# pdlfs/old-vpic

Measured on AMD Instinct MI355X. Metric: particle-pushes/sec (full step: advance_p + sort when due + field solve + glue), higher is better.
Workload: dtype f32

## Files before the change

### include/vpic_hip.h

```cpp
#ifndef VPIC_HIP_H
#define VPIC_HIP_H

#include <stddef.h>
#include <stdint.h>

#ifdef __cplusplus
#define VPIC_HIP_STATIC_ASSERT(c, msg) static_assert(c, msg)
extern "C" {
#else
#define VPIC_HIP_STATIC_ASSERT(c, msg) _Static_assert(c, msg)
#endif


typedef struct vpic_particle {
  float dx, dy, dz;
  int32_t i;
  float ux, uy, uz;
  float q;
  int64_t tag, tag2;
} vpic_particle_t;
typedef struct vpic_particle_mover { float dispx, dispy, dispz; int32_t i; } vpic_particle_mover_t;
typedef struct vpic_particle_injector {
  float dx, dy, dz; int32_t i; float ux, uy, uz, q; float dispx, dispy, dispz; int32_t sp_id;
} vpic_particle_injector_t;
// ... 242 lines not shown
int vpic_hip_advance_p_async(vpic_hip_engine_t *e, int sp);
int vpic_hip_advance_p_phase(vpic_hip_engine_t *e, int sp, int phase);
int vpic_hip_exchange_pack_species(vpic_hip_engine_t *e, uint32_t species_mask, void *const dev_msg[6], const int32_t cap[6], int mover_cap);
int vpic_hip_exchange_begin(vpic_hip_engine_t *e);
int vpic_hip_exchange_pack(vpic_hip_engine_t *e, void *const dev_msg[6], const int32_t cap[6], int mover_cap);
int vpic_hip_exchange_inject(vpic_hip_engine_t *e, const void *dev_msg, int cap);
int vpic_hip_exchange_finish(vpic_hip_engine_t *e, const void *const *dev_msgs, int n_msgs , int32_t *headers , int32_t *flags);
int vpic_hip_boundary_p_counts(vpic_hip_engine_t *e, int32_t ns[6]);
void *vpic_hip_boundary_p_send_buffer(vpic_hip_engine_t *e, int face);
int vpic_hip_boundary_p_get_injectors(vpic_hip_engine_t *e, int face, void *dev_dst);
int vpic_hip_boundary_p_inject(vpic_hip_engine_t *e, const void *dev_injectors, int n);
int vpic_hip_face_count(const vpic_hip_engine_t *e, int dir);
int vpic_hip_pack_tang_b(vpic_hip_engine_t *e, int dir, void *dev_buf);
int vpic_hip_unpack_tang_b(vpic_hip_engine_t *e, int dir, const void *dev_buf);
int vpic_hip_pack_jf(vpic_hip_engine_t *e, int dir, void *dev_buf);
int vpic_hip_unpack_jf(vpic_hip_engine_t *e, int dir, const void *dev_buf);

int vpic_hip_clear_rhof(vpic_hip_engine_t *e);
int vpic_hip_accumulate_rho_p(vpic_hip_engine_t *e, int sp);
int vpic_hip_synchronize_rho(vpic_hip_engine_t *e);
int vpic_hip_local_adjust_rho(vpic_hip_engine_t *e);
int vpic_hip_synchronize_rho_self(vpic_hip_engine_t *e, int axis);
int vpic_hip_rho_count(const vpic_hip_engine_t *e, int dir);
int vpic_hip_pack_rho(vpic_hip_engine_t *e, int dir, void *dev_buf);
int vpic_hip_unpack_rho(vpic_hip_engine_t *e, int dir, const void *dev_buf);
int vpic_hip_compute_rhob(vpic_hip_engine_t *e);
int vpic_hip_compute_curl_b(vpic_hip_engine_t *e);
int vpic_hip_synchronize_tang_e_norm_b(vpic_hip_engine_t *e, double *err);
int vpic_hip_compute_div_e_err(vpic_hip_engine_t *e);
int vpic_hip_clean_div_e(vpic_hip_engine_t *e);
int vpic_hip_compute_div_b_err(vpic_hip_engine_t *e);
int vpic_hip_clean_div_b(vpic_hip_engine_t *e);
enum { VPIC_HIP_MSG_NORM_E = 0, VPIC_HIP_MSG_DIV_B = 1, VPIC_HIP_MSG_TANG_E_NORM_B = 2 };
int vpic_hip_face_message_count(const vpic_hip_engine_t *e, int kind, int dir);
int vpic_hip_pack_face_message(vpic_hip_engine_t *e, int kind, int dir, void *dev_buf);
int vpic_hip_unpack_face_message(vpic_hip_engine_t *e, int kind, int dir, const void *dev_buf, double *err);
int vpic_hip_local_adjust_tang_e_norm_b(vpic_hip_engine_t *e);
int vpic_hip_synchronize_tang_e_norm_b_self(vpic_hip_engine_t *e, int axis, double *err);
int vpic_hip_rms_div_e_err_local(vpic_hip_engine_t *e, double *local2);
int vpic_hip_rms_div_b_err_local(vpic_hip_engine_t *e, double *local2);
int vpic_hip_compute_rms_div_e_err(vpic_hip_engine_t *e, double *rms);
int vpic_hip_compute_rms_div_b_err(vpic_hip_engine_t *e, double *rms);

int vpic_hip_clear_hydro(vpic_hip_engine_t *e);
int vpic_hip_accumulate_hydro_p(vpic_hip_engine_t *e, int sp);
int vpic_hip_moments_stats(vpic_hip_engine_t *e, int64_t out[4]);
int vpic_hip_accumulate_hydro_p_select(vpic_hip_engine_t *e, int sp, const vpic_hip_select_t *s);
int vpic_hip_synchronize_hydro(vpic_hip_engine_t *e);
int vpic_hip_local_adjust_hydro(vpic_hip_engine_t *e);
int vpic_hip_synchronize_hydro_self(vpic_hip_engine_t *e, int axis);
int vpic_hip_hydro_count(const vpic_hip_engine_t *e, int dir);
int vpic_hip_pack_hydro(vpic_hip_engine_t *e, int dir, void *dev_buf);
int vpic_hip_unpack_hydro(vpic_hip_engine_t *e, int dir, const void *dev_buf);
int vpic_hip_set_hydro(vpic_hip_engine_t *e, const vpic_hydro_t *h);
int vpic_hip_get_hydro(vpic_hip_engine_t *e, vpic_hydro_t *h);

enum { VPIC_HIP_DUMP_FIELDS = 0, VPIC_HIP_DUMP_HYDRO = 1 };
enum { VPIC_HIP_DUMP_BAND = 0, VPIC_HIP_DUMP_INTERLEAVE = 1, VPIC_HIP_DUMP_INTERLEAVE_INNER = 2 };
int vpic_hip_dump_gather(vpic_hip_engine_t *e, int what, int layout, const int32_t *words, int nwords,
                         int sx, int sy, int sz, void *out, size_t out_bytes);

#define VPIC_HIP_COMM_ID_BYTES 128
typedef struct vpic_hip_comm vpic_hip_comm_t;
int vpic_hip_comm_unique_id(void *id128);
int vpic_hip_comm_create(vpic_hip_comm_t **c, vpic_hip_engine_t *e, const void *id128, int nranks, int rank);
int vpic_hip_comm_destroy(vpic_hip_comm_t *c);
int vpic_hip_comm_start(vpic_hip_comm_t *c, int n_send, const void *const *sbuf, const size_t *sbytes, const int *speer,
                        int n_recv, void *const *rbuf, const size_t *rbytes, const int *rpeer, int *token);
int vpic_hip_comm_finish(vpic_hip_comm_t *c, int token);
int vpic_hip_comm_stats(vpic_hip_comm_t *c, int64_t *messages_sent, int64_t *bytes_sent);
int vpic_hip_comm_timing(vpic_hip_comm_t *c, int on, double *exchange_ms, double *exposed_ms, int64_t *exchanges);

void *vpic_hip_device_alloc(vpic_hip_engine_t *e, size_t bytes);
void vpic_hip_device_free(vpic_hip_engine_t *e, void *p);
int vpic_hip_copy_to_host(vpic_hip_engine_t *e, void *host, const void *dev, size_t bytes);
int vpic_hip_copy_from_host(vpic_hip_engine_t *e, void *dev, const void *host, size_t bytes);

int vpic_hip_step(vpic_hip_engine_t *e, int64_t step, int sort_interval);

int vpic_hip_sort_due(vpic_hip_engine_t *e, int sp, int max_interval, int *due);
int vpic_hip_measure_disorder(vpic_hip_engine_t *e, int sp, double *fraction);
int vpic_hip_species_sort_order(vpic_hip_engine_t *e, int sp, int *order);
int vpic_hip_species_stats(vpic_hip_engine_t *e, int sp, int64_t out[8]);
int vpic_hip_set_sort_order(vpic_hip_engine_t *e, int order);

int vpic_hip_profile_enable(vpic_hip_engine_t *e, int on);
int vpic_hip_profile_read(vpic_hip_engine_t *e, double *advance_p_ms, int64_t *launches, int64_t *particles);
int vpic_hip_profile_read_sorting(vpic_hip_engine_t *e, double *advance_p_ms, int64_t *launches, int64_t *particles);
int vpic_hip_profile_read_species(vpic_hip_engine_t *e, int sp, double *advance_p_ms, int64_t *launches, int64_t *particles);

#ifdef __cplusplus
}
#endif
#endif
```

### old-vpic_amd/_lib.py

```python
import ctypes as C
import os
import subprocess

HERE = os.path.dirname(os.path.abspath(__file__))
SO = os.path.join(HERE, "libvpic_hip.so")
CSRC = os.path.join(HERE, "csrc")
_lib = None


def build(force=False):
    if force:
        subprocess.check_call(["make", "-s", "-C", CSRC, "clean"])
    subprocess.check_call(["make", "-s", "-C", CSRC, "-j4"])
    if not os.path.exists(SO):
        raise RuntimeError("building libvpic_hip.so failed")
    return SO


def _stale():
    if not os.path.exists(SO):
        return True
    t = os.path.getmtime(SO)
    srcs = [os.path.join(CSRC, f) for f in os.listdir(CSRC) if f.endswith((".hip", ".h"))]
    srcs += [os.path.join(HERE, "..", "include", f) for f in os.listdir(os.path.join(HERE, "..", "include"))]
# ... 25 lines not shown
        L.vpic_hip_species_capacity.argtypes = [C.c_void_p, C.c_int, C.c_void_p, C.c_void_p, C.c_void_p]
        L.vpic_hip_exchange_pack_species.argtypes = [C.c_void_p, C.c_uint32, C.c_void_p, C.c_void_p, C.c_int]
    if hasattr(L, "vpic_hip_set_accumulation"):
        L.vpic_hip_set_accumulation.argtypes = [C.c_void_p, C.c_int, C.c_double]
    L.vpic_hip_push_plan.argtypes = [C.c_int64, C.c_int, C.c_void_p, C.c_void_p, C.c_void_p, C.c_int]
    L.vpic_hip_set_reflux_draws.argtypes = [C.c_void_p, C.c_void_p, C.c_int64]
    L.vpic_hip_set_emit_draws.argtypes = [C.c_void_p, C.c_void_p, C.c_int64]
    L.vpic_hip_species_append_particles.argtypes = [C.c_void_p, C.c_int, C.c_void_p, C.c_int64]
    L.vpic_hip_emit.argtypes = [C.c_void_p, C.c_int, C.c_void_p, C.c_int, C.c_int, C.c_float, C.c_float, C.c_float, C.c_float, C.c_uint32]
    L.vpic_hip_inject_aged.argtypes = [C.c_void_p, C.c_void_p, C.c_void_p, C.c_int]
    L.vpic_hip_accumulate_rhob.argtypes = [C.c_void_p, C.c_void_p, C.c_int64, C.c_float]
    L.vpic_hip_set_maxwellian_reflux.argtypes = [C.c_void_p, C.c_int, C.c_void_p, C.c_void_p, C.c_int, C.c_uint32]
    L.vpic_hip_species_get_movers.argtypes = [C.c_void_p, C.c_int, C.c_void_p, C.c_int64]
    L.vpic_hip_species_np.argtypes = [C.c_void_p, C.c_int]
    L.vpic_hip_species_load_maxwellian.argtypes = [C.c_void_p, C.c_int, C.c_int, C.c_uint32] + [C.c_float] * 5
    L.vpic_hip_species_nm.argtypes = [C.c_void_p, C.c_int]
    L.vpic_hip_advance_b.argtypes = [C.c_void_p, C.c_float]
    L.vpic_hip_step.argtypes = [C.c_void_p, C.c_int64, C.c_int]
    L.vpic_hip_boundary_p_send_buffer.argtypes = [C.c_void_p, C.c_int]
    L.vpic_hip_boundary_p_inject.argtypes = [C.c_void_p, C.c_void_p, C.c_int]
    L.vpic_hip_boundary_p_get_injectors.argtypes = [C.c_void_p, C.c_int, C.c_void_p]
    L.vpic_hip_synchronize_jf_self.argtypes = [C.c_void_p, C.c_int]
    L.vpic_hip_exchange_pack.argtypes = [C.c_void_p, C.c_void_p, C.c_void_p, C.c_int]
    L.vpic_hip_exchange_inject.argtypes = [C.c_void_p, C.c_void_p, C.c_int]
    L.vpic_hip_exchange_finish.argtypes = [C.c_void_p, C.c_void_p, C.c_int, C.c_void_p, C.c_void_p]
    L.vpic_hip_stream_wait_event.argtypes = [C.c_void_p, C.c_void_p]
    L.vpic_hip_advance_e_part.argtypes = [C.c_void_p, C.c_int]
    for n in ("vpic_hip_pack_tang_b", "vpic_hip_unpack_tang_b", "vpic_hip_pack_jf", "vpic_hip_unpack_jf"):
        getattr(L, n).argtypes = [C.c_void_p, C.c_int, C.c_void_p]
    L.vpic_hip_face_count.argtypes = [C.c_void_p, C.c_int]
    if hasattr(L, "vpic_hip_comm_create"):
        L.vpic_hip_comm_unique_id.argtypes = [C.c_void_p]
        L.vpic_hip_comm_create.argtypes = [C.c_void_p, C.c_void_p, C.c_void_p, C.c_int, C.c_int]
        L.vpic_hip_comm_destroy.argtypes = [C.c_void_p]
        L.vpic_hip_comm_start.argtypes = [C.c_void_p, C.c_int, C.c_void_p, C.c_void_p, C.c_void_p, C.c_int, C.c_void_p, C.c_void_p, C.c_void_p, C.c_void_p]
        L.vpic_hip_comm_finish.argtypes = [C.c_void_p, C.c_int]
        L.vpic_hip_comm_stats.argtypes = [C.c_void_p, C.c_void_p, C.c_void_p]
        L.vpic_hip_comm_timing.argtypes = [C.c_void_p, C.c_int, C.c_void_p, C.c_void_p, C.c_void_p]
    L.vpic_hip_energy_spectrum.argtypes = [C.c_void_p, C.c_int, C.c_void_p, C.c_void_p, C.c_void_p]
    L.vpic_hip_energy_bands.argtypes = [C.c_void_p, C.c_int, C.c_void_p, C.c_void_p]
    L.vpic_hip_energy_spectrum_stats.argtypes = [C.c_void_p, C.c_void_p]
    L.vpic_hip_species_distribution.argtypes = [C.c_void_p, C.c_int, C.c_void_p, C.c_void_p]
    L.vpic_hip_species_distribution_stats.argtypes = [C.c_void_p, C.c_void_p]
    L.vpic_hip_species_distribution_sums.argtypes = [C.c_void_p, C.c_int, C.c_void_p, C.c_void_p, C.c_int, C.c_void_p, C.c_void_p]
    L.vpic_hip_species_distribution_sums_stats.argtypes = [C.c_void_p, C.c_void_p]
    L.vpic_hip_cell_distribution.argtypes = [C.c_void_p, C.c_void_p, C.c_void_p, C.c_int, C.c_void_p, C.c_void_p]
    L.vpic_hip_cell_distribution_stats.argtypes = [C.c_void_p, C.c_void_p]
    L.vpic_hip_moments_stats.argtypes = [C.c_void_p, C.c_void_p]
    L.vpic_hip_species_select_count.argtypes = [C.c_void_p, C.c_int, C.c_void_p, C.c_void_p]
    L.vpic_hip_species_select.argtypes = [C.c_void_p, C.c_int, C.c_void_p, C.c_int64] + [C.c_void_p] * 4
    L.vpic_hip_species_select_stats.argtypes = [C.c_void_p, C.c_void_p]
    L.vpic_hip_accumulate_hydro_p_select.argtypes = [C.c_void_p, C.c_int, C.c_void_p]
    if hasattr(L, "vpic_hip_collide"):
        L.vpic_hip_collide.argtypes = [C.c_void_p, C.c_void_p]
        L.vpic_hip_collide_stats.argtypes = [C.c_void_p, C.c_void_p]
        L.vpic_hip_collide_instance.argtypes = [C.c_void_p, C.c_void_p]
        L.vpic_hip_set_collide_draws.argtypes = [C.c_void_p, C.c_void_p, C.c_int64]
    if hasattr(L, "vpic_hip_collide_relativistic"):
        L.vpic_hip_collide_relativistic.argtypes = [C.c_void_p, C.c_void_p]
    if hasattr(L, "vpic_hip_wall_setup"):
        L.vpic_hip_wall_setup.argtypes = [C.c_void_p, C.c_double, C.c_double, C.c_int64]
        L.vpic_hip_set_wall.argtypes = [C.c_void_p, C.c_int, C.c_int]
        L.vpic_hip_wall_tally.argtypes = [C.c_void_p, C.c_void_p, C.c_int, C.c_int]
        L.vpic_hip_wall_records.argtypes = [C.c_void_p, C.c_void_p, C.c_int64, C.c_void_p, C.c_void_p, C.c_int]
    if hasattr(L, "vpic_hip_species_load_profile"):
        L.vpic_hip_species_load_profile.argtypes = [C.c_void_p, C.c_int, C.c_void_p, C.c_void_p]
        L.vpic_hip_set_load_draws.argtypes = [C.c_void_p, C.c_void_p, C.c_int64]
    L.vpic_hip_dump_gather.argtypes = [C.c_void_p, C.c_int, C.c_int, C.c_void_p] + [C.c_int] * 4 + [C.c_void_p, C.c_size_t]
    _lib = L
    return L


EXPORTS = """vpic_hip_clear_jf_unload_accumulator vpic_hip_set_emit_draws vpic_hip_set_reflux_draws vpic_hip_set_host_access_hook vpic_hip_last_error vpic_hip_device_count vpic_hip_create vpic_hip_destroy vpic_hip_sync
vpic_hip_stream vpic_hip_nv vpic_hip_set_fields vpic_hip_get_fields vpic_hip_set_interpolator
vpic_hip_get_interpolator vpic_hip_set_accumulator vpic_hip_get_accumulator
vpic_hip_set_material_coefficients vpic_hip_species_create vpic_hip_species_set_particles vpic_hip_species_append_particles vpic_hip_set_maxwellian_reflux vpic_hip_accumulate_rhob vpic_hip_inject_aged vpic_hip_emit
vpic_hip_species_get_particles vpic_hip_species_load_maxwellian vpic_hip_species_np vpic_hip_species_nm vpic_hip_species_get_movers
vpic_hip_species_get_partition vpic_hip_load_interpolator vpic_hip_clear_accumulators
vpic_hip_reduce_accumulators vpic_hip_unload_accumulator vpic_hip_advance_p vpic_hip_sort_p
vpic_hip_set_push_mode vpic_hip_species_get_particles_range vpic_hip_push_plan vpic_hip_species_sort_hint vpic_hip_set_accumulation vpic_hip_advance_p_async vpic_hip_advance_p_phase vpic_hip_exchange_pack_species vpic_hip_species_capacity vpic_hip_species_reserve vpic_hip_exchange_begin vpic_hip_exchange_pack vpic_hip_exchange_inject vpic_hip_exchange_finish vpic_hip_advance_e_part vpic_hip_stream_wait_event vpic_hip_energy_p vpic_hip_center_p vpic_hip_uncenter_p vpic_hip_clear_jf vpic_hip_sort_due vpic_hip_species_sort_order vpic_hip_set_sort_order vpic_hip_measure_disorder vpic_hip_species_set_movers vpic_hip_device_alloc vpic_hip_device_free vpic_hip_copy_to_host vpic_hip_copy_from_host vpic_hip_clear_hydro vpic_hip_accumulate_hydro_p vpic_hip_synchronize_hydro vpic_hip_local_adjust_hydro vpic_hip_synchronize_hydro_self vpic_hip_hydro_count vpic_hip_pack_hydro vpic_hip_unpack_hydro vpic_hip_set_hydro vpic_hip_get_hydro vpic_hip_dump_gather vpic_hip_clear_rhof vpic_hip_accumulate_rho_p vpic_hip_synchronize_rho vpic_hip_local_adjust_rho vpic_hip_synchronize_rho_self vpic_hip_rho_count vpic_hip_pack_rho vpic_hip_unpack_rho vpic_hip_compute_rhob vpic_hip_compute_curl_b vpic_hip_synchronize_tang_e_norm_b vpic_hip_face_message_count vpic_hip_pack_face_message vpic_hip_unpack_face_message vpic_hip_local_adjust_tang_e_norm_b vpic_hip_synchronize_tang_e_norm_b_self vpic_hip_compute_div_e_err vpic_hip_clean_div_e vpic_hip_compute_div_b_err vpic_hip_clean_div_b vpic_hip_rms_div_e_err_local vpic_hip_rms_div_b_err_local vpic_hip_compute_rms_div_e_err vpic_hip_compute_rms_div_b_err vpic_hip_synchronize_jf vpic_hip_advance_b vpic_hip_advance_e
vpic_hip_energy_f vpic_hip_boundary_p_pack vpic_hip_boundary_p_counts vpic_hip_boundary_p_send_buffer
vpic_hip_boundary_p_inject vpic_hip_boundary_p_get_injectors vpic_hip_local_adjust_jf
vpic_hip_synchronize_jf_self vpic_hip_face_count vpic_hip_pack_tang_b vpic_hip_unpack_tang_b
vpic_hip_pack_jf vpic_hip_unpack_jf vpic_hip_step vpic_hip_profile_enable vpic_hip_profile_read vpic_hip_profile_read_sorting vpic_hip_sort_advance_p vpic_hip_species_get_tile_partition vpic_hip_profile_read_species vpic_hip_comm_unique_id vpic_hip_comm_create vpic_hip_comm_destroy vpic_hip_comm_start vpic_hip_comm_finish vpic_hip_comm_stats vpic_hip_comm_timing vpic_hip_species_stats
vpic_hip_energy_spectrum vpic_hip_energy_bands vpic_hip_energy_spectrum_stats
vpic_hip_species_distribution vpic_hip_species_distribution_stats vpic_hip_moments_stats
vpic_hip_species_distribution_sums vpic_hip_species_distribution_sums_stats
vpic_hip_cell_distribution vpic_hip_cell_distribution_stats
vpic_hip_species_select_count vpic_hip_species_select vpic_hip_species_select_stats
vpic_hip_accumulate_hydro_p_select
vpic_hip_wall_setup vpic_hip_set_wall vpic_hip_wall_tally vpic_hip_wall_records
vpic_hip_collide vpic_hip_collide_relativistic vpic_hip_collide_stats vpic_hip_collide_instance vpic_hip_set_collide_draws
vpic_hip_species_load_profile vpic_hip_set_load_draws""".split()
```

### old-vpic_amd/csrc/engine.h

```cpp
#pragma once
#include <hip/hip_runtime.h>
#include <stdint.h>
#include <string>
#include <vector>
#include "vpic_hip.h"
#include "policy.h"
#include "moments_device.h"

namespace vpichip {

void set_error(const char *fmt, ...);
#define VH_CHECK(expr)                                                                     \
  do {                                                                                     \
    hipError_t _e = (expr);                                                                \
    if (_e != hipSuccess) {                                                                \
      vpichip::set_error("%s failed: %s (%s:%d)", #expr, hipGetErrorString(_e), __FILE__, __LINE__); \
      return 1;                                                                            \
    }                                                                                      \
  } while (0)
#define VH_FAIL(...) do { vpichip::set_error(__VA_ARGS__); return 1; } while (0)

struct GridK {
  int nx, ny, nz, sy, sz, nv;
  int fbc[6], pbc[6];
  int rank;
};

enum { F_EX = 0, F_EY, F_EZ, F_DIV_E_ERR, F_CBX, F_CBY, F_CBZ, F_DIV_B_ERR,
       F_TCAX, F_TCAY, F_TCAZ, F_RHOB, F_JFX, F_JFY, F_JFZ, F_RHOF, F_NCOMP };
enum { M_EMATX = 0, M_EMATY, M_EMATZ, M_NMAT, M_FMATX, M_FMATY, M_FMATZ, M_CMAT, M_NCOMP };
struct FieldsK {
  float *c[F_NCOMP];
  uint16_t *m[M_NCOMP];
};

struct ParticlesK {
  float4 *r;
  float *ux, *uy, *uz, *q;
};
__host__ __device__ __forceinline__ float4 make_record(float dx, float dy, float dz, int i) {
  union { int i; float f; } w; w.i = i;
  return make_float4(dx, dy, dz, w.f);
}
__device__ __forceinline__ int record_cell(const float4 *r, long long k) { return __float_as_int(r[k].w); }
__device__ __forceinline__ int record_cell(const float4 &v) { return __float_as_int(v.w); }
__device__ __forceinline__ void record_set_cell(float4 *r, long long k, int i) { r[k].w = __int_as_float(i); }
__host__ __device__ __forceinline__ ParticlesK offset_particles(const ParticlesK &p, int64_t at) {
  ParticlesK o = p;
  o.r += at; o.ux += at; o.uy += at; o.uz += at; o.q += at;
  return o;
}

struct DrainParams {
  int nx, ny, nz, sy, sz, rank, max_nm;
  unsigned mul_sz;
  int pbc[6];
  unsigned mul_sy, shifts;
  vpic_particle_mover_t *pm;
  int *nm_counter;
};

inline void magic_div(unsigned d, unsigned &mul, unsigned &shift) {
  unsigned l = 0;
  while ((1ull << l) < d) l++;
  const unsigned p = 31 + l;
  mul = (unsigned)(((unsigned long long)1 << p) / d + 1);
  shift = p - 32;
}

enum { C_NM = 0, C_DISORDER = 1, C_LOCAL = 2, C_SEND = 8, C_HOLES = 14, C_FILLS = 15, C_NP = 16, C_NMS = 48, C_CHARGED = 80, C_OVER = 81, C_RETRY = 82, C_QMSG = 83, C_NHOLE = 96, C_QTOP = 128, C_TOTAL = 160 };
constexpr int MAX_SPECIES = 32;
constexpr int HEADER_BASE = 256, MAX_HEADERS = 192;
constexpr int RETRY_CAP = 1 << 16;
static_assert(C_NMS + MAX_SPECIES == C_CHARGED && C_NP + MAX_SPECIES == C_NMS && C_NHOLE + MAX_SPECIES == C_QTOP && C_QTOP + MAX_SPECIES == C_TOTAL && C_TOTAL <= HEADER_BASE, "counter layout");

struct Species {
  float q_m = 0;
  float q_max = 0;
  int64_t np = 0, max_np = 0, nm = 0, max_nm = 0;
  int64_t n_holes = 0;
  ParticlesK p{}, aux{};
  DrainParams *drain_k = nullptr;
  hipEvent_t ev[4] = {nullptr, nullptr, nullptr, nullptr};
  bool push_timed = false, sort_timed = false;
  Policy pol;
  int64_t *tag = nullptr, *tag2 = nullptr, *tag_aux = nullptr, *tag2_aux = nullptr;
  bool has_tags = false;
  unsigned *crossed_dev = nullptr, *crossed_host = nullptr, *crossed_host_dev = nullptr;
  bool chargeless = false;
  vpic_particle_mover_t *pm = nullptr;
  int *nm_dev = nullptr;
  int *partition = nullptr;
  bool partition_valid = false;
  int *tpart = nullptr; int64_t tpart_count = 0;
  int *ttail = nullptr;
  bool tail_sorted = false;
  int *hist = nullptr; int64_t hist_count = 0; bool hist_request = false, hist_valid = false;
  bool tail_regrouped = false;
  int *tpart2 = nullptr; int64_t tpart2_count = 0; bool fuse_pending = false;
  bool phase_pending = false;
  bool tile_valid = false, adaptive = false;
  int64_t n_sorted = 0;
  bool coarse_sorted = false;
  hipEvent_t sp_ev[2] = {nullptr, nullptr}; int sp_kind = -1;
  hipEvent_t hp_ev[2] = {nullptr, nullptr}; bool hp_pending = false;
};

constexpr int TILE_CELLS = TILE_EDGE * TILE_EDGE * TILE_EDGE;
struct TileK {
  int sy, sz, ntx, nty, ntz, ntiles;
  unsigned mul_sy, sh_sy, mul_sz, sh_sz;
  int mx, my, mz;
};
TileK make_tile_k(const GridK &g);

__device__ __forceinline__ void voxel_cell(int voxel, const TileK &t, int &cx, int &cy, int &cz) {
  cz = (int)(__umulhi((unsigned)voxel, t.mul_sz) >> t.sh_sz);
  const int rem = voxel - cz * t.sz;
  cy = (int)(__umulhi((unsigned)rem, t.mul_sy) >> t.sh_sy);
  cx = rem - cy * t.sy;
}

template <bool TILE>
__device__ __forceinline__ int sort_key(int voxel, const TileK &t) {
  if (!TILE) return voxel;
  int cx, cy, cz;
  voxel_cell(voxel, t, cx, cy, cz);
  const int x = min(max(cx - 1, 0), t.mx), y = min(max(cy - 1, 0), t.my), z = min(max(cz - 1, 0), t.mz);
  const int tile = ((z >> 2) * t.nty + (y >> 2)) * t.ntx + (x >> 2);
  return tile * TILE_CELLS + ((z & 3) << 4 | (y & 3) << 2 | (x & 3));
}

template <typename T>
__device__ __forceinline__ void add_together(T *word, int a, bool on, int lane) {
  const unsigned long long any = __ballot(on);
  if (!any) return;
  const int lead = __ffsll((long long)any) - 1;
  const int a0 = __builtin_amdgcn_readlane(a, lead);
  const unsigned long long same = __ballot(on && a == a0);
  if (on) {
    if (a != a0) atomicAdd(word + a, (T)1);
    else if (lane == lead) atomicAdd(word + a, (T)__popcll(same));
  }
}

constexpr int SUMS_TOGETHER_MIN = 8;

__device__ __forceinline__ void add_sums_together(unsigned long long *word, int a, long long x, bool on, bool together,
                                                  unsigned long long same, int lead, int lane) {
  bool mine = on;
  if (together) {
    const bool shared = same >> lane & 1ull;
    long long s = shared ? x : 0;
#pragma unroll
    for (int m = 32; m >= 1; m >>= 1) s += __shfl_xor(s, m);
    if (shared) { mine = lane == lead; x = s; }
  }
  if (mine && x) atomicAdd(word + a, (unsigned long long)x);
}

constexpr int WINDOW_BACKOFF = 16;
struct SlideWindow {
  int base = 0, backoff = 0;
  bool placed = false;
};
template <typename Place, typename Flush>
__device__ __forceinline__ bool window_add(SlideWindow &w, unsigned *win, int n_slots, int stride, int pos, int offset, bool pending, int lane,
                                           Place place, Flush flush) {
  for (int round = 0; round < 3; round++) {
    if (round > 0) {
      const unsigned long long left = __ballot(pending && pos >= 0);
      if (!left) break;
      if (w.backoff > 0) { w.backoff--; break; }
      if (w.placed) flush(w.base);
      w.base = place(left);
      w.placed = true;
    }
    const bool hit = w.placed && pending && pos >= w.base && pos < w.base + n_slots;
    add_together(win, (pos - w.base) * stride + offset, hit, lane);
    if (hit) pending = false;
    if (round == 2 && __popcll(__ballot(pending)) > 32) w.backoff = WINDOW_BACKOFF;
  }
  return pending;
}

struct Knobs {
  int window = 0;
  int tile_coarse = -1;
  long long tail_sort_min = 4096;
  bool no_tail_sort = false;
  int iters = 0;
  int ablate = 0;
  bool policy_debug = false;
  int follow = -1;
  int fuse_in_step = -1;
  bool old_sort = false;
  int stage = -1;
  int follow_from = 16;
  bool early_sort = true;
  int unload_tiled = 1;
  int field_tiles = 0;
  bool rho_per_particle = false, hydro_per_particle = false;
  bool collide_group = false;
  bool moments_tiled = true;
};
Knobs read_knobs();

template <typename T, bool PINNED = false>
inline int grow(T *&buf, size_t &have, size_t want) {
  if (want <= have) return 0;
  (void)(PINNED ? hipHostFree(buf) : hipFree(buf)); buf = nullptr; have = 0;
  VH_CHECK(PINNED ? hipHostMalloc((void **)&buf, want * sizeof(T), hipHostMallocDefault) : hipMalloc((void **)&buf, want * sizeof(T)));
  have = want;
  return 0;
}
template <typename T> inline int grow_pinned(T *&buf, size_t &have, size_t want) { return grow<T, true>(buf, have, want); }

template <int WORDS>
struct DiagStats {
  unsigned long long *dev = nullptr, *host = nullptr;
  int64_t last[WORDS] = {};
  bool pending = false;
  int begin(hipStream_t stream) {
    if (!dev) VH_CHECK(hipMalloc((void **)&dev, (WORDS + 1) * sizeof(unsigned long long)));
    if (!host) VH_CHECK(hipHostMalloc((void **)&host, WORDS * sizeof(unsigned long long), hipHostMallocDefault));
    VH_CHECK(hipMemsetAsync(dev, 0, (WORDS + 1) * sizeof(unsigned long long), stream));
    return 0;
  }
  int read(hipStream_t stream) {
    VH_CHECK(hipMemcpyAsync(host, dev, WORDS * sizeof(unsigned long long), hipMemcpyDeviceToHost, stream));
    VH_CHECK(hipStreamSynchronize(stream));
    for (int j = 0; j < WORDS; j++) last[j] = (int64_t)host[j];
    pending = false;
    return 0;
  }
  unsigned *bad_partition() const { return reinterpret_cast<unsigned *>(dev + WORDS); }
  void release() { (void)hipFree(dev); (void)hipHostFree(host); dev = host = nullptr; }
};

struct HistResult {
  unsigned long long *counts = nullptr, *counts_host = nullptr, *sums = nullptr, *sums_host = nullptr;
  size_t bins = 0, words = 0;
  DiagStats<8> stats;
  static int grow_pair(unsigned long long *&dev, unsigned long long *&host, size_t &have, size_t want) {
    size_t dev_have = have;
    return grow(dev, dev_have, want) || grow_pinned(host, have, want);
  }
  int grow_counts(size_t n_bins) { return grow_pair(counts, counts_host, bins, n_bins); }
  int grow_sums(size_t n_words) { return grow_pair(sums, sums_host, words, n_words); }
  int begin(size_t n_bins, size_t n_words, hipStream_t stream) {
    if (grow_counts(n_bins) || grow_sums(n_words) || stats.begin(stream)) return 1;
    VH_CHECK(hipMemsetAsync(counts, 0, n_bins * sizeof(unsigned long long), stream));
    if (n_words) VH_CHECK(hipMemsetAsync(sums, 0, n_words * sizeof(unsigned long long), stream));
    return 0;
  }
  int read(size_t n_bins, size_t n_words, hipStream_t stream) {
    VH_CHECK(hipMemcpyAsync(counts_host, counts, n_bins * sizeof(unsigned long long), hipMemcpyDeviceToHost, stream));
    if (n_words) VH_CHECK(hipMemcpyAsync(sums_host, sums, n_words * sizeof(unsigned long long), hipMemcpyDeviceToHost, stream));
    return stats.read(stream);
  }
  void release() {
    (void)hipFree(counts); (void)hipHostFree(counts_host); (void)hipFree(sums); (void)hipHostFree(sums_host);
    counts = counts_host = sums = sums_host = nullptr; bins = words = 0;
    stats.release();
  }
};

struct Engine {
  int device = 0;
  Knobs knobs;
  hipStream_t stream = nullptr;
  vpic_hip_grid_t grid{};
  GridK gk{};
  FieldsK f{};
  float *field_block = nullptr;
  uint16_t *mat_block = nullptr;
  vpic_material_coefficient_t *mc = nullptr;
  int n_mat = 0;
// ... 61 lines not shown
  hipEvent_t step_done[4] = {}; int64_t steps_enqueued = 0;
  bool profile = false;
  std::vector<std::pair<hipEvent_t, hipEvent_t>> ev_pool;
  size_t ev_used = 0;
  std::vector<int64_t> ev_particles;
  std::vector<char> ev_kind;
  std::vector<int> ev_species;
  double prof_sp_ms[MAX_SPECIES] = {}; int64_t prof_sp_launches[MAX_SPECIES] = {}, prof_sp_particles[MAX_SPECIES] = {};
  double prof_ms = 0; int64_t prof_launches = 0, prof_particles = 0;
  double prof_sort_ms = 0; int64_t prof_sort_launches = 0, prof_sort_particles = 0;
};

int ensure_stage(Engine *e, size_t bytes);
int acc_prepare_det(Engine *e, double q_arriving = 0);
int acc_finalize(Engine *e);
void host_will_read(const void *p, size_t bytes);
void host_will_write(void *p, size_t bytes);
constexpr int PUSH_TILE = 64;
constexpr int64_t PARTICLE_PAD = 2048;
int alloc_particles(ParticlesK &p, int64_t n);
void free_particles(ParticlesK &p);

int k_fields_from_aos(Engine *e, const vpic_field_t *host);
int k_fields_to_aos(Engine *e, vpic_field_t *host);
int k_load_interpolator(Engine *e);
int k_unload_accumulator(Engine *e);
int k_clear_jf(Engine *e);
int k_clear_jf_unload_accumulator(Engine *e);
int k_synchronize_jf_local(Engine *e);
int k_synchronize_jf_self(Engine *e, int axis);
int k_advance_b(Engine *e, float frac);
int k_advance_e(Engine *e, int part = 0);
int k_energy_f(Engine *e, double *en6);
int k_clear_rhof(Engine *e);
int k_accumulate_rho_p(Engine *e, Species &s, bool wants_tile);
int k_rho_p_untiled(Engine *e, Species &s, bool by_cell);
int k_compute_div_e_err(Engine *e);
int k_compute_rhob(Engine *e);
int k_rms_div_e_err_local(Engine *e, double *local2);
int k_rms_div_b_err_local(Engine *e, double *local2);
int k_clean_div_e(Engine *e);
int k_compute_div_b_err(Engine *e);
int k_clean_div_b(Engine *e);
int k_compute_curl_b(Engine *e);
enum { FAM_TANG_B = 0, FAM_JF, FAM_RHO, FAM_HYDRO, FAM_NORM_E, FAM_DIV_B, FAM_TANG_E_NORM_B, FAM_COUNT };
int k_msg_count(const Engine *e, int fam, int dir);
int k_pack_msg(Engine *e, int fam, int dir, float *buf);
int k_unpack_msg(Engine *e, int fam, int dir, const float *buf);
int k_local_adjust(Engine *e, int fam);
int k_synchronize_self(Engine *e, int fam, int axis);
int k_synchronize_local(Engine *e, int fam, double *err = nullptr);
int k_err_begin(Engine *e);
int k_err_read(Engine *e, double *err);
int ensure_hydro(Engine *e);
int k_dump_gather(Engine *e, int what, int layout, const int32_t *words, int nwords, int sx, int sy, int sz, void *out, size_t out_bytes);
int k_clear_hydro(Engine *e);
int k_accumulate_hydro_p(Engine *e, Species &s, bool wants_tile);
int k_accumulate_hydro_p_select(Engine *e, Species &s, const vpic_hip_select_t &d);
int k_hydro_p_untiled(Engine *e, Species &s, bool by_cell);
HydroConsts hydro_consts(const Engine *e, const Species &s);
int k_moments_stats(Engine *e, int64_t out[4]);
int k_check_tile_partition(Engine *e, const Species &s, unsigned *bad);
inline bool tile_partition_usable(const Species &s, const TileK &t) {
  return s.tile_valid && s.tpart && s.tpart_count >= (int64_t)t.ntiles * TILE_CELLS + 1 && s.n_sorted >= 0 && s.n_sorted <= s.np;
}

int k_particles_from_aos(Engine *e, Species &s, const vpic_particle_t *host, int64_t n_new, int64_t at = 0, bool any_voxel = false);
int k_particles_to_aos(Engine *e, Species &s, vpic_particle_t *host, int64_t cap, int64_t from = 0, int64_t count = -1);
int k_load_maxwellian(Engine *e, Species &s, int ppc, unsigned seed, float q, float ux, float uy, float uz, float vth);
int ensure_tags(Engine *e, Species &s);
int k_load_profile(Engine *e, Species &s, const vpic_hip_load_t &d, int64_t *n_loaded);
int k_energy_p(Engine *e, Species &s, double *energy);
int k_center_p(Engine *e, Species &s, bool uncenter);
int k_energy_spectrum(Engine *e, Species &s, const vpic_hip_spectrum_t &sp);
int k_energy_bands(Engine *e, int n_lin);
int k_species_distribution(Engine *e, Species &s, const vpic_hip_dist_t &d);
int k_species_distribution_sums(Engine *e, Species &s, const vpic_hip_dist_t &d, const vpic_hip_dist_value_t *v, int n_val);
int k_cell_distribution(Engine *e, const vpic_hip_dist_t &d, const vpic_hip_dist_value_t *v, int n_val);
int k_species_select(Engine *e, Species &s, const vpic_hip_select_t &d, int64_t cap, bool want_p, bool want_f, bool want_i, bool count_only);
int k_collide(Engine *e, const vpic_hip_collision_t &c, bool wants_tile_a, bool wants_tile_b, bool relativistic);
int k_sort_p(Engine *e, Species &s, bool tile_order = false, bool may_fuse = false);
int k_sort_scan(Engine *e, const int *counts, int *starts, int n1);
int k_sort_check(Engine *e, Species &s, const int *starts, int n1);
int k_sort_finish(Engine *e, Species &s, bool tile_order, bool coarse);
int k_tail_sort(Engine *e, Species &s);
int k_measure_disorder(Engine *e, Species &s, int slot);
int k_boundary_p_pack(Engine *e);
int k_exchange_begin(Engine *e);
int k_exchange_pack(Engine *e, void *const msg[6], const int32_t cap[6], int mover_cap, uint32_t species_mask = ~0u);
int k_compact(Engine *e, Species &s);
int k_species_reserve(Engine *e, Species &s, int64_t max_np, int64_t max_nm);
int k_exchange_inject(Engine *e, const void *msg, int cap);
int k_exchange_finish(Engine *e, const void *const *recv, int n_recv, int32_t *headers_out, int32_t *flags_out);
int k_advance_p(Engine *e, Species &s, bool async = false, int phase = 0);
int k_boundary_p_inject(Engine *e, const vpic_particle_injector_t *inj, int n, const int64_t *tags = nullptr);
int k_emit(Engine *e, int sp, const int32_t *host_components, int n, int n_emit, float ut_perp, float ut_para, float coef, float thresh, unsigned seed);
int k_inject_aged(Engine *e, const vpic_particle_injector_t *host_inj, const int64_t *host_tags, int n);
int k_accumulate_rhob(Engine *e, const vpic_particle_t *host, int64_t n, float q_scale);

__device__ __forceinline__ int pbc_of(const GridK &g, int face) {
  return face == 0 ? g.pbc[0] : face == 1 ? g.pbc[1] : face == 2 ? g.pbc[2]
       : face == 3 ? g.pbc[3] : face == 4 ? g.pbc[4] : g.pbc[5];
}

__device__ __forceinline__ unsigned xcd_block(unsigned b, unsigned nb) {
  const unsigned per = nb >> 3;
  if (per == 0 || (nb & 7)) return b;
  return (b & 7) * per + (b >> 3);
}

}

struct vpic_hip_engine : public vpichip::Engine {};
```

### old-vpic_amd/csrc/engine.hip

```cpp
#include "engine.h"
#include "cell_coords.h"
#include <algorithm>
#include <cstdarg>
#include <cstdio>
#include <cstring>
#include <functional>
#include <cstdlib>
#include <cmath>

namespace vpichip {

static thread_local char g_error[1024] = "";
void set_error(const char *fmt, ...) {
  va_list ap;
  va_start(ap, fmt);
  vsnprintf(g_error, sizeof(g_error), fmt, ap);
  va_end(ap);
}

static vpic_hip_host_access_fn g_host_access = nullptr;
void host_will_read(const void *p, size_t bytes) { if (g_host_access && p && bytes) g_host_access(p, bytes, 0); }
void host_will_write(void *p, size_t bytes) { if (g_host_access && p && bytes) g_host_access(p, bytes, 1); }

int ensure_stage(Engine *e, size_t bytes) { return grow(e->stage, e->stage_bytes, bytes); }

Knobs read_knobs() {
  Knobs k;
  if (const char *w = getenv("VPIC_HIP_WINDOW")) k.window = (w[0] == 't' || w[0] == 'w' || w[0] == 'n') ? w[0] : 0;
  if (const char *c = getenv("VPIC_HIP_TILE_COARSE")) k.tile_coarse = atoi(c) != 0;
  if (const char *t = getenv("VPIC_HIP_TAIL_SORT_MIN")) k.tail_sort_min = atoll(t);
  k.no_tail_sort = getenv("VPIC_HIP_NO_TAIL_SORT") != nullptr;
  if (const char *it = getenv("VPIC_HIP_ITERS")) k.iters = atoi(it) > 0 ? atoi(it) : 0;
  if (const char *ab = getenv("VPIC_HIP_ABLATE")) k.ablate = atoi(ab);
  k.policy_debug = getenv("VPIC_HIP_POLICY_DEBUG") != nullptr;
  k.old_sort = getenv("VPIC_HIP_OLD_SORT") != nullptr;
  if (const char *v = getenv("VPIC_HIP_SORT_IN_PUSH")) k.fuse_in_step = atoi(v) != 0 ? 1 : 0;
  if (const char *v = getenv("VPIC_HIP_FOLLOW")) k.follow = atoi(v) != 0;
  if (const char *v = getenv("VPIC_HIP_STAGE")) k.stage = atoi(v) != 0;
  if (const char *v = getenv("VPIC_HIP_FOLLOW_FROM")) k.follow_from = atoi(v) > 0 ? atoi(v) : 16;
  if (const char *v = getenv("VPIC_HIP_EARLY_SORT")) k.early_sort = atoi(v) != 0;
  if (const char *v = getenv("VPIC_HIP_UNLOAD_TILED")) k.unload_tiled = atoi(v);
  if (const char *v = getenv("VPIC_HIP_FIELD_TILES")) k.field_tiles = atoi(v);
  k.rho_per_particle = getenv("VPIC_HIP_RHO_PER_PARTICLE") != nullptr;
  k.hydro_per_particle = getenv("VPIC_HIP_HYDRO_PER_PARTICLE") != nullptr;
  if (const char *v = getenv("VPIC_HIP_MOMENTS_TILED")) k.moments_tiled = atoi(v) != 0;
  if (const char *v = getenv("VPIC_HIP_COLLIDE_INSTANCE")) k.collide_group = v[0] == 'g';
  return k;
}

static int validate_grid(const vpic_hip_grid_t *g) {
  if (!g) VH_FAIL("Bad grid");
  if (g->nx < 1 || g->ny < 1 || g->nz < 1) VH_FAIL("Bad resolution %d x %d x %d", g->nx, g->ny, g->nz);
  const int64_t nv = (int64_t)(g->nx + 2) * (g->ny + 2) * (g->nz + 2);
  if (nv * 12 >= (1ll << 31)) VH_FAIL("domain of %lld voxels is too large for 32-bit voxel arithmetic", (long long)nv);
  if (!(g->dt > 0) || !(g->cvac > 0) || !(g->eps0 > 0)) VH_FAIL("Bad dt/cvac/eps0");
  for (int f = 0; f < 6; f++) {
    if (g->fbc[f] < VPIC_ABSORB_FIELDS) VH_FAIL("Bad field boundary code %d on face %d", g->fbc[f], f);
  }
  for (int a = 0; a < 3; a++) {
    if ((g->fbc[a] == g->rank) != (g->fbc[a + 3] == g->rank)) VH_FAIL("axis %d: field faces are periodic on one side only", a);
    if ((g->pbc[a] == g->rank) != (g->pbc[a + 3] == g->rank)) VH_FAIL("axis %d: particle faces are periodic on one side only", a);
  }
  return 0;
}

static int create(Engine *e, const vpic_hip_grid_t *g, int device) {
  if (validate_grid(g)) return 1;
  e->knobs = read_knobs();
  int n_dev = 0;
  if (hipGetDeviceCount(&n_dev) != hipSuccess || n_dev < 1)
    VH_FAIL("no HIP device is available: the MI355X engine has no CPU fallback");
  if (device >= 0) { VH_CHECK(hipSetDevice(device)); }
  VH_CHECK(hipGetDevice(&e->device));
  VH_CHECK(hipStreamCreateWithFlags(&e->stream, hipStreamNonBlocking));
  e->grid = *g;
  GridK &k = e->gk;
  k.nx = g->nx; k.ny = g->ny; k.nz = g->nz;
  k.sy = g->nx + 2; k.sz = k.sy * (g->ny + 2); k.nv = k.sz * (g->nz + 2);
  for (int f = 0; f < 6; f++) { k.fbc[f] = g->fbc[f]; k.pbc[f] = g->pbc[f]; }
  k.rank = g->rank;
  for (int f = 0; f < 6; f++) if (g->pbc[f] != g->rank && g->pbc[f] != VPIC_REFLECT_PARTICLES) e->can_strand = true;
  const size_t nv = (size_t)k.nv;

  VH_CHECK(hipMalloc(&e->field_block, sizeof(float) * F_NCOMP * nv));
  VH_CHECK(hipMemsetAsync(e->field_block, 0, sizeof(float) * F_NCOMP * nv, e->stream));
  for (int c = 0; c < F_NCOMP; c++) e->f.c[c] = e->field_block + c * nv;
  for (int c = 0; c < M_NCOMP; c++) e->f.m[c] = nullptr;
  VH_CHECK(hipMalloc(&e->fi, sizeof(vpic_interpolator_t) * nv));
  VH_CHECK(hipMemsetAsync(e->fi, 0, sizeof(vpic_interpolator_t) * nv, e->stream));
  VH_CHECK(hipMalloc(&e->acc_block, sizeof(vpic_accumulator_t) * nv));
  e->acc = reinterpret_cast<vpic_accumulator_t *>(e->acc_block);
  VH_CHECK(hipHostMalloc(&e->host_miss, sizeof(int) * MAX_SPECIES));
  for (int k = 0; k < MAX_SPECIES; k++) e->host_miss[k] = 0;
  VH_CHECK(hipMemsetAsync(e->acc, 0, sizeof(vpic_accumulator_t) * nv, e->stream));

  VH_CHECK(hipMalloc(&e->counters, sizeof(int) * 256));
  VH_CHECK(hipMemsetAsync(e->counters, 0, sizeof(int) * 256, e->stream));
  VH_CHECK(hipHostMalloc(&e->host_counters, sizeof(int) * (HEADER_BASE + 4 * MAX_HEADERS)));
  e->dsum_count = 6 * 1024;
  VH_CHECK(hipMalloc(&e->dsum, sizeof(double) * e->dsum_count));
  VH_CHECK(hipHostMalloc(&e->host_dsum, sizeof(double) * e->dsum_count));
  {
    const TileK tk = make_tile_k(e->gk);
    const size_t n1 = (size_t)std::max((int64_t)nv, (int64_t)tk.ntiles * TILE_CELLS) + 1;
    VH_CHECK(hipMalloc(&e->sort_next, sizeof(int) * n1));
    e->scan_tmp_count = (n1 + 1023) / 1024 + 1;
  }
  VH_CHECK(hipMalloc(&e->scan_tmp, sizeof(int) * e->scan_tmp_count));
  size_t face = 0;
  for (int fam = 0; fam < FAM_COUNT; fam++) {
    if (fam == FAM_HYDRO) continue;
    for (int d = 0; d < 3; d++) face = std::max(face, (size_t)k_msg_count(e, fam, d));
  }
  e->face_buf_count = face;
  VH_CHECK(hipMalloc(&e->face_buf[0], sizeof(float) * face));
  VH_CHECK(hipMalloc(&e->face_buf[1], sizeof(float) * face));
  VH_CHECK(hipStreamSynchronize(e->stream));
  return 0;
}

__global__ __launch_bounds__(256)
void acc_finalize_kernel(float *__restrict__ acc, unsigned long long *__restrict__ acc64, size_t n, double inv_scale) {
  const size_t k = (size_t)blockIdx.x * 256 + threadIdx.x;
  if (k >= n) return;
  const long long v = (long long)acc64[k];
  if (v) { acc[k] += (float)((double)v * inv_scale); acc64[k] = 0; }
}
static double fixed_scale(double largest) {
  int ex = 0;
  (void)frexp(largest, &ex);
  return ldexp(1.0, 37 - ex);
}
int acc_prepare_det(Engine *e, double q_arriving) {
  if (!e->acc64) {
    VH_CHECK(hipMalloc(&e->acc64, sizeof(unsigned long long) * 12 * (size_t)e->gk.nv));
    VH_CHECK(hipMemsetAsync(e->acc64, 0, sizeof(unsigned long long) * 12 * (size_t)e->gk.nv, e->stream));
  }
  if (e->acc_scale == 0) {
    double q = e->acc_qref;
    if (!(q > 0)) for (auto &s : e->species) q = std::max(q, (double)s.q_max);
    if (!(q > 0)) q = q_arriving;
    if (!(q > 0) && q_arriving < 0) return 0;
    if (!(q > 0)) VH_FAIL("deterministic accumulation: no macro-particle charge is known yet (give vpic_hip_set_accumulation a reference charge)");
    e->acc_scale = fixed_scale(4.2 * q);
  }
  e->acc64_dirty = true;
  return 0;
}
int acc_finalize(Engine *e) {
  if (!e->acc64 || !e->acc64_dirty) return 0;
  const size_t n = 12 * (size_t)e->gk.nv;
  hipLaunchKernelGGL(acc_finalize_kernel, dim3((unsigned)((n + 255) / 256)), dim3(256), 0, e->stream,
                     reinterpret_cast<float *>(e->acc), e->acc64, n, 1.0 / e->acc_scale);
  VH_CHECK(hipGetLastError());
  e->acc64_dirty = false;
  return 0;
}

void free_particles(ParticlesK &p) {
  (void)hipFree(p.r);
  (void)hipFree(p.ux); (void)hipFree(p.uy); (void)hipFree(p.uz); (void)hipFree(p.q);
  p = ParticlesK{};
}

static void destroy(Engine *e) {
  if (e->stream) (void)hipStreamSynchronize(e->stream);
  for (auto &s : e->species) {
    free_particles(s.p); free_particles(s.aux);
    (void)hipFree(s.tag); (void)hipFree(s.tag2); (void)hipFree(s.tag_aux); (void)hipFree(s.tag2_aux);
    (void)hipFree(s.pm); (void)hipFree(s.partition); (void)hipFree(s.tpart); (void)hipFree(s.tpart2); (void)hipFree(s.ttail); (void)hipFree(s.hist); (void)hipFree(s.drain_k); (void)hipFree(s.crossed_dev); (void)hipHostFree(s.crossed_host);
    for (int i = 0; i < 4; i++) if (s.ev[i]) (void)hipEventDestroy(s.ev[i]);
    for (auto ev : s.sp_ev) if (ev) (void)hipEventDestroy(ev);
    for (auto ev : s.hp_ev) if (ev) (void)hipEventDestroy(ev);
  }
  (void)hipFree(e->field_block); (void)hipFree(e->mat_block); (void)hipFree(e->mc);
  (void)hipFree(e->fi); (void)hipFree(e->acc_block); (void)hipHostFree(e->host_miss); (void)hipFree(e->stage); (void)hipFree(e->counters); (void)hipFree(e->hydro); (void)hipFree(e->hydro_buf[0]); (void)hipFree(e->hydro_buf[1]);
  (void)hipHostFree(e->host_counters); (void)hipFree(e->dsum); (void)hipHostFree(e->host_dsum);
  (void)hipFree(e->sort_next); (void)hipFree(e->scan_tmp);
  (void)hipFree(e->face_buf[0]); (void)hipFree(e->face_buf[1]);
  for (int f = 0; f < 6; f++) (void)hipFree(e->send_buf[f]);
  (void)hipFree(e->local_buf); (void)hipFree(e->reflux_draws); (void)hipFree(e->emit_draws);
  (void)hipFree(e->wall_table); (void)hipFree(e->wall_rec); (void)hipFree(e->wall_cursor);
  (void)hipFree(e->collide_draws); (void)hipFree(e->collide_dev); (void)hipHostFree(e->collide_host);
  (void)hipFree(e->load_draws); (void)hipFree(e->load_tab);
  (void)hipFree(e->hole_list); (void)hipFree(e->fill_list); (void)hipFree(e->tail_flag);
  (void)hipFree(e->sp_table_dev); (void)hipHostFree(e->sp_table_host); (void)hipFree(e->xmsg_dev); (void)hipHostFree(e->xmsg_host);
  (void)hipFree(e->retry_buf); (void)hipFree(e->tile_list[0]); (void)hipFree(e->tile_list[1]);
  (void)hipFree(e->acc64); (void)hipFree(e->rho64);
  (void)hipFree(e->spec_lin); (void)hipFree(e->spec_bands); (void)hipFree(e->spec_log); (void)hipHostFree(e->spec_log_host);
  e->species_hist.release(); e->cell_hist.release(); (void)hipFree(e->hydro64);
  (void)hipFree(e->sel_mask); (void)hipFree(e->sel_offsets); (void)hipFree(e->sel_counts);
  (void)hipFree(e->sel_p); (void)hipFree(e->sel_f); (void)hipFree(e->sel_i);
  for (DiagStats<4> *st : {&e->spec_stats, &e->dist_stats, &e->mom_stats, &e->sel_stats}) st->release();
  for (auto &ev : e->ev_pool) { (void)hipEventDestroy(ev.first); (void)hipEventDestroy(ev.second); }
  for (auto ev : e->step_done) if (ev) (void)hipEventDestroy(ev);
  if (e->stream) (void)hipStreamDestroy(e->stream);
}

static int collect_profile(Engine *e) {
  for (size_t k = 0; k < e->ev_used; k++) {
    float ms = 0;
    VH_CHECK(hipEventSynchronize(e->ev_pool[k].second));
    VH_CHECK(hipEventElapsedTime(&ms, e->ev_pool[k].first, e->ev_pool[k].second));
    if (e->ev_kind[k]) { e->prof_sort_ms += ms; e->prof_sort_launches++; e->prof_sort_particles += e->ev_particles[k]; continue; }
    e->prof_ms += ms;
    if (e->ev_particles[k] >= 0) { e->prof_launches++; e->prof_particles += e->ev_particles[k]; }
    const int sp = e->ev_species[k];
    if (sp >= 0 && sp < MAX_SPECIES) {
      e->prof_sp_ms[sp] += ms;
      if (e->ev_particles[k] >= 0) { e->prof_sp_launches[sp]++; e->prof_sp_particles[sp] += e->ev_particles[k]; }
    }
  }
  e->ev_used = 0;
  return 0;
}

}

using namespace vpichip;

#define ENGINE(e) do { if (!(e)) { set_error("null engine"); return 1; } if (hipSetDevice((e)->device) != hipSuccess) { set_error("hipSetDevice failed"); return 1; } } while (0)
#define SPECIES(e, sp) do { if ((sp) < 0 || (size_t)(sp) >= (e)->species.size()) { set_error("bad species id %d", (sp)); return 1; } } while (0)

extern "C" {

const char *vpic_hip_last_error(void) { return g_error; }
void vpic_hip_set_host_access_hook(vpic_hip_host_access_fn fn) { g_host_access = fn; }

int vpic_hip_device_count(void) {
  int n = 0;
  if (hipGetDeviceCount(&n) != hipSuccess) return 0;
  return n;
}

int vpic_hip_create(vpic_hip_engine_t **out, const vpic_hip_grid_t *g, int device) {
  if (!out) { set_error("null output pointer"); return 1; }
  *out = nullptr;
  vpic_hip_engine *e = new vpic_hip_engine();
  if (create(e, g, device)) { destroy(e); delete e; return 1; }
  *out = e;
  return 0;
}

void vpic_hip_destroy(vpic_hip_engine_t *e) {
  if (!e) return;
  (void)hipSetDevice(e->device);
  destroy(e);
  delete e;
}

int vpic_hip_sync(vpic_hip_engine_t *e) { ENGINE(e); VH_CHECK(hipStreamSynchronize(e->stream)); return 0; }
void *vpic_hip_stream(vpic_hip_engine_t *e) { return e ? (void *)e->stream : nullptr; }
int vpic_hip_nv(const vpic_hip_engine_t *e) { return e ? e->gk.nv : 0; }
// ... 752 lines not shown
  double l2[2];
  if (k_rms_div_b_err_local(e, l2)) return 1;
  *rms = e->grid.eps0 * sqrt(l2[0] / l2[1]);
  return 0;
}
int vpic_hip_synchronize_jf(vpic_hip_engine_t *e) { ENGINE(e); return k_synchronize_jf_local(e); }
int vpic_hip_local_adjust_jf(vpic_hip_engine_t *e) { ENGINE(e); return k_local_adjust(e, FAM_JF); }
int vpic_hip_synchronize_jf_self(vpic_hip_engine_t *e, int axis) {
  ENGINE(e);
  if (axis < 0 || axis > 2) VH_FAIL("bad axis %d", axis);
  return k_synchronize_jf_self(e, axis);
}
int vpic_hip_advance_b(vpic_hip_engine_t *e, float frac) { ENGINE(e); return k_advance_b(e, frac); }
int vpic_hip_advance_e(vpic_hip_engine_t *e) { ENGINE(e); return k_advance_e(e); }
int vpic_hip_advance_e_part(vpic_hip_engine_t *e, int part) { ENGINE(e); if (part < 0 || part > 2) VH_FAIL("Bad part"); return k_advance_e(e, part); }
int vpic_hip_stream_wait_event(vpic_hip_engine_t *e, void *event) { ENGINE(e); VH_CHECK(hipStreamWaitEvent(e->stream, (hipEvent_t)event, 0)); return 0; }
int vpic_hip_energy_f(vpic_hip_engine_t *e, double *en6) {
  ENGINE(e);
  if (!en6) VH_FAIL("Bad energy");
  return k_energy_f(e, en6);
}

int vpic_hip_boundary_p_pack(vpic_hip_engine_t *e) { ENGINE(e); return k_boundary_p_pack(e); }
void *vpic_hip_device_alloc(vpic_hip_engine_t *e, size_t bytes) {
  if (!e || hipSetDevice(e->device) != hipSuccess) return nullptr;
  void *p = nullptr;
  if (hipMalloc(&p, bytes ? bytes : 1) != hipSuccess) { set_error("out of device memory (%zu bytes)", bytes); return nullptr; }
  return p;
}
void vpic_hip_device_free(vpic_hip_engine_t *e, void *p) { if (e && p) { (void)hipSetDevice(e->device); (void)hipFree(p); } }
int vpic_hip_copy_to_host(vpic_hip_engine_t *e, void *host, const void *dev, size_t bytes) {
  ENGINE(e); if (bytes && (!host || !dev)) VH_FAIL("Bad buffer");
  return bytes ? copy_out(e, host, dev, bytes) : 0;
}
int vpic_hip_copy_from_host(vpic_hip_engine_t *e, void *dev, const void *host, size_t bytes) {
  ENGINE(e); if (bytes && (!host || !dev)) VH_FAIL("Bad buffer");
  return bytes ? copy_in(e, dev, host, bytes) : 0;
}
int vpic_hip_boundary_p_counts(vpic_hip_engine_t *e, int32_t ns[6]) {
  ENGINE(e);
  for (int f = 0; f < 6; f++) ns[f] = e->send_count[f];
  return 0;
}
void *vpic_hip_boundary_p_send_buffer(vpic_hip_engine_t *e, int face) {
  return (e && face >= 0 && face < 6) ? (void *)e->send_buf[face] : nullptr;
}
int vpic_hip_boundary_p_get_injectors(vpic_hip_engine_t *e, int face, void *dev_dst) {
  ENGINE(e);
  if (face < 0 || face > 5 || !dev_dst) VH_FAIL("bad face/buffer");
  const size_t n = (size_t)e->send_count[face];
  if (n) VH_CHECK(hipMemcpyAsync(dev_dst, e->send_buf[face], n * sizeof(vpic_particle_injector_t), hipMemcpyDeviceToDevice, e->stream));
  return 0;
}
int vpic_hip_boundary_p_inject(vpic_hip_engine_t *e, const void *dev_injectors, int n) {
  ENGINE(e);
  return k_boundary_p_inject(e, (const vpic_particle_injector_t *)dev_injectors, n);
}

int vpic_hip_face_count(const vpic_hip_engine_t *e, int dir) { return (e && dir >= 0 && dir < 6) ? k_msg_count(e, FAM_TANG_B, dir) : 0; }
int vpic_hip_pack_tang_b(vpic_hip_engine_t *e, int dir, void *buf) { ENGINE(e); if (dir < 0 || dir > 5 || !buf) VH_FAIL("Bad face message"); return k_pack_msg(e, FAM_TANG_B, dir, (float *)buf); }
int vpic_hip_unpack_tang_b(vpic_hip_engine_t *e, int dir, const void *buf) { ENGINE(e); if (dir < 0 || dir > 5 || !buf) VH_FAIL("Bad face message"); return k_unpack_msg(e, FAM_TANG_B, dir, (const float *)buf); }
int vpic_hip_pack_jf(vpic_hip_engine_t *e, int dir, void *buf) { ENGINE(e); if (dir < 0 || dir > 5 || !buf) VH_FAIL("Bad face message"); return k_pack_msg(e, FAM_JF, dir, (float *)buf); }
int vpic_hip_unpack_jf(vpic_hip_engine_t *e, int dir, const void *buf) { ENGINE(e); if (dir < 0 || dir > 5 || !buf) VH_FAIL("Bad face message"); return k_unpack_msg(e, FAM_JF, dir, (const float *)buf); }

static int sort_due(Engine *e, Species &s, int max_interval, int *due) {
  e->time_kernels = true;
  s.adaptive = true;
  const float sort_ms = s.sort_timed ? event_ms(s.ev + 2, true) : -1, push_ms = s.push_timed ? event_ms(s.ev, true) : -1;
  if (sort_ms >= 0) s.sort_timed = false;
  if (push_ms >= 0) s.push_timed = false;
  *due = vpichip::sort_due(s.pol, sort_ms, push_ms, s.coarse_sorted, s.tile_valid, max_interval, e->knobs.policy_debug);
  return 0;
}
int vpic_hip_sort_due(vpic_hip_engine_t *e, int sp, int max_interval, int *due) {
  ENGINE(e); SPECIES(e, sp); if (!due) VH_FAIL("Bad output");
  return sort_due(e, e->species[sp], max_interval, due);
}

int vpic_hip_species_sort_hint(vpic_hip_engine_t *e, int sp) {
  ENGINE(e); SPECIES(e, sp);
  e->species[sp].hist_request = true;
  return 0;
}
int vpic_hip_species_stats(vpic_hip_engine_t *e, int sp, int64_t out[8]) {
  ENGINE(e); SPECIES(e, sp); if (!out) VH_FAIL("Bad output");
  const Species &s = e->species[sp];
  out[0] = s.crossed_host ? s.crossed_host[PW_CROSSERS] : 0; out[1] = s.crossed_host ? s.crossed_host[PW_FULLEST_TILE] : 0; out[2] = s.crossed_host ? s.crossed_host[PW_MISSED] : 0;
  out[3] = s.pol.n_cycle; out[4] = s.pol.early_sorts; out[5] = s.pol.tile_unbalanced; out[6] = s.coarse_sorted; out[7] = s.n_holes;
  return 0;
}
int vpic_hip_species_sort_order(vpic_hip_engine_t *e, int sp, int *order) {
  ENGINE(e); SPECIES(e, sp); if (!order) VH_FAIL("Bad output");
  const Species &s = e->species[sp];
  *order = s.tile_valid ? 2 : s.partition_valid ? 1 : 0;
  return 0;
}

int vpic_hip_step(vpic_hip_engine_t *e, int64_t step, int sort_interval) {
  ENGINE(e);
  for (int f = 0; f < 6; f++) {
    const int fb = e->gk.fbc[f], pb = e->gk.pbc[f];
    if ((fb >= 0 && fb != e->gk.rank) || (pb >= 0 && pb != e->gk.rank))
      VH_FAIL("vpic_hip_step drives single-domain steps; face %d is shared with another domain", f);
  }
  if (!e->step_done[0]) for (auto &ev : e->step_done) VH_CHECK(hipEventCreateWithFlags(&ev, hipEventDisableTiming));
  if (e->steps_enqueued >= 2) VH_CHECK(hipEventSynchronize(e->step_done[(e->steps_enqueued - 2) & 3]));
  if (vpic_hip_clear_accumulators(e)) return 1;
  std::vector<int> due_list;
  for (size_t k = 0; k < e->species.size(); k++) {
    Species &s = e->species[k];
    int due = sort_interval > 0 && step % sort_interval == 0;
    if (sort_interval < 0 && sort_due(e, s, -sort_interval, &due)) return 1;
    if (!due && sort_interval > 0 && e->knobs.early_sort && s.tile_valid && !s.chargeless && s.crossed_host &&
        early_sort(s.pol, s.crossed_host[PW_MISSED], s.crossed_host[PW_CYCLE], sort_interval - step % sort_interval, make_tile_k(e->gk).ntiles, s.np)) due = 1;
    if (due) due_list.push_back((int)k);
  }
  std::vector<char> pushed(e->species.size(), 0), sort_first(e->species.size(), 0);
  auto push = [&](size_t k) -> int {
    Species &s = e->species[k];
    pushed[k] = 1;
    auto hints = [&](Species &sp) -> int {
      if (sort_interval > 0 && (step + 1) % sort_interval == 0 && wants_tile_order(e, sp)) sp.hist_request = true;
      return order_for_deterministic_push(e, sp);
    };
    if (sort_first[k]) { sort_first[k] = 0; return sort_and_push(e, s, sort_interval > 0, hints); }
    if (hints(s)) return 1;
    return push_timing_hinted(e, s);
  };
  for (int k : due_list) sort_first[(size_t)k] = 1;
  for (size_t k = 0; k < e->species.size(); k++) if (!pushed[k] && push(k)) return 1;
  for (int round = 0; round < 3; round++) {
    if (k_boundary_p_pack(e)) return 1;
    bool pending = false;
    for (auto &s : e->species) pending = pending || s.nm > 0;
    if (!pending) break;
  }
  if (k_clear_jf_unload_accumulator(e)) return 1;
  if (k_synchronize_jf_local(e)) return 1;
  if (k_advance_b(e, 0.5f)) return 1;
  if (k_advance_e(e)) return 1;
  if (k_advance_b(e, 0.5f)) return 1;
  if (k_load_interpolator(e)) return 1;
  VH_CHECK(hipEventRecord(e->step_done[e->steps_enqueued & 3], e->stream));
  e->steps_enqueued++;
  return 0;
}

int vpic_hip_measure_disorder(vpic_hip_engine_t *e, int sp, double *fraction) {
  ENGINE(e); SPECIES(e, sp); if (!fraction || sp >= MAX_SPECIES) VH_FAIL("Bad argument");
  if (k_measure_disorder(e, e->species[sp], sp)) return 1;
  VH_CHECK(hipStreamSynchronize(e->stream));
  *fraction = e->species[sp].np ? 8.0 * e->host_miss[sp] / (double)e->species[sp].np : 0.0;
  return 0;
}
int vpic_hip_profile_enable(vpic_hip_engine_t *e, int on) {
  ENGINE(e);
  if (collect_profile(e)) return 1;
  e->profile = on != 0;
  e->prof_ms = 0; e->prof_launches = 0; e->prof_particles = 0;
  e->prof_sort_ms = 0; e->prof_sort_launches = 0; e->prof_sort_particles = 0;
  for (int k = 0; k < MAX_SPECIES; k++) { e->prof_sp_ms[k] = 0; e->prof_sp_launches[k] = 0; e->prof_sp_particles[k] = 0; }
  return 0;
}
int vpic_hip_profile_read_species(vpic_hip_engine_t *e, int sp, double *ms, int64_t *launches, int64_t *particles) {
  ENGINE(e); SPECIES(e, sp); if (sp >= MAX_SPECIES) VH_FAIL("bad species id %d", sp);
  VH_CHECK(hipStreamSynchronize(e->stream));
// ... 27 lines not shown
```

### old-vpic_amd/csrc/particles.hip

```cpp
#include "push_device.h"
#include "unit_draw.h"
#include "dist_coords.h"
#include <cstddef>
#include <cstring>
#include <algorithm>

namespace vpichip {

__global__ void particles_from_aos_kernel(ParticlesK p, int64_t *tag, int64_t *tag2,
                                          const vpic_particle_t *__restrict__ src, int64_t first, int n) {
  const int t = blockIdx.x * blockDim.x + threadIdx.x;
  if (t >= n) return;
  const vpic_particle_t s = src[t];
  const int64_t k = first + t;
  p.r[k] = make_record(s.dx, s.dy, s.dz, s.i);
  p.ux[k] = s.ux; p.uy[k] = s.uy; p.uz[k] = s.uz; p.q[k] = s.q;
  if (tag) { tag[k] = s.tag; tag2[k] = s.tag2; }
}
__global__ void particles_to_aos_kernel(ParticlesK p, const int64_t *tag, const int64_t *tag2,
                                        vpic_particle_t *__restrict__ dst, int64_t first, int n) {
  const int t = blockIdx.x * blockDim.x + threadIdx.x;
  if (t >= n) return;
  const int64_t k = first + t;
  vpic_particle_t s;
// ... 402 lines not shown
__device__ __forceinline__ int tile_of(int voxel, const TileK &t) { return sort_key<true>(voxel, t) / TILE_CELLS; }

__device__ __forceinline__ int coarse_slot(int *s_key, int tile) {
  unsigned h = ((unsigned)tile * 2654435761u) >> 25;
  for (int probe = 0; probe < COARSE_TABLE; probe++) {
    const int prev = atomicCAS(&s_key[h], -1, tile);
    if (prev == -1 || prev == tile) return (int)h;
    h = (h + 1) & (COARSE_TABLE - 1);
  }
  return -1;
}

__global__ __launch_bounds__(256)
void coarse_count_kernel(const float4 *__restrict__ rec, int np, int *__restrict__ count, const TileK t) {
  __shared__ int s_key[COARSE_TABLE], s_cnt[COARSE_TABLE];
  if (threadIdx.x < COARSE_TABLE) { s_key[threadIdx.x] = -1; s_cnt[threadIdx.x] = 0; }
  __syncthreads();
  const int first = blockIdx.x * COARSE_CHUNK;
#pragma unroll
  for (int j = 0; j < COARSE_PER_THREAD; j++) {
    const int idx = first + j * 256 + threadIdx.x;
    const int voxel = idx < np ? record_cell(rec, idx) : -1;
    if (voxel >= 0) {
      const int tile = tile_of(voxel, t);
      const int h = coarse_slot(s_key, tile);
      if (h >= 0) atomicAdd(&s_cnt[h], 1);
      else atomicAdd(&count[tile * TILE_CELLS], 1);
    }
  }
  __syncthreads();
  if (threadIdx.x < COARSE_TABLE && s_key[threadIdx.x] >= 0) atomicAdd(&count[s_key[threadIdx.x] * TILE_CELLS], s_cnt[threadIdx.x]);
}

int alloc_particles(ParticlesK &p, int64_t n_req) {
  const int64_t n = (n_req + PUSH_TILE + PARTICLE_PAD - 1) / PARTICLE_PAD * PARTICLE_PAD;
  if (alloc_particles_raw(p, n)) return 1;
  VH_CHECK(hipMemset(p.r + (n - PARTICLE_PAD), 0, sizeof(float4) * PARTICLE_PAD));
  float *arr[4] = {p.ux, p.uy, p.uz, p.q};
  for (float *a : arr) VH_CHECK(hipMemset(a + (n - PARTICLE_PAD), 0, sizeof(float) * PARTICLE_PAD));
  VH_CHECK(hipDeviceSynchronize());
  return 0;
}
static int alloc_particles_raw_impl(ParticlesK &p, int64_t n) {
  VH_CHECK(hipMalloc(&p.r, sizeof(float4) * n));
  VH_CHECK(hipMalloc(&p.ux, sizeof(float) * n)); VH_CHECK(hipMalloc(&p.uy, sizeof(float) * n));
  VH_CHECK(hipMalloc(&p.uz, sizeof(float) * n)); VH_CHECK(hipMalloc(&p.q, sizeof(float) * n));
  return 0;
}

__global__ __launch_bounds__(256) void tile_max_kernel(const int *__restrict__ tpart, int ntiles, unsigned *__restrict__ host_word) {
  __shared__ int s_max[4];
  int m = 0;
  for (int t = blockIdx.x * 256 + threadIdx.x; t < ntiles; t += gridDim.x * 256) m = max(m, tpart[(t + 1) * TILE_CELLS] - tpart[t * TILE_CELLS]);
  for (int off = 32; off; off >>= 1) m = max(m, __shfl_down(m, off));
  if ((threadIdx.x & 63) == 0) s_max[threadIdx.x >> 6] = m;
  __syncthreads();
  if (threadIdx.x == 0) atomicMax(host_word, (unsigned)max(max(s_max[0], s_max[1]), max(s_max[2], s_max[3])));
}
__global__ void clear_word_kernel(unsigned *__restrict__ w) { *w = 0; }
__global__ void publish_word_kernel(unsigned *__restrict__ host_word, const unsigned *__restrict__ dev_word) { *host_word = *dev_word; }

int k_sort_p(Engine *e, Species &s, bool tile_order, bool may_fuse) {
  const TileK tk = make_tile_k(e->gk);
  const int n1 = (tile_order ? tk.ntiles * TILE_CELLS : e->gk.nv) + 1;
  SortInputs in;
  in.tile_order = tile_order; in.may_fuse = may_fuse; in.np = s.np; in.n_sorted = s.n_sorted;
  in.adaptive = s.adaptive; in.chargeless = s.chargeless; in.has_tags = s.has_tags;
  in.tile_valid = s.tile_valid; in.coarse_sorted = s.coarse_sorted; in.counts_ready = s.hist_valid && s.hist && s.hist_count >= n1;
  in.det_acc = e->det_acc; in.time_kernels = e->time_kernels; in.tile_coarse = e->knobs.tile_coarse; in.old_sort = e->knobs.old_sort;
  const SortPlan pl = plan_sort(s.pol, in);
  const bool coarse = pl.coarse;
  const int nv = e->gk.nv;
  if (!s.partition) VH_CHECK(hipMalloc(&s.partition, sizeof(int) * (nv + 1)));
  if (tile_order && s.tpart_count < n1) {
    if (s.tpart) VH_CHECK(hipFree(s.tpart));
    s.tpart = nullptr; s.tpart_count = 0;
    VH_CHECK(hipMalloc(&s.tpart, sizeof(int) * n1));
    s.tpart_count = n1;
  }
  s.tile_valid = false;
  if (s.np == s.n_holes) { s.np = 0; s.n_holes = 0; }
  if (s.np == 0) return 0;
  if (!s.aux.r && alloc_particles(s.aux, s.max_np)) return 1;
  if (s.has_tags && !s.tag_aux) {
    VH_CHECK(hipMalloc(&s.tag_aux, sizeof(int64_t) * s.max_np));
    VH_CHECK(hipMalloc(&s.tag2_aux, sizeof(int64_t) * s.max_np));
  }
  const int np = (int)s.np;
  s.fuse_pending = false;
  if (pl.fuse) {
    if (s.tpart2_count < n1) {
      if (s.tpart2) VH_CHECK(hipFree(s.tpart2));
      s.tpart2 = nullptr; s.tpart2_count = 0;
      VH_CHECK(hipMalloc(&s.tpart2, sizeof(int) * n1));
      s.tpart2_count = n1;
    }
    s.fuse_pending = true; s.tile_valid = true;
    return 0;
  }
  const bool by_wave = pl.by_wave, count_by_wave = pl.count_by_wave;
  int *starts = tile_order ? s.tpart : s.partition;
  if (e->time_kernels) { if (!s.ev[0]) for (int i = 0; i < 4; i++) VH_CHECK(hipEventCreate(&s.ev[i])); (void)hipEventRecord(s.ev[2], e->stream); }
  const bool counted = pl.counted;
  const int *counts = counted ? s.hist : e->sort_next;
  s.hist_valid = false;
  if (counted) {}
  else VH_CHECK(hipMemsetAsync(e->sort_next, 0, sizeof(int) * n1, e->stream));
  if (counted) {}
  else if (coarse) hipLaunchKernelGGL(coarse_count_kernel, dim3((np + COARSE_CHUNK - 1) / COARSE_CHUNK), dim3(256), 0, e->stream, (const float4 *)s.p.r, np, e->sort_next, tk);
  else if (count_by_wave) {
    if (tile_order) hipLaunchKernelGGL(sort_count_kernel<true>, dim3((np + 255) / 256), dim3(256), 0, e->stream, (const float4 *)s.p.r, np, e->sort_next, tk);
    else hipLaunchKernelGGL(sort_count_kernel<false>, dim3((np + 255) / 256), dim3(256), 0, e->stream, (const float4 *)s.p.r, np, e->sort_next, tk);
  }
  else if (tile_order) hipLaunchKernelGGL(wg_count_kernel<true>, dim3((np + WG_CHUNK - 1) / WG_CHUNK), dim3(WG_T), 0, e->stream, (const float4 *)s.p.r, np, e->sort_next, tk);
  else hipLaunchKernelGGL(wg_count_kernel<false>, dim3((np + WG_CHUNK - 1) / WG_CHUNK), dim3(WG_T), 0, e->stream, (const float4 *)s.p.r, np, e->sort_next, tk);
  if (k_sort_scan(e, counts, starts, n1)) return 1;
  if (coarse) hipLaunchKernelGGL((wg_scatter_kernel<true, true>), dim3(((np + WG_CHUNK - 1) / WG_CHUNK + 7) / 8 * 8), dim3(WG_T), 0, e->stream, s.p, s.aux,
                             s.has_tags ? s.tag : nullptr, s.tag2, s.tag_aux, s.tag2_aux, np, e->sort_next, tk);
  else if (by_wave) {
    if (tile_order) hipLaunchKernelGGL(sort_scatter_kernel<true>, dim3((np + 255) / 256), dim3(256), 0, e->stream, s.p, s.aux,
                                       s.has_tags ? s.tag : nullptr, s.tag2, s.tag_aux, s.tag2_aux, np, e->sort_next, tk);
    else hipLaunchKernelGGL(sort_scatter_kernel<false>, dim3((np + 255) / 256), dim3(256), 0, e->stream, s.p, s.aux,
                            s.has_tags ? s.tag : nullptr, s.tag2, s.tag_aux, s.tag2_aux, np, e->sort_next, tk);
  }
  else if (tile_order) hipLaunchKernelGGL(wg_scatter_kernel<true>, dim3(((np + WG_CHUNK - 1) / WG_CHUNK + 7) / 8 * 8), dim3(WG_T), 0, e->stream, s.p, s.aux,
                                     s.has_tags ? s.tag : nullptr, s.tag2, s.tag_aux, s.tag2_aux, np, e->sort_next, tk);
  else hipLaunchKernelGGL(wg_scatter_kernel<false>, dim3(((np + WG_CHUNK - 1) / WG_CHUNK + 7) / 8 * 8), dim3(WG_T), 0, e->stream, s.p, s.aux,
                          s.has_tags ? s.tag : nullptr, s.tag2, s.tag_aux, s.tag2_aux, np, e->sort_next, tk);
  VH_CHECK(hipGetLastError());
  if (counted && k_sort_check(e, s, starts, n1)) return 1;
  return k_sort_finish(e, s, tile_order, coarse);
}

int k_sort_scan(Engine *e, const int *counts, int *starts, int n1) {
  const int nb = (n1 + 1023) / 1024;
  hipLaunchKernelGGL(scan_local_kernel, dim3(nb), dim3(256), 0, e->stream, counts, starts, e->scan_tmp, n1);
  hipLaunchKernelGGL(scan_blocks_kernel, dim3(1), dim3(256), 0, e->stream, e->scan_tmp, nb);
  hipLaunchKernelGGL(scan_add_kernel, dim3(nb), dim3(256), 0, e->stream, starts, e->sort_next, e->scan_tmp, n1);
  VH_CHECK(hipGetLastError());
  return 0;
}

int k_sort_finish(Engine *e, Species &s, bool tile_order, bool coarse) {
  const TileK tk = make_tile_k(e->gk);
  if (tile_order) {
    unsigned *word = reinterpret_cast<unsigned *>(e->counters + 200);
    hipLaunchKernelGGL(clear_word_kernel, dim3(1), dim3(1), 0, e->stream, word);
    hipLaunchKernelGGL(tile_max_kernel, dim3((unsigned)std::min(256, (tk.ntiles + 255) / 256)), dim3(256), 0, e->stream, s.tpart, tk.ntiles, word);
    hipLaunchKernelGGL(publish_word_kernel, dim3(1), dim3(1), 0, e->stream, s.crossed_host_dev + PW_FULLEST_TILE, (const unsigned *)word);
  }
  VH_CHECK(hipGetLastError());
  std::swap(s.p, s.aux);
  if (s.has_tags) { std::swap(s.tag, s.tag_aux); std::swap(s.tag2, s.tag2_aux); }
  s.np -= s.n_holes; s.n_holes = 0;
  s.partition_valid = !tile_order;
  s.tile_valid = tile_order; s.n_sorted = s.np; s.coarse_sorted = coarse;
  if (s.crossed_dev) VH_CHECK(hipMemsetAsync(s.crossed_dev + 2, 0, sizeof(unsigned), e->stream));
  if (e->time_kernels) { (void)hipEventRecord(s.ev[3], e->stream); s.sort_timed = true; }
  s.pol.new_cycle(tile_order);
  return 0;
}

int k_compact(Engine *e, Species &s) { return s.n_holes > 0 ? k_sort_p(e, s, s.tile_valid) : 0; }

int k_species_reserve(Engine *e, Species &s, int64_t max_np, int64_t max_nm) {
  VH_CHECK(hipStreamSynchronize(e->stream));
  if (max_np > (1ll << 31) - 8192) VH_FAIL("a species holds at most 2^31 - 8192 particles");
  if (max_np > s.max_np) {
    ParticlesK bigger{};
    if (alloc_particles(bigger, max_np)) return 1;
    float *src[4] = {s.p.ux, s.p.uy, s.p.uz, s.p.q};
    float *dst[4] = {bigger.ux, bigger.uy, bigger.uz, bigger.q};
    if (s.np > 0) VH_CHECK(hipMemcpyAsync(bigger.r, s.p.r, sizeof(float4) * (size_t)s.np, hipMemcpyDeviceToDevice, e->stream));
    for (int a = 0; a < 4; a++) {
      if (s.np > 0) VH_CHECK(hipMemcpyAsync(dst[a], src[a], sizeof(float) * (size_t)s.np, hipMemcpyDeviceToDevice, e->stream));
    }
    VH_CHECK(hipStreamSynchronize(e->stream));
    free_particles(s.p);
    s.p = bigger;
// ... 834 lines not shown
```

### old-vpic_amd/csrc/policy.h

```cpp
#pragma once
#include <stdint.h>
#include <stdio.h>
#include <math.h>
#include <algorithm>

namespace vpichip {

constexpr int TILE_EDGE = 4;

enum PinnedWord { PW_CROSSERS = 0, PW_FULLEST_TILE, PW_SORT_CHECK, PW_MISSED, PW_CYCLE };

struct Policy {
  bool sorted_once = false;
  double t_sort = 0, t_sum = 0; int n_push = 0;
  double t_last = 0, growth_first = 0; int n_cycle = 0;
  double t_hist[2][32] = {{0}}; int n_hist[2] = {0, 0};
  double s_hist[2][33] = {{0}}; int sorted_after = 0;
  double c_hist[2][34] = {{0}}; double prev_sum = 0;
  bool coarse_order = false;
  double flavour_cost[2] = {0, 0}; int flavour_cycles = 0;
  float sort_push_ms[2] = {0, 0}; bool sp_last = true;
  float hint_push_ms = 0;
  bool wide_window = false;
  bool tile_unbalanced = false;
// ... 33 lines not shown
    s.t_last = ms;
    s.t_sum += ms; s.n_push++;
    const int n = s.n_push;
    const double t_next = ms + (growth > 0 ? growth : 0);
    const double sort_now = (n <= 32 && s_hist[n] > 0) ? s_hist[n] : s.t_sort;
    double sort_later = (n + 1 <= 32 && s_hist[n + 1] > 0) ? s_hist[n + 1] : sort_now;
    if (sort_later < sort_now) sort_later = sort_now;
    if ((s.n_cycle & 63) == 63) sort_later = sort_now;
    due = (sort_later + s.t_sum + t_next) * n >= (sort_now + s.t_sum) * (n + 1);
    if ((s.n_cycle & 63) == 63) for (int k = 0; k < 34; k++) c_hist[k] = 0;
    if (n <= 32 && c_hist[n] > 0 && c_hist[n + 1] > 0) due = c_hist[n] <= c_hist[n + 1];
    else if (!due && n <= 32 && c_hist[n] == 0 && (s.n_cycle & 7) == 7 && n == s.sorted_after - 1) due = true;
    if (debug) fprintf(stderr, "sort policy: n=%d T=%.3f T_next=%.3f S_now=%.3f S_later=%.3f sum=%.3f c[n]=%.3f c[n+1]=%.3f flavour %d (%.3f / %.3f per step) -> %s\n", n, ms, t_next, sort_now, sort_later, s.t_sum, n <= 32 ? c_hist[n] : 0.0, n <= 32 ? c_hist[n + 1] : 0.0, (int)coarse_sorted, s.flavour_cost[0], s.flavour_cost[1], due ? "sort" : "go on");
  }
  if (!s.sorted_once || (max_interval > 0 && s.n_push >= max_interval)) due = true;
  return due;
}

inline bool wants_tile_order(const Policy &s, int64_t np, int window, int min_axis, bool engine_choice) {
  if (np > ((int64_t)1 << 30)) return false;
  if (window == 't') return true;
  if (window == 'w' || window == 'n') return false;
  if (min_axis < TILE_EDGE) return false;
  if (s.tile_unbalanced && (s.n_cycle & 31) != 31) return false;
  return engine_choice;
}

inline bool sort_inside_push(Policy &s, bool debug) {
  if (s.sort_push_ms[1] == 0) s.sp_last = true;
  else if (s.sort_push_ms[0] == 0)
    s.sp_last = !((s.hint_push_ms > 0 && s.sort_push_ms[1] > 1.9f * s.hint_push_ms) || (s.n_cycle & 15) == 15);
  else { s.sp_last = s.sort_push_ms[1] <= s.sort_push_ms[0]; if ((s.n_cycle & 7) == 7) s.sp_last = !s.sp_last; }
  if (debug) fprintf(stderr, "sort and push: inside %.2f ms, before %.2f ms, the push that counted %.2f ms -> %s\n", (double)s.sort_push_ms[1], (double)s.sort_push_ms[0], (double)s.hint_push_ms, s.sp_last ? "inside" : "before");
  return s.sp_last;
}

inline bool early_sort(Policy &s, int64_t missed, unsigned cycle, int64_t left, int64_t ntiles, int64_t np) {
  if (cycle == (unsigned)s.n_cycle && left >= 2 && missed > 32ll * ntiles && missed * left * 27 > np) { s.early_sorts++; return true; }
  return false;
}

struct SortInputs {
  bool tile_order = false, may_fuse = false, adaptive = false, chargeless = false, has_tags = false, tile_valid = false, coarse_sorted = false;
  bool counts_ready = false, det_acc = false, time_kernels = false, old_sort = false; int tile_coarse = -1; int64_t np = 0, n_sorted = 0;
};
struct SortPlan { bool coarse = false, fuse = false, counted = false, by_wave = false, count_by_wave = false; };
inline SortPlan plan_sort(Policy &s, const SortInputs &in) {
  SortPlan pl;
  if (in.tile_order) {
    const bool eligible = in.np >= ((int64_t)8 << 20) && (s.cross_frac > 0.20 || (s.coarse_order && s.cross_frac > 0.15));
    if (!eligible) { s.coarse_order = false; s.flavour_cost[0] = s.flavour_cost[1] = 0; s.flavour_cycles = 0; }
    else if (!in.adaptive) s.coarse_order = true;
    else {
      const int cur = s.coarse_order ? 1 : 0, other = 1 - cur;
      bool change = false;
      if ((s.n_cycle & 127) == 127) s.flavour_cost[other] = 0;
      if (s.flavour_cycles >= 4 && s.flavour_cost[cur] > 0) {
        if (s.flavour_cost[other] == 0) change = true;
        else if (s.flavour_cost[other] < 0.97 * s.flavour_cost[cur]) change = true;
      }
      if (change) {
        s.coarse_order = !s.coarse_order; s.flavour_cycles = 0;
      }
    }
  }
  pl.coarse = in.tile_order && (s.coarse_order || in.chargeless);
  if (in.tile_order && in.tile_coarse >= 0) pl.coarse = in.tile_coarse != 0;
  pl.fuse = in.may_fuse && in.tile_order && !pl.coarse && in.tile_valid && !in.coarse_sorted && !s.tile_unbalanced && in.counts_ready &&
            !in.has_tags && !in.det_acc && !in.time_kernels && !in.old_sort && in.np <= ((int64_t)1 << 30) && in.np == in.n_sorted;
  pl.by_wave = in.old_sort;
  pl.count_by_wave = pl.by_wave || (!in.tile_order && s.cross_frac > 0.15);
  pl.counted = in.tile_order && !pl.coarse && in.counts_ready;
  return pl;
}

struct PushInputs {
  int phase = 0;
  int64_t np = 0, n_sorted = 0; double ppc = 0;
  unsigned crossers = 0, fullest_tile = 0;
  int window = 0, iters = 0, stage = -1; int64_t tail_sort_min = 0; bool no_tail_sort = false;
  int wx[2] = {0, 0}, wmargin = 0, threads = 0, max_iters = 0;
  bool tile_valid = false, chargeless = false, coarse_sorted = false, det_acc = false, time_kernels = false;
  bool fuse_pending = false, hist_request = false, hist_valid = false, fuse_buffers = false;
};
enum class PushInstance { chargeless, det_tile_only, det_tile, det_row, tile_only, tile_sort, tile_hist, tile, row_wide, row_narrow };
struct PushPlan {
  bool tiled = false, fuse = false, sort_first = false, regroup_tail = false, hist = false, det = false; int stage = 0;
  PushInstance instance = PushInstance::row_narrow;
};

inline int push_passes(Policy &s, const PushInputs &in) {
  if (in.phase != 2) {
    const double frac = s.np_pushed_last > 0 ? (double)in.crossers / (double)s.np_pushed_last : 0.0;
    s.cross_frac = frac;
    if (frac > 0.30) s.wide_window = true; else if (frac < 0.20) s.wide_window = false;
    if (in.window == 'w') s.wide_window = true; else if (in.window == 'n') s.wide_window = false;
    s.np_pushed_last = in.np;
  }
  const int wx = in.wx[s.wide_window ? 1 : 0];
  const int it = (int)(0.9 * (wx - 2 * in.wmargin) * in.ppc / in.threads);
  if (in.iters > 0) return in.iters;
  return it < 1 ? 1 : it > in.max_iters ? in.max_iters : it;
}

inline PushPlan plan_push(Policy &s, const PushInputs &in, int n_seg) {
  PushPlan pl;
  if (in.phase != 2 && in.tile_valid && (double)in.fullest_tile * 1280.0 > 4.0 * (double)in.np && in.fullest_tile > 65536u) s.tile_unbalanced = true;
  pl.tiled = in.phase == 2 ? true : (in.tile_valid && !s.tile_unbalanced && !in.chargeless && n_seg == 1);
  pl.stage = in.stage >= 0 ? in.stage : (s.cross_frac > 0.33 ? 1 : 0);
  pl.fuse = in.fuse_pending && pl.tiled && !in.coarse_sorted && in.phase == 0 && !in.det_acc && !in.hist_request && in.hist_valid &&
            in.fuse_buffers && in.np == in.n_sorted && !in.time_kernels;
  pl.sort_first = in.fuse_pending && !pl.fuse;
  const int64_t behind = in.np > in.n_sorted ? in.np - in.n_sorted : 0;
  pl.regroup_tail = pl.tiled && behind >= in.tail_sort_min && behind > 0 && !in.no_tail_sort;
  pl.hist = !pl.fuse && in.hist_request && pl.tiled && !in.coarse_sorted && in.phase == 0 && !(in.det_acc && !in.chargeless) &&
            (uint64_t)in.fullest_tile + (uint64_t)behind < 30000u;
  pl.det = in.det_acc && !in.chargeless;
  pl.instance = in.chargeless ? PushInstance::chargeless
              : pl.det ? (pl.tiled ? (in.coarse_sorted ? PushInstance::det_tile_only : PushInstance::det_tile) : PushInstance::det_row)
              : !pl.tiled ? (s.wide_window ? PushInstance::row_wide : PushInstance::row_narrow)
              : in.coarse_sorted ? PushInstance::tile_only : pl.fuse ? PushInstance::tile_sort : pl.hist ? PushInstance::tile_hist : PushInstance::tile;
  return pl;
}

inline long long chunk_for(long long n, long long waves) { return ((n + waves - 1) / waves + 63) / 64 * 64; }
struct Chunks { long long groups = 0, chunk = 0; };
inline Chunks plan_chunks(long long np, int waves_per_group) {
  Chunks c;
  const long long per_group = 64ll * waves_per_group * 16;
  c.groups = std::min(2048ll, (np + per_group - 1) / per_group);
  c.chunk = chunk_for(np, c.groups * waves_per_group);
  return c;
}

constexpr int SPEC_WIN_WORDS = 3072;
constexpr int SPEC_WIN_KEYS = 128;
inline int spectrum_window(int n_lin) {
  if (n_lin <= 0) return 0;
  const int win = SPEC_WIN_WORDS / n_lin;
  return win >= SPEC_WIN_KEYS ? SPEC_WIN_KEYS : win >= 64 ? 64 : 0;
}

constexpr int DIST_WIN_WORDS = 3072;
constexpr int DIST_WIN_SPARE_WORDS = 2048;
constexpr int DIST_WIN_SPARE = 3;
enum { DIST_LDS = 0, DIST_WINDOW = 1, DIST_GLOBAL = 2 };
struct DistPlan { int path = DIST_LDS, pos_axis = 0, win = 0, n_other = 1; };
inline DistPlan plan_distribution(int n_axes, const int n[2], const double d[2], const bool position[2], int lds_bins) {
  DistPlan pl;
  if ((long long)n[0] * n[1] <= lds_bins) return pl;
  pl.path = DIST_GLOBAL;
  int pa = -1;
  for (int a = n_axes - 1; a >= 0; a--) if (position[a]) pa = a;
  if (pa < 0) return pl;
  const int n_pos = n[pa], n_other = n[1 - pa];
  const double tile_bins = ceil((double)TILE_EDGE / d[pa]) + 1.0;
  if (!(tile_bins * n_other <= (double)DIST_WIN_WORDS)) return pl;
  int win = (int)tile_bins;
  if ((win + DIST_WIN_SPARE) * n_other <= DIST_WIN_SPARE_WORDS) win += DIST_WIN_SPARE;
  if (win > n_pos) win = n_pos;
  pl.path = DIST_WINDOW; pl.pos_axis = pa; pl.win = win; pl.n_other = n_other;
  return pl;
}

struct DistSumsPlan { int path = DIST_LDS; long long words = 0; };
inline DistSumsPlan plan_distribution_sums(long long bins, int n_val, int lds_words) {
  DistSumsPlan pl;
  const long long words = bins * (1 + 2 * (long long)n_val);
  if (words <= lds_words) pl.words = words; else pl.path = DIST_GLOBAL;
  return pl;
}

inline long long plan_cell_groups(long long cells, int per_group) {
  return std::max(1ll, std::min(2048ll, (cells + per_group - 1) / per_group));
}

constexpr long long DIST_ITEM_PARTICLES = 32768;
struct DistTilePlan {
  bool by_tile = false;
  int n_col = 0, members = 0, group = 0, groups_per_col = 0, items = 0, item_waves = 0;
  long long groups = 0, tail_chunk = 0, fallback_chunk = 0;
};
inline DistTilePlan plan_dist_tiles(int ntx, int nty, int ntz, int axis, bool usable, long long n_sorted, long long np, int waves_per_group) {
  DistTilePlan pl;
  if (!usable || n_sorted <= 0) return pl;
  const int ntiles = ntx * nty * ntz;
  pl.n_col = axis == 0 ? ntx : axis == 1 ? nty : ntz;
  pl.members = ntiles / pl.n_col;
  pl.group = std::min(pl.members, std::max(8, (ntiles + 8191) / 8192));
  while (pl.group > 1 && (long long)pl.n_col * ((pl.members + pl.group - 1) / pl.group) * DIST_ITEM_PARTICLES < n_sorted)
    pl.group = (pl.group + 1) / 2;
  pl.groups_per_col = (pl.members + pl.group - 1) / pl.group;
  pl.items = pl.n_col * pl.groups_per_col;
  if (!(pl.items >= 4096 || (long long)pl.items * DIST_ITEM_PARTICLES >= n_sorted)) return pl;
  pl.by_tile = true;
  const long long item_groups = (pl.items + waves_per_group - 1) / waves_per_group;
  pl.item_waves = (int)(item_groups * waves_per_group);
  const Chunks tail = np > n_sorted ? plan_chunks(np - n_sorted, waves_per_group) : Chunks();
  pl.tail_chunk = tail.chunk;
// ... 69 lines not shown
```

### old-vpic_amd/csrc/push.hip

```cpp
#include "push_device.h"
#include "record_offsets.h"
#include <cstdlib>
#include <cstring>
#include <cstddef>
#include <vector>
#include <algorithm>

namespace vpichip {

struct PushParams {
  float qdt_2mc, cdt_dx, cdt_dy, cdt_dz;
  int np;
  int iters;
  int sy, sz;
  int idx_base;
  unsigned *crossed;
  const int *tpart, *ttail; int ntx, nty, ntiles, n_sorted; unsigned mul_sy, sh_sy, mul_sz, sh_sz;
  const int *tile_list; int n_launch, tail_chunks;
  int nx, ny, nz;
  int follow;
  double acc_scale;
  int *hist; int ntz;
  ParticlesK out; int *next;
  int stage;
#ifdef VPIC_HIP_ABLATION
  int ablate;
#endif
};

#define SEG_STEP(v, flag, CTRL)                                                                   \
  asm volatile("v_fmac_f32_dpp %0, %0, %1 " CTRL : "+v"(v) : "v"(flag))
#define SEG_STEP12(a, flag, CTRL)                                                                 \
  do {                                                                                            \
    asm volatile("s_nop 1");                                                                      \
    SEG_STEP(a[0], flag, CTRL); SEG_STEP(a[1], flag, CTRL); SEG_STEP(a[2], flag, CTRL);           \
    SEG_STEP(a[3], flag, CTRL); SEG_STEP(a[4], flag, CTRL); SEG_STEP(a[5], flag, CTRL);           \
    SEG_STEP(a[6], flag, CTRL); SEG_STEP(a[7], flag, CTRL); SEG_STEP(a[8], flag, CTRL);           \
    SEG_STEP(a[9], flag, CTRL); SEG_STEP(a[10], flag, CTRL); SEG_STEP(a[11], flag, CTRL);         \
  } while (0)

typedef float rec4 __attribute__((ext_vector_type(4)));
__device__ __forceinline__ rec4 ldr(const float4 *base, unsigned off) { return *reinterpret_cast<const rec4 *>(reinterpret_cast<const char *>(base) + off); }
__device__ __forceinline__ void str(float4 *base, unsigned off, float x, float y, float z, int i) {
  rec4 v; v.x = x; v.y = y; v.z = z; v.w = __int_as_float(i);
  *reinterpret_cast<rec4 *>(reinterpret_cast<char *>(base) + off) = v;
}
__device__ __forceinline__ void str_nt(float4 *base, unsigned off, float x, float y, float z, int i) {
  rec4 v; v.x = x; v.y = y; v.z = z; v.w = __int_as_float(i);
  __builtin_nontemporal_store(v, reinterpret_cast<rec4 *>(reinterpret_cast<char *>(base) + off));
}
__device__ __forceinline__ rec4 *rec_at(float4 *base, unsigned dst) {
  return reinterpret_cast<rec4 *>(reinterpret_cast<char *>(base) + ((uint64_t)dst << RECORD_SHIFT));
}
__device__ __forceinline__ int ldcell(const float4 *base, unsigned off) { return __float_as_int(*reinterpret_cast<const float *>(reinterpret_cast<const char *>(base) + off + 12u)); }
__device__ __forceinline__ float ldf(const float *base, unsigned off) { return *reinterpret_cast<const float *>(reinterpret_cast<const char *>(base) + off); }
__device__ __forceinline__ void stf(float *base, unsigned off, float v) { *reinterpret_cast<float *>(reinterpret_cast<char *>(base) + off) = v; }
__device__ __forceinline__ void stf_nt(float *base, unsigned off, float v) { __builtin_nontemporal_store(v, reinterpret_cast<float *>(reinterpret_cast<char *>(base) + off)); }


__device__ __forceinline__ int in_vgpr(int s) { int v; asm volatile("v_mov_b32 %0, %1" : "=v"(v) : "s"(s)); return v; }

__device__ __forceinline__ int mbcnt64(unsigned long long m) {
  return (int)__builtin_amdgcn_mbcnt_hi((unsigned)(m >> 32), __builtin_amdgcn_mbcnt_lo((unsigned)m, 0u));
}

#ifndef VPIC_HIP_MAX_KEYS
#define VPIC_HIP_MAX_KEYS 12
#endif
constexpr int MAX_KEYS = VPIC_HIP_MAX_KEYS;

__device__ __forceinline__ int group_lanes_by_key(int key, int lane) {
  unsigned long long todo = ~0ull;
  int dest = lane, offset = 0;
  for (int it = 0; todo && it < MAX_KEYS; ++it) {
    const int lead = __ffsll((long long)todo) - 1;
    const int k0 = __builtin_amdgcn_readlane(key, lead);
    const bool mine = (key == k0);
    const unsigned long long m = __ballot(mine);
    if (mine) dest = offset + mbcnt64(m);
    offset += __popcll(m);
    todo &= ~m;
  }
  if ((todo >> lane) & 1ull) dest = offset + mbcnt64(todo);
  return dest;
}

constexpr int MISS_CAP = 5;
struct MissList { int key[MISS_CAP]; float v[MISS_CAP][12]; int total; };

__device__ __forceinline__ void flush_misses(MissList *ml, int &n_miss, float *g_acc, int lane) {
  if (n_miss > 0) {
    __builtin_amdgcn_fence(__ATOMIC_ACQ_REL, "workgroup");
    const int entry = lane / 12, k = lane - entry * 12;
    if (entry < n_miss) atomicAdd(g_acc + (size_t)ml->key[entry] * 12 + k, ml->v[entry][k]);
    if (lane == 0) ml->total += n_miss;
    __builtin_amdgcn_fence(__ATOMIC_ACQ_REL, "workgroup");
    n_miss = 0;
  }
}

struct HistK { int *hist; unsigned *s_cnt; TileK tk; };
template <class W>
__device__ __forceinline__ void hist_count(const HistK &h, int key, int wbase, int sy, int sz, const TileDiv &td) {
  const int slot = slot_of<W>(key, wbase, sy, sz, td);
  if (slot >= 0) atomicAdd(&h.s_cnt[slot >> 1], 1u << ((slot & 1) << 4));
  else atomicAdd(&h.hist[sort_key<true>(key, h.tk)], 1);
}

template <class W>
__device__ __forceinline__ void deposit_run(const bool tail, float (&a)[12], int key, int lane, typename W::acc_t *s_acc, float *g_acc,
                                            int wbase, int sy, int sz, const TileDiv &td, MissList *ml, int &n_miss, const int pre_slot = -2) {
  const int slot = pre_slot != -2 ? pre_slot : slot_of<W>(key, wbase, sy, sz, td);
  if constexpr (is_det<W>::value) {
    if (tail) deposit12<true, W>(s_acc, g_acc, key, slot, a, td.scale);
    return;
  }
  if (tail && slot >= 0) deposit12<true, W>(s_acc, g_acc, key, slot, a);
  const bool miss = tail && slot < 0;
  const unsigned long long mm = __ballot(miss);
  if (mm) {
    if (miss) moments_to_terms(a, a);
    const int cnt = __popcll(mm);
    if (cnt > MISS_CAP) {
      if (miss) deposit12<true, W>(s_acc, g_acc, key, -1, a);
      if (lane == 0) ml->total += cnt;
      } else {
      if (n_miss + cnt > MISS_CAP) flush_misses(ml, n_miss, g_acc, lane);
      if (miss) {
        const int e = n_miss + mbcnt64(mm);
        ml->key[e] = key;
#pragma unroll
        for (int k = 0; k < 12; k++) ml->v[e][k] = a[k];
      }
      n_miss += cnt;
    }
  }
}

template <int BLOCK, class W>
__device__ __forceinline__ void run_deposit(float (&a)[12], int key, int lane, typename W::acc_t *s_acc, float *g_acc,
                                            int wbase, int sy, int sz, const TileDiv &td, MissList *ml, int &n_miss,
                                            const HistK *hk = nullptr, const bool counted = false, const int given_slot = -2) {
  static_assert(BLOCK == 1 || BLOCK == 2 || BLOCK == 4 || BLOCK == 8 || BLOCK == 16 || BLOCK == 64, "scan width");
  if (BLOCK == 1) {
    deposit_run<W>(key >= 0, a, key, lane, s_acc, g_acc, wbase, sy, sz, td, ml, n_miss);
    return;
  }
  const int prev = __builtin_amdgcn_update_dpp(-2, key, 0x138 , 0xf, 0xf, false);
  const unsigned long long block_heads = BLOCK == 64 ? 0ull : BLOCK == 16 ? 0x0001000100010001ull : BLOCK == 8 ? 0x0101010101010101ull
                                       : BLOCK == 4 ? 0x1111111111111111ull : 0x5555555555555555ull;
  const unsigned long long heads = __ballot(prev != key) | block_heads;
  const unsigned long long below = heads & ((2ull << lane) - 1ull);
  const int d = lane - (63 - __clzll((long long)below));
  const float f1 = d >= 1 ? 1.f : 0.f;
  SEG_STEP12(a, f1, "row_shr:1 row_mask:0xf bank_mask:0xf bound_ctrl:1");
  if (BLOCK >= 4) {
    const float f2 = d >= 2 ? 1.f : 0.f;
    SEG_STEP12(a, f2, "row_shr:2 row_mask:0xf bank_mask:0xf bound_ctrl:1");
  }
  if (BLOCK >= 8) {
    const float f4 = d >= 4 ? 1.f : 0.f;
    SEG_STEP12(a, f4, "row_shr:4 row_mask:0xf bank_mask:0xf bound_ctrl:1");
  }
  if (BLOCK >= 16) {
    const float f8 = d >= 8 ? 1.f : 0.f;
    SEG_STEP12(a, f8, "row_shr:8 row_mask:0xf bank_mask:0xf bound_ctrl:1");
  }
  if (BLOCK == 64) {
    const int r = lane & 15;
    const float f16 = d > r ? 1.f : 0.f;
    const float f32 = d > (lane & 31) ? 1.f : 0.f;
    SEG_STEP12(a, f16, "row_bcast:15 row_mask:0xa bank_mask:0xf");
    SEG_STEP12(a, f32, "row_bcast:31 row_mask:0xc bank_mask:0xf");
  }
  asm volatile("s_nop 1");
  const bool tail = (lane == 63) || ((heads >> ((lane + 1) & 63)) & 1ull);
  if (hk) {
    const int slot = slot_of<W>(key, wbase, sy, sz, td);
    const unsigned long long inc = __ballot(counted);
    const unsigned long long run = ((2ull << lane) - 1ull) & ~((1ull << (lane - d)) - 1ull);
    const int n = __popcll(inc & run);
    if (tail && key >= 0 && n) {
      if (slot >= 0) atomicAdd(&hk->s_cnt[slot >> 1], (unsigned)n << ((slot & 1) << 4));
      else atomicAdd(&hk->hist[sort_key<true>(key, hk->tk)], n);
    }
    deposit_run<W>(tail && key >= 0, a, key, lane, s_acc, g_acc, wbase, sy, sz, td, ml, n_miss, slot);
    return;
  }
  deposit_run<W>(tail && key >= 0, a, key, lane, s_acc, g_acc, wbase, sy, sz, td, ml, n_miss, given_slot);
}

template <int BLOCK, class W>
__device__ __forceinline__ void run_deposit_fixed(const float (&a)[12], int key, int lane, typename W::acc_t *s_acc, float *g_acc,
                                                  int wbase, int sy, int sz, const TileDiv &td, MissList *ml, int &n_miss) {
  static_assert(BLOCK == 16, "runs of at most 16 lanes, within a DPP row");
  unsigned long long v[12];
#pragma unroll
  for (int k = 0; k < 12; k++) v[k] = to_fixed(a[k], td.scale);
  const int prev = __builtin_amdgcn_update_dpp(-2, key, 0x138 , 0xf, 0xf, false);
  const unsigned long long heads = __ballot(prev != key) | 0x0001000100010001ull;
  const unsigned long long below = heads & ((2ull << lane) - 1ull);
  const int d = lane - (63 - __clzll((long long)below));
#pragma unroll
  for (int step = 1; step < 16; step <<= 1) {
    const bool on = d >= step;
#pragma unroll
    for (int k = 0; k < 12; k++) {
      const int lo = (int)(unsigned)v[k], hi = (int)(unsigned)(v[k] >> 32);
      const int tl = step == 1 ? __builtin_amdgcn_update_dpp(0, lo, 0x111 , 0xf, 0xf, true)
                   : step == 2 ? __builtin_amdgcn_update_dpp(0, lo, 0x112, 0xf, 0xf, true)
                   : step == 4 ? __builtin_amdgcn_update_dpp(0, lo, 0x114, 0xf, 0xf, true)
                               : __builtin_amdgcn_update_dpp(0, lo, 0x118, 0xf, 0xf, true);
      const int th = step == 1 ? __builtin_amdgcn_update_dpp(0, hi, 0x111, 0xf, 0xf, true)
                   : step == 2 ? __builtin_amdgcn_update_dpp(0, hi, 0x112, 0xf, 0xf, true)
                   : step == 4 ? __builtin_amdgcn_update_dpp(0, hi, 0x114, 0xf, 0xf, true)
                               : __builtin_amdgcn_update_dpp(0, hi, 0x118, 0xf, 0xf, true);
      const unsigned long long t = ((unsigned long long)(unsigned)th << 32) | (unsigned long long)(unsigned)tl;
      v[k] += on ? t : 0ull;
    }
  }
  const bool tail = key >= 0 && ((lane == 63) || ((heads >> ((lane + 1) & 63)) & 1ull));
  if (tail) {
    const int slot = slot_of<W>(key, wbase, sy, sz, td);
    unsigned long long *g64 = reinterpret_cast<unsigned long long *>(g_acc) + (size_t)key * 12;
#pragma unroll
    for (int k = 0; k < 12; k++) {
      if (slot >= 0) atomicAdd(&s_acc[k * W::NSLOT_PAD + slot], v[k]); else atomicAdd(&g64[k], v[k]);
    }
  }
  asm volatile("" ::: "memory");
}

constexpr int WAVES = PUSH_THREADS / 64;

#ifndef VPIC_HIP_MQW
#define VPIC_HIP_MQW 64
#endif
static_assert(VPIC_HIP_MQW >= 64, "a pass can yield 64 cell-crossers: the queue must hold them once it has been drained");
constexpr int MQW = VPIC_HIP_MQW;
struct WaveQueue { float4 pos_i[MQW]; float4 disp_idx[MQW]; float q[MQW]; };
constexpr int FLIP_SHIFT = 28;

__device__ __forceinline__ float fast_rsq(float x) { return __builtin_amdgcn_rsqf(x); }
__device__ __forceinline__ float fast_rcp(float x) { return __builtin_amdgcn_rcpf(x); }

template <class W>
__device__ __forceinline__ void mover_streak12(float *a, float q, float mx, float my, float mz, float sx, float sy, float sz) {
  if constexpr (is_det<W>::value) {
    const float v5 = (float)((double)(q * sx * sy * sz) * (1. / 3.));
    streak12(a, q, mx, my, mz, sx, sy, sz, v5);
  } else {
    streak12_moments(a, q, mx, my, mz, sx, sy, sz);
  }
}

constexpr int STAGE_CAP = 2;
template <bool CHARGELESS> struct StageRounds { static constexpr int value = CHARGELESS ? 2 : 1; };
struct StagePark { int base[STAGE_CAP], qb[STAGE_CAP]; unsigned cm_lo[STAGE_CAP], cm_hi[STAGE_CAP], act_lo[STAGE_CAP], act_hi[STAGE_CAP]; };
constexpr int STAGED_BIT = 31;
struct Straggler { float4 pos_i, disp_idx; float q; bool live; unsigned long long again; };

template <bool FAST, class W, bool HIST = false, bool STAGE = false, bool WIDE = false>
__device__ __forceinline__ int drain_wave(const ParticlesK &p, const int rel, WaveQueue *mq, const int n_mq,
                                          const int lane, typename W::acc_t *s_acc, float *g_acc, const int wbase,
                                          const DrainParams *dp, const int ablate, const int max_round, const int idx_base,
                                          MissList *ml, int &n_miss, const double det_scale = 0, const HistK *hk = nullptr, Straggler *sg = nullptr) {
  if (ablate & 64) return 0;
// ... 68 lines not shown
      const bool wall = live && moved_on && edge && wcode;
      const bool refl = wall && rcode, stop = wall && !rcode;
      const bool hop = live && moved_on && !wall;
      if (live) {
        m.dispx -= s_dispx; m.dispy -= s_dispy; m.dispz -= s_dispz;
        dx += s_dispx + s_dispx; dy += s_dispy + s_dispy; dz += s_dispz + s_dispz;
        const float dir = ty0 ? s_dir0 : ty1 ? s_dir1 : s_dir2;
        const float face = hop ? -dir : dir;
        dx = ty0 ? face : dx; dy = ty1 ? face : dy; dz = ty2 ? face : dz;
        const int sgn = hi ? 1 : -1;
        const int nm1 = ty0 ? gnx - 1 : ty1 ? gny - 1 : gnz - 1;
        const int stride = ty0 ? 1 : ty1 ? gsy : gsz;
        const int dc = hop ? (edge ? -sgn * nm1 : sgn) : 0;
        pi += dc * stride;
        cx += ty0 ? dc : 0; cy += ty1 ? dc : 0; cz += ty2 ? dc : 0;
      }
      if (__ballot(refl)) {
        if (refl && ty0) { flips ^= 1; m.dispx = -m.dispx; }
        if (refl && ty1) { flips ^= 2; m.dispy = -m.dispy; }
        if (refl && ty2) { flips ^= 4; m.dispz = -m.dispz; }
      }
      stuck = stuck || stop;
      live = hop || refl;
      if (ablate & 32) {}
      else run_deposit<W::DRAIN_BLOCK, W>(a, key, lane, s_acc, g_acc, wbase, gsy, gsz, td, ml, n_miss);
      {
        const float n0 = ((m.dispx > 0) ? 1.f : -1.f) - dx, n1 = ((m.dispy > 0) ? 1.f : -1.f) - dy, n2 = ((m.dispz > 0) ? 1.f : -1.f) - dz;
        const float d0 = m.dispx + m.dispx, d1 = m.dispy + m.dispy, d2 = m.dispz + m.dispz;
        const bool h0 = (m.dispx > 0) ? (n0 < d0) : (m.dispx < 0) ? (n0 > d0) : false;
        const bool h1 = (m.dispy > 0) ? (n1 < d1) : (m.dispy < 0) ? (n1 > d1) : false;
        const bool h2 = (m.dispz > 0) ? (n2 < d2) : (m.dispz < 0) ? (n2 > d2) : false;
        const bool fin = live && !(h0 || h1 || h2);
        if (__ballot(fin)) {
          float b[12];
          mover_streak12<W>(b, q, dx + m.dispx, dy + m.dispy, dz + m.dispz, m.dispx, m.dispy, m.dispz);
          const int fkey = fin ? pi : -1;
          if (fin) {
            dx += m.dispx + m.dispx; dy += m.dispy + m.dispy; dz += m.dispz + m.dispz;
            live = false;
          }
          if (ablate & 32) {}
          else run_deposit<W::DRAIN_BLOCK, W>(b, fkey, lane, s_acc, g_acc, wbase, gsy, gsz, td, ml, n_miss);
        }
      }
    }
    const unsigned long long again = __ballot(live);
    if (STAGE) {
      sg->live = live; sg->again = again; sg->q = q;
      sg->pos_i = make_float4(dx, dy, dz, __int_as_float(pi | (flips << FLIP_SHIFT)));
      sg->disp_idx = make_float4(m.dispx, m.dispy, m.dispz, __int_as_float(idx));
      if (staged) mq->pos_i[k] = make_float4(dx, dy, dz, __int_as_float(live ? -1 : pi));
    } else
    if (live) {
      const int d = mbcnt64(again);
      mq->pos_i[d] = make_float4(dx, dy, dz, __int_as_float(pi | (flips << FLIP_SHIFT)));
      mq->disp_idx[d] = make_float4(m.dispx, m.dispy, m.dispz, __int_as_float(idx));
      mq->q[d] = q;
    }
    n_again = __popcll(again);
    if (mine && !live) {
#ifdef VPIC_HIP_ABLATION
      if (ablate & 256) {} else
#endif
      if (!staged) {
        if (WIDE) { rec4 v; v.x = dx; v.y = dy; v.z = dz; v.w = __int_as_float(pi); __builtin_nontemporal_store(v, rec_at(p.r, (unsigned)idx)); }
        else str_nt(p.r, o4 << 2, dx, dy, dz, pi);
      }
      if (HIST) hist_count<W>(*hk, pi, wbase, gsy, gsz, td);
      if (flips) {
        asm volatile("s_waitcnt vmcnt(0)" ::: "memory");
        if (flips & 1) stf(p.ux, o4, -ldf(p.ux, o4));
        if (flips & 2) stf(p.uy, o4, -ldf(p.uy, o4));
        if (flips & 4) stf(p.uz, o4, -ldf(p.uz, o4));
      }
      if (stuck) {
        const int gs = __hip_atomic_fetch_add(nm_counter, 1, __ATOMIC_RELAXED, __HIP_MEMORY_SCOPE_AGENT);
        if (gs < max_nm) { pm[gs].dispx = m.dispx; pm[gs].dispy = m.dispy; pm[gs].dispz = m.dispz; pm[gs].i = m.i + idx_base; }
      }
    }
  }
  return n_again;
}

constexpr int TAIL_CHUNK = 1024;

template <bool CHARGELESS = false, bool FAST = false, int WIN = 0, bool HIST = false, bool SORT = false>
#ifndef VPIC_HIP_PUSH_VGPRS
#define VPIC_HIP_PUSH_VGPRS 80
#endif
__global__ __launch_bounds__(PUSH_THREADS) __attribute__((amdgpu_num_vgpr(VPIC_HIP_PUSH_VGPRS)))
void advance_p_kernel(ParticlesK p, const float4 *__restrict__ fi, float *__restrict__ g_acc,
                      const DrainParams *__restrict__ dp, const PushParams P) {
  typedef Window<WIN> W;
  typedef typename W::acc_t acc_t;
  constexpr bool TILE = W::TILE;
  constexpr bool DET = is_det<W>::value;
  constexpr bool UNORDERED = WIN == 3 || WIN == 5 || WIN == 6;
  constexpr int WX = W::WX, NSLOT_PAD = W::NSLOT_PAD;
  __shared__ acc_t s_acc[12 * NSLOT_PAD];
  __shared__ WaveQueue s_mq[WAVES];
  __shared__ MissList s_miss[WAVES];
  __shared__ int s_wbase;
  __shared__ unsigned s_cnt[HIST ? (NSLOT_PAD + 1) / 2 : SORT ? NSLOT_PAD : 1];
  constexpr bool STAGE = (WIN == 3 || CHARGELESS) && !HIST && !SORT;
  __shared__ StagePark s_park[STAGE ? WAVES : 1];
  static_assert(!HIST || WIN == 2, "the histogram of the next sort is taken in tile order, by cell");
  static_assert(!SORT || (WIN == 2 && !HIST && !CHARGELESS), "the sort inside the push: tile order by cell, its counts taken by the push before");

#ifdef VPIC_HIP_ABLATION
  const int ablate = P.ablate | (CHARGELESS ? (1 | 8 | 16 | 32) : 0);
#else
  constexpr int ablate = CHARGELESS ? (1 | 8 | 16 | 32) : 0;
#endif
  const int tid = threadIdx.x;
  const int lane = tid & 63;
  const int wave = __builtin_amdgcn_readfirstlane(tid >> 6);
  const unsigned chunk = xcd_block(blockIdx.x, gridDim.x);
  int first, last, wave_span = 0, tile_base = NO_WINDOW;
  int first2 = 0, last2 = 0;
  int bx0 = 0, by0 = 0, bz0 = 0;
  if (TILE) {
    if (chunk < (unsigned)P.n_launch) {
      const unsigned tile = P.tile_list ? (unsigned)P.tile_list[chunk] : chunk;
      first = min(P.tpart[tile * TILE_CELLS], P.np);
      last = min(P.tpart[tile * TILE_CELLS + TILE_CELLS], P.np);
      if (P.ttail) {
        first2 = min(P.n_sorted + P.ttail[tile * TILE_CELLS], P.np);
        last2 = min(P.n_sorted + P.ttail[tile * TILE_CELLS + TILE_CELLS], P.np);
      }
      const unsigned txy = tile % (unsigned)(P.ntx * P.nty), tz = tile / (unsigned)(P.ntx * P.nty);
      const unsigned tx = txy % (unsigned)P.ntx, ty = txy / (unsigned)P.ntx;
      tile_base = TILE_EDGE * ((int)tx + P.sy * (int)ty + P.sz * (int)tz);
      bx0 = TILE_EDGE * (int)tx; by0 = TILE_EDGE * (int)ty; bz0 = TILE_EDGE * (int)tz;
    } else {
      if (chunk - (unsigned)P.n_launch >= (unsigned)P.tail_chunks) return;
      first = min(P.n_sorted, P.np) + (int)(chunk - (unsigned)P.n_launch) * TAIL_CHUNK;
      last = min(first + TAIL_CHUNK, P.np);
    }
    if (first >= last && first2 >= last2) return;
  } else {
    wave_span = 64 * P.iters;
    if ((long long)chunk * (WAVES * wave_span) >= P.np) return;
    first = (int)chunk * (WAVES * wave_span);
    last = P.np;
  }

#ifndef VPIC_HIP_FOLLOW
#define VPIC_HIP_FOLLOW 1
#endif
  constexpr int FOLLOW_REACH = 3;
  int sample = -1;
  bool follow = false;
  if (TILE && VPIC_HIP_FOLLOW && tile_base != NO_WINDOW) {
    unsigned flag = 0;
    if (P.follow < 0) asm volatile("s_load_dword %0, %1, 0x8\n\ts_waitcnt lgkmcnt(0)" : "=s"(flag) : "s"(P.crossed));
    follow = P.follow > 0 || flag == 1u;
  }
  if (follow && wave == 0 && last > first)
    sample = record_cell(p.r, (long long)first + (int)(((long long)lane * (last - first)) >> 6));
  if (!CHARGELESS)
    for (int k = tid; k < 12 * NSLOT_PAD; k += PUSH_THREADS) s_acc[k] = 0;
  if (HIST)
    for (int k = tid; k < (NSLOT_PAD + 1) / 2; k += PUSH_THREADS) s_cnt[k] = 0;
  if (SORT)
    for (int k = tid; k < NSLOT_PAD; k += PUSH_THREADS) s_cnt[k] = 0;
  if (TILE) {
    if (follow) {
      if (wave == 0) {
        const bool have = sample >= 0;
        const int cz = (int)(__umulhi((unsigned)max(sample, 0), P.mul_sz) >> P.sh_sz), rem = max(sample, 0) - cz * P.sz;
        const int cy = (int)(__umulhi((unsigned)rem, P.mul_sy) >> P.sh_sy), cx = rem - cy * P.sy;
        int best[3];
#pragma unroll
        for (int a = 0; a < 3; a++) {
          const int c = a == 0 ? cx : a == 1 ? cy : cz, b0 = a == 0 ? bx0 : a == 1 ? by0 : bz0, n = a == 0 ? P.nx : a == 1 ? P.ny : P.nz;
          const int hi = max(n - 4, 0);
          int pick = min(max(b0, 0), hi), top = -1;
#pragma unroll
          for (int t = 0; t < 2 * FOLLOW_REACH + 1; t++) {
            const int d = (t & 1) ? -((t + 1) >> 1) : (t >> 1);
            const int b = min(max(b0 + d, 0), hi);
            const int cover = __popcll(__ballot(have && c >= b && c <= b + 5)), inner = __popcll(__ballot(have && c > b && c < b + 5));
            const int score = 2 * cover + inner;
            if (score > top) { top = score; pick = b; }
          }
          best[a] = pick;
        }
        if (lane == 0) s_wbase = best[0] + P.sy * best[1] + P.sz * best[2];
      }
    } else if (tid == 0) s_wbase = tile_base;
  } else if (DET) {
    if (tid == 0) s_wbase = NO_WINDOW;
  } else if (!CHARGELESS && wave == 0) {
    const int chunk_n = min(WAVES * wave_span, P.np - first);
    const int sidx = first + (int)(((long long)lane * chunk_n) >> 6);
    const int k0 = record_cell(p.r, sidx);
    int rank = 0;
    for (int l = 0; l < 64; l++) {
      const int kl = __builtin_amdgcn_readlane(k0, l);
      rank += (kl < k0 || (kl == k0 && l < lane)) ? 1 : 0;
    }
    const unsigned long long is_med = __ballot(rank == 31);
    const int m = __builtin_amdgcn_readlane(k0, __ffsll((long long)is_med) - 1) - WX / 2 + WMARGIN;
    if (lane == 0) s_wbase = m - WMARGIN;
  }
  __syncthreads();
  const int wbase = s_wbase;
  const int gsy = P.sy, gsz = P.sz;
  WaveQueue *mq = &s_mq[wave];
  MissList *ml = &s_miss[wave];
  if (lane == 0) ml->total = 0;
  int n_miss = 0;
  int n_mq = 0, n_crossed = 0;

  TileDiv td = {0u, 0u, 0u, 0u, 0.0};
  if (TILE) { td.mul_sy = P.mul_sy; td.sh_sy = P.sh_sy; td.mul_sz = P.mul_sz; td.sh_sz = P.sh_sz; }
  if (DET) td.scale = P.acc_scale;
  TileDiv vtd = td;
  int vsy = gsy, vsz = gsz;
  if (TILE && !DET) {
    vtd.mul_sy = (unsigned)in_vgpr((int)P.mul_sy); vtd.sh_sy = (unsigned)in_vgpr((int)P.sh_sy);
    vtd.mul_sz = (unsigned)in_vgpr((int)P.mul_sz); vtd.sh_sz = (unsigned)in_vgpr((int)P.sh_sz);
    vsy = in_vgpr(gsy); vsz = in_vgpr(gsz);
  }
  HistK hk;
  if (HIST || SORT) {
    hk.hist = P.hist; hk.s_cnt = s_cnt;
    hk.tk.sy = P.sy; hk.tk.sz = P.sz; hk.tk.ntx = P.ntx; hk.tk.nty = P.nty; hk.tk.ntz = P.ntz; hk.tk.ntiles = P.ntiles;
    hk.tk.mul_sy = P.mul_sy; hk.tk.sh_sy = P.sh_sy; hk.tk.mul_sz = P.mul_sz; hk.tk.sh_sz = P.sh_sz;
    hk.tk.mx = P.nx - 1; hk.tk.my = P.ny - 1; hk.tk.mz = P.nz - 1;
  }

  float st0x = 0.f, st0y = 0.f, st0z = 0.f, st1x = 0.f, st1y = 0.f, st1z = 0.f;
  int st0i = 0, st1i = 0;
  int n_pend = 0;
  const bool stage = STAGE && P.stage != 0;
  StagePark *park = &s_park[STAGE ? wave : 0];
  ParticlesK pw = p;
  int rel = 0;
  auto drain_release = [&](const bool all) -> int {
    Straggler sg; sg.live = false; sg.again = 0ull;
    int n_back = 0;
    if (n_mq > 0) {
      __builtin_amdgcn_fence(__ATOMIC_RELEASE, "workgroup");
      n_back = drain_wave<FAST, W, HIST, STAGE>(pw, rel, mq, n_mq, lane, s_acc, g_acc, wbase, dp, ablate, all ? (1 << 30) : StageRounds<CHARGELESS>::value, P.idx_base, ml, n_miss, td.scale, &hk, &sg);
      __builtin_amdgcn_fence(__ATOMIC_ACQ_REL, "workgroup");
    }
#pragma unroll
    for (int j = 0; j < STAGE_CAP; j++) {
      if (j >= n_pend) break;
      const int pb = __builtin_amdgcn_readfirstlane(park->base[j]), qb = __builtin_amdgcn_readfirstlane(park->qb[j]);
      const unsigned long long cmj = ((unsigned long long)(unsigned)__builtin_amdgcn_readfirstlane((int)park->cm_hi[j]) << 32) | (unsigned)__builtin_amdgcn_readfirstlane((int)park->cm_lo[j]);
      const unsigned long long actj = ((unsigned long long)(unsigned)__builtin_amdgcn_readfirstlane((int)park->act_hi[j]) << 32) | (unsigned)__builtin_amdgcn_readfirstlane((int)park->act_lo[j]);
      float fx = j ? st1x : st0x, fy = j ? st1y : st0y, fz = j ? st1z : st0z;
      int fi_ = j ? st1i : st0i;
      const bool cr = (cmj >> lane) & 1ull;
      if (cr) {
        const float4 r = mq->pos_i[qb + mbcnt64(cmj)];
        const int newi = __float_as_int(r.w);
        if (newi >= 0) { fx = r.x; fy = r.y; fz = r.z; fi_ = newi; }
      }
      if ((actj >> lane) & 1ull) str(pw.r, record_offset(pb + lane, rel), fx, fy, fz, fi_);
    }
    n_pend = 0;
    __builtin_amdgcn_fence(__ATOMIC_ACQ_REL, "workgroup");
    if (sg.live) {
      const int d = mbcnt64(sg.again);
      mq->pos_i[d] = sg.pos_i; mq->disp_idx[d] = sg.disp_idx; mq->q[d] = sg.q;
    }
    return n_back;
  };
  const float one = 1.f, one_third = 1. / 3., two_fifteenths = 2. / 15.;
  const float qdt_2mc = P.qdt_2mc, cdt_dx = P.cdt_dx, cdt_dy = P.cdt_dy, cdt_dz = P.cdt_dz;

  if (SORT) {
    typedef __attribute__((address_space(1))) int *global_int_ptr;
#pragma unroll 1
    for (int seg = 0; seg < 2; seg++) {
      const int sfirst = seg ? first2 : first, slast = seg ? last2 : last;
      constexpr int AHEAD = 8;
#pragma unroll 1
      for (int base = sfirst + wave * 64; base < slast; base += AHEAD * PUSH_THREADS) {
        int keys[AHEAD];
        const float4 *const recs = p.r + sfirst;
#pragma unroll
        for (int j = 0; j < AHEAD; j++) { const int at = base + j * PUSH_THREADS + lane; keys[j] = at < slast ? ldcell(recs, record_offset(at, sfirst)) : -1; }
#pragma unroll
        for (int j = 0; j < AHEAD; j++) {
          const int key = keys[j];
          const int slot = key >= 0 ? slot_of<W>(key, wbase, vsy, vsz, vtd) : -1;
          const int kprev = __builtin_amdgcn_update_dpp(-2, key, 0x138 , 0xf, 0xf, false);
          const unsigned long long heads = __ballot(kprev != key);
          const unsigned long long above = heads & ~((2ull << lane) - 1ull);
          const int run_end = above ? __ffsll((long long)above) - 1 : 64;
          if (((heads >> lane) & 1ull) && slot >= 0) atomicAdd(&s_cnt[slot], (unsigned)(run_end - lane));
        }
      }
    }
    __syncthreads();
    for (int t = tid; t < W::NSLOT; t += PUSH_THREADS) {
      const unsigned c = s_cnt[t];
      if (c) {
        const int lx = t % WX, lyz = t / WX, ly = lyz % WX, lz = lyz / WX;
        s_cnt[t] = (unsigned)__hip_atomic_fetch_add((global_int_ptr)P.next + sort_key<true>(wbase + lx + gsy * ly + gsz * lz, hk.tk), (int)c,
                                                    __ATOMIC_RELAXED, __HIP_MEMORY_SCOPE_AGENT);
      }
    }
    __syncthreads();
  }

#pragma unroll 1
  for (int seg = 0; seg < (TILE ? 2 : 1); seg++) {
  const int sfirst = seg ? first2 : first, slast = seg ? last2 : last;
  if (TILE && sfirst >= slast) continue;
  const int sspan = TILE ? ((slast - sfirst + 64 * WAVES - 1) / (64 * WAVES)) * 64 : wave_span;
  const int wave_passes = TILE ? sspan >> 6 : P.iters;
  constexpr int PASS_STRIDE = 64;
  const int wave_first = sfirst + wave * sspan;
  const int wave_last = TILE ? min(slast, wave_first + sspan) : slast;
  if (TILE && !SORT && seg && (n_mq > 0 || (STAGE && n_pend > 0))) {
    __builtin_amdgcn_fence(__ATOMIC_RELEASE, "workgroup");
    if constexpr (STAGE) n_mq = drain_release(true);
    else n_mq = drain_wave<FAST, W, HIST>(pw, rel, mq, n_mq, lane, s_acc, g_acc, wbase, dp, ablate, 1 << 30, P.idx_base, ml, n_miss, td.scale, &hk);
    __builtin_amdgcn_fence(__ATOMIC_ACQ_REL, "workgroup");
  }
  pw = offset_particles(p, sfirst);
  rel = SORT ? 0 : sfirst;
  const int vrel_max = TILE ? in_vgpr(P.np - 1 - sfirst) : P.np - 1 - sfirst;
  rec4 r_rec;
  float r_ux, r_uy, r_uz, r_q;
  {
    const unsigned k4 = (unsigned)min(wave_first - sfirst + lane, P.np - 1 - sfirst) << 2;
    r_rec = ldr(pw.r, k4 << 2);
    r_ux = ldf(pw.ux, k4); r_uy = ldf(pw.uy, k4); r_uz = ldf(pw.uz, k4); r_q = ldf(pw.q, k4);
  }

#pragma unroll 1
  for (int it = 0; it < wave_passes; it++) {
    const int base = wave_first + it * PASS_STRIDE;
    if (base >= wave_last) break;
    int idx = base + lane, key = (base + lane < wave_last) ? __float_as_int(r_rec.w) : -1;
    float dx = r_rec.x, dy = r_rec.y, dz = r_rec.z, ux = r_ux, uy = r_uy, uz = r_uz, q = r_q;
    const int kk = key < 0 ? 0x7fffffff : key;
    const int kprev = __builtin_amdgcn_update_dpp((int)0x80000000, kk, 0x138 , 0xf, 0xf, false);
    if (!UNORDERED && !(ablate & 16) && __ballot(kk < kprev)) {
      const int dest = group_lanes_by_key(key, lane);
      if (__ballot(dest != lane)) {
        const int a4 = dest << 2;
        idx = base + __builtin_amdgcn_ds_permute(a4, lane);
        key = __builtin_amdgcn_ds_permute(a4, key);
        dx = __int_as_float(__builtin_amdgcn_ds_permute(a4, __float_as_int(dx)));
        dy = __int_as_float(__builtin_amdgcn_ds_permute(a4, __float_as_int(dy)));
        dz = __int_as_float(__builtin_amdgcn_ds_permute(a4, __float_as_int(dz)));
        ux = __int_as_float(__builtin_amdgcn_ds_permute(a4, __float_as_int(ux)));
        uy = __int_as_float(__builtin_amdgcn_ds_permute(a4, __float_as_int(uy)));
        uz = __int_as_float(__builtin_amdgcn_ds_permute(a4, __float_as_int(uz)));
        q = __int_as_float(__builtin_amdgcn_ds_permute(a4, __float_as_int(q)));
      }
    }
    int dst = idx, sort_slot = -2, sort_b = 0, sort_head = 0;
    if (SORT) {
      typedef __attribute__((address_space(1))) int *global_int_ptr;
      const int slot = key >= 0 ? slot_of<W>(key, wbase, vsy, vsz, vtd) : -1;
      sort_slot = slot;
      const int kprev2 = __builtin_amdgcn_update_dpp(-2, key, 0x138 , 0xf, 0xf, false);
      const unsigned long long heads = __ballot(kprev2 != key);
      const unsigned long long upto = (2ull << lane) - 1ull;
      const int head = 63 - __clzll((long long)(heads & upto));
      const unsigned long long above = heads & ~upto;
      const int run_end = above ? __ffsll((long long)above) - 1 : 64;
      const bool reserves = lane == head && key >= 0;
      int b = 0;
      if (reserves && slot >= 0) b = (int)atomicAdd(&s_cnt[slot], (unsigned)(run_end - lane));
      if (__ballot(reserves && slot < 0)) {
        if (reserves && slot < 0)
          b = __hip_atomic_fetch_add((global_int_ptr)P.next + sort_key<true>(key, hk.tk), run_end - lane, __ATOMIC_RELAXED, __HIP_MEMORY_SCOPE_AGENT);
      }
      sort_b = b; sort_head = head;
    }
    const float4 *f = reinterpret_cast<const float4 *>(reinterpret_cast<const char *>(fi) + (unsigned)((ablate & 4) ? 0 : max(key, 0)) * 80u);
    const float4 fe_x = f[0], fe_y = f[1], fe_z = f[2], fb0 = f[3];
    const float2 fb1 = *reinterpret_cast<const float2 *>(f + 4);
    __builtin_amdgcn_sched_barrier(0);
    {
      const int k = base - sfirst + ((it + 1 < wave_passes) ? PASS_STRIDE : 0) + lane;
      const unsigned k4 = (unsigned)min(k, vrel_max) << 2;
      r_rec = ldr(pw.r, k4 << 2);
      r_ux = ldf(pw.ux, k4); r_uy = ldf(pw.uy, k4); r_uz = ldf(pw.uz, k4); r_q = ldf(pw.q, k4);
    }
    __builtin_amdgcn_sched_barrier(0);
    const bool active = key >= 0;
    float a[12];
    bool crosser;
    float sux, suy, suz;
    float spx = 0.f, spy = 0.f, spz = 0.f;
    {
      const unsigned o4 = word_offset(idx, sfirst);
      float v0, v1, v2, v3, v4, v5;
      if (FAST) {
        const float hax = qdt_2mc * __builtin_fmaf(dz, __builtin_fmaf(dy, fe_x.w, fe_x.z), __builtin_fmaf(dy, fe_x.y, fe_x.x));
        const float hay = qdt_2mc * __builtin_fmaf(dx, __builtin_fmaf(dz, fe_y.w, fe_y.z), __builtin_fmaf(dz, fe_y.y, fe_y.x));
        const float haz = qdt_2mc * __builtin_fmaf(dy, __builtin_fmaf(dx, fe_z.w, fe_z.z), __builtin_fmaf(dx, fe_z.y, fe_z.x));
        const float cbx = __builtin_fmaf(dx, fb0.y, fb0.x), cby = __builtin_fmaf(dy, fb0.w, fb0.z), cbz = __builtin_fmaf(dz, fb1.y, fb1.x);
        ux += hax; uy += hay; uz += haz;
        v0 = qdt_2mc * fast_rsq(__builtin_fmaf(ux, ux, __builtin_fmaf(uy, uy, __builtin_fmaf(uz, uz, one))));
        v1 = __builtin_fmaf(cbx, cbx, __builtin_fmaf(cby, cby, cbz * cbz));
        v2 = (v0 * v0) * v1;
        v3 = v0 * __builtin_fmaf(v2, __builtin_fmaf(v2, two_fifteenths, one_third), one);
        v4 = (v3 + v3) * fast_rcp(__builtin_fmaf(v1, v3 * v3, one));
        v0 = __builtin_fmaf(v3, __builtin_fmaf(uy, cbz, -(uz * cby)), ux);
        v1 = __builtin_fmaf(v3, __builtin_fmaf(uz, cbx, -(ux * cbz)), uy);
        v2 = __builtin_fmaf(v3, __builtin_fmaf(ux, cby, -(uy * cbx)), uz);
        ux = __builtin_fmaf(v4, __builtin_fmaf(v1, cbz, -(v2 * cby)), ux);
        uy = __builtin_fmaf(v4, __builtin_fmaf(v2, cbx, -(v0 * cbz)), uy);
        uz = __builtin_fmaf(v4, __builtin_fmaf(v0, cby, -(v1 * cbx)), uz);
        ux += hax; uy += hay; uz += haz;
      } else {
        const float hax = qdt_2mc * ((fe_x.x + dy * fe_x.y) + dz * (fe_x.z + dy * fe_x.w));
        const float hay = qdt_2mc * ((fe_y.x + dz * fe_y.y) + dx * (fe_y.z + dz * fe_y.w));
        const float haz = qdt_2mc * ((fe_z.x + dx * fe_z.y) + dy * (fe_z.z + dx * fe_z.w));
        const float cbx = fb0.x + dx * fb0.y;
        const float cby = fb0.z + dy * fb0.w;
        const float cbz = fb1.x + dz * fb1.y;
        ux += hax; uy += hay; uz += haz;
        v0 = div_normal(qdt_2mc, sqrt_normal(one + (ux * ux + (uy * uy + uz * uz))));
        v1 = cbx * cbx + (cby * cby + cbz * cbz);
        v2 = (v0 * v0) * v1;
        v3 = v0 * (one + v2 * (one_third + v2 * two_fifteenths));
        v4 = div_normal(v3, one + v1 * (v3 * v3));
        v4 += v4;
        v0 = ux + v3 * (uy * cbz - uz * cby);
        v1 = uy + v3 * (uz * cbx - ux * cbz);
        v2 = uz + v3 * (ux * cby - uy * cbx);
        ux += v4 * (v1 * cbz - v2 * cby);
        uy += v4 * (v2 * cbx - v0 * cbz);
        uz += v4 * (v0 * cby - v1 * cbx);
        ux += hax; uy += hay; uz += haz;
      }
      sux = ux; suy = uy; suz = uz;
      if (FAST) v0 = fast_rsq(__builtin_fmaf(ux, ux, __builtin_fmaf(uy, uy, __builtin_fmaf(uz, uz, one))));
      else v0 = div_normal(one, sqrt_normal(one + (ux * ux + (uy * uy + uz * uz))));
      ux *= cdt_dx; uy *= cdt_dy; uz *= cdt_dz;
      ux *= v0; uy *= v0; uz *= v0;
      v0 = dx + ux; v1 = dy + uy; v2 = dz + uz;
      v3 = v0 + ux; v4 = v1 + uy; v5 = v2 + uz;
      const bool incell = (ablate & 2) || fmaxf(fmaxf(fabsf(v3), fabsf(v4)), fabsf(v5)) <= one;
      crosser = active && !incell;
      if (SORT) {
        dst = __shfl(sort_b, sort_head) + (lane - sort_head);
        if (active) {
          const unsigned d4 = (unsigned)dst << 2;
          stf(P.out.ux, d4, sux); stf(P.out.uy, d4, suy); stf(P.out.uz, d4, suz);
          rec4 v; v.x = incell ? v3 : dx; v.y = incell ? v4 : dy; v.z = incell ? v5 : dz; v.w = __int_as_float(key);
          *rec_at(P.out.r, (unsigned)dst) = v;
          stf(P.out.q, d4, q);
        }
      } else
      if (STAGE && stage) {
        if (!TILE || active) { stf(pw.ux, o4, sux); stf(pw.uy, o4, suy); stf(pw.uz, o4, suz); }
        spx = incell ? v3 : dx; spy = incell ? v4 : dy; spz = incell ? v5 : dz;
      } else
      if ((!TILE || active) && !(ablate & 128)) {
        stf_nt(pw.ux, o4, sux); stf_nt(pw.uy, o4, suy); stf_nt(pw.uz, o4, suz);
        str(pw.r, o4 << 2, incell ? v3 : dx, incell ? v4 : dy, incell ? v5 : dz, key);
      }
      if (!CHARGELESS && !(ablate & 1)) {
        const float qd = (incell && active) ? q : 0.f;
// ... 5 lines not shown
      }
    }
    if constexpr (WIN == 4) run_deposit_fixed<16, W>(a, key, lane, s_acc, g_acc, wbase, gsy, gsz, td, ml, n_miss);
    else
    if (!CHARGELESS) run_deposit<UNORDERED ? 1 : TILE ? TILE_MAIN_BLOCK : MAIN_BLOCK, W>(a, (UNORDERED && crosser) ? -1 : key, lane, s_acc, g_acc, wbase, vsy, vsz, vtd, ml, n_miss,
                                                                                            HIST ? &hk : nullptr, active && !crosser, SORT ? sort_slot : -2);
    {
      const unsigned long long cm = __ballot(crosser);
      const int cnt = __popcll(cm);
      n_crossed += cnt;
      if constexpr (STAGE) {
        int phase = (n_mq + cnt > MQW) ? 0 : 1, attempt = 0;
#pragma unroll 1
        for (;;) {
          if (phase == 1) {
            if (crosser) {
              const int d = n_mq + mbcnt64(cm);
              mq->pos_i[d] = make_float4(dx, dy, dz, __int_as_float(stage ? (key | (1 << STAGED_BIT)) : key));
              mq->disp_idx[d] = make_float4(ux, uy, uz, __int_as_float(idx));
              mq->q[d] = q;
            }
            if (stage) {
              if (n_pend == 0) { st0x = spx; st0y = spy; st0z = spz; st0i = key; } else { st1x = spx; st1y = spy; st1z = spz; st1i = key; }
              const unsigned long long act = __ballot(!TILE || active);
              if (lane == 0) {
                park->base[n_pend] = base; park->qb[n_pend] = n_mq;
                park->cm_lo[n_pend] = (unsigned)cm; park->cm_hi[n_pend] = (unsigned)(cm >> 32);
                park->act_lo[n_pend] = (unsigned)act; park->act_hi[n_pend] = (unsigned)(act >> 32);
              }
              n_pend++;
            }
            n_mq += cnt;
            if (n_mq < 64 && n_pend < STAGE_CAP) break;
          }
          n_mq = drain_release(phase == 0 && attempt > 0);
          if (phase == 1) break;
          attempt++;
          if (n_mq + cnt <= MQW) phase = 1;
        }
      } else {
      int attempt = 0;
#pragma unroll 1
      for (int phase = (n_mq + cnt > MQW) ? 0 : 1; phase < 2;) {
        if (phase == 1) {
          if (crosser) {
            const int d = n_mq + mbcnt64(cm);
            mq->pos_i[d] = make_float4(dx, dy, dz, __int_as_float(key));
            mq->disp_idx[d] = make_float4(ux, uy, uz, __int_as_float(SORT ? dst : idx));
            mq->q[d] = q;
          }
          n_mq += cnt;
          if (n_mq < 64) break;
        }
        const int n_now = min(n_mq, 64);
        __builtin_amdgcn_fence(__ATOMIC_RELEASE, "workgroup");
        const int cap = (phase == 0 && attempt > 0) ? (1 << 30) : 1;
        const int n_back = drain_wave<FAST, W, HIST, false, SORT>(SORT ? P.out : pw, rel, mq, n_now, lane, s_acc, g_acc, wbase, dp, ablate, cap, P.idx_base, ml, n_miss, td.scale, &hk);
            const int n_left = n_mq - n_now;
        const int src = lane < n_left ? 64 + lane : 0;
        const float4 t0 = mq->pos_i[src], t2 = mq->disp_idx[src];
        const float t1 = mq->q[src];
        __builtin_amdgcn_fence(__ATOMIC_ACQ_REL, "workgroup");
        if (lane < n_left) { const int d = n_back + lane; mq->pos_i[d] = t0; mq->disp_idx[d] = t2; mq->q[d] = t1; }
        n_mq = n_back + n_left;
        if (phase == 0) { attempt++; if (n_mq + cnt <= MQW) phase = 1; }
        else phase = 2;
      }
      }
    }
  }
  }
  __builtin_amdgcn_fence(__ATOMIC_RELEASE, "workgroup");
  if constexpr (STAGE) n_mq = drain_release(true);
  else
  drain_wave<FAST, W, HIST, false, SORT>(SORT ? P.out : pw, rel, mq, n_mq, lane, s_acc, g_acc, wbase, dp, ablate, 1 << 30, P.idx_base, ml, n_miss, td.scale, &hk);
  if (!CHARGELESS && !DET) flush_misses(ml, n_miss, g_acc, lane);

  if (lane == 0 && n_crossed) atomicAdd(P.crossed + (blockIdx.x & 255u) * 16u, (unsigned)n_crossed);
  if (!CHARGELESS && lane == 0 && ml->total) atomicAdd(P.crossed + (blockIdx.x & 255u) * 16u + 1u, (unsigned)ml->total);

  __syncthreads();
  if (ablate & 8) return;
  if (HIST && wbase != NO_WINDOW) {
    for (int slot = tid; slot < W::NSLOT; slot += PUSH_THREADS) {
      const unsigned n = (s_cnt[slot >> 1] >> ((slot & 1) << 4)) & 0xffffu;
      const int lx = slot % WX, lyz = slot / WX, ly = lyz % WX, lz = lyz / WX;
      if (n) atomicAdd(&P.hist[sort_key<true>(wbase + lx + gsy * ly + gsz * lz, hk.tk)], (int)n);
    }
  }
  const int k = tid % 12, c0 = tid / 12;
  if constexpr (DET) {
    if (TILE && wbase != NO_WINDOW && tid < 12 * FLUSH_CELLS) {
      unsigned long long *g64 = reinterpret_cast<unsigned long long *>(g_acc);
      for (int cell = c0; cell < W::NSLOT; cell += FLUSH_CELLS) {
        const unsigned long long v = (unsigned long long)s_acc[k * NSLOT_PAD + cell];
        const int lx = cell % WX, lyz = cell / WX, ly = lyz % WX, lz = lyz / WX;
        if (v) atomicAdd(g64 + (size_t)(wbase + lx + gsy * ly + gsz * lz) * 12 + k, v);
      }
    }
  } else if constexpr (TILE) {
    if (wbase != NO_WINDOW && tid < 12 * FLUSH_CELLS) {
      const TermSigns sg = term_signs(k & 3);
      const acc_t *src = s_acc + (k & ~3) * NSLOT_PAD;
      for (int cell = c0; cell < W::NSLOT; cell += FLUSH_CELLS) {
        const float v = (float)term_of(sg, src[cell], src[NSLOT_PAD + cell], src[2 * NSLOT_PAD + cell], src[3 * NSLOT_PAD + cell]);
        const int lx = cell % WX, lyz = cell / WX, ly = lyz % WX, lz = lyz / WX;
        if (v != 0.f) atomicAdd(g_acc + (size_t)(wbase + lx + gsy * ly + gsz * lz) * 12 + k, v);
      }
    }
  } else if (tid < 12 * FLUSH_CELLS) {
    const TermSigns sg = term_signs(k & 3);
#pragma unroll
    for (int s = 0; s < NSEG; s++) {
      const int seg_base = wbase + ((s == 0) ? 0 : (s == 1) ? gsy : (s == 2) ? -gsy : (s == 3) ? gsz : -gsz);
      const acc_t *src = s_acc + (k & ~3) * NSLOT_PAD + s * WX;
      float *dst = g_acc + (size_t)seg_base * 12 + k;
      for (int cell = c0; cell < WX; cell += FLUSH_CELLS) {
        const float v = (float)term_of(sg, src[cell], src[NSLOT_PAD + cell], src[2 * NSLOT_PAD + cell], src[3 * NSLOT_PAD + cell]);
        if (v != 0.f) atomicAdd(dst + cell * 12, v);
      }
    }
  }
}

__global__ __launch_bounds__(256) void publish_counter_kernel(unsigned *__restrict__ host_word, unsigned *__restrict__ dev_shards, unsigned cycle, unsigned long long follow_from) {
  __shared__ unsigned s_sum[4];
  unsigned v = dev_shards[threadIdx.x * 16];
  dev_shards[threadIdx.x * 16] = 0;
  for (int off = 32; off; off >>= 1) v += __shfl_down(v, off);
  if ((threadIdx.x & 63) == 0) s_sum[threadIdx.x >> 6] = v;
  __syncthreads();
  if (threadIdx.x == 0) host_word[0] = s_sum[0] + s_sum[1] + s_sum[2] + s_sum[3];
  __syncthreads();
  v = dev_shards[threadIdx.x * 16 + 1];
  dev_shards[threadIdx.x * 16 + 1] = 0;
  for (int off = 32; off; off >>= 1) v += __shfl_down(v, off);
  if ((threadIdx.x & 63) == 0) s_sum[threadIdx.x >> 6] = v;
  __syncthreads();
  if (threadIdx.x == 0) {
    const unsigned missed = s_sum[0] + s_sum[1] + s_sum[2] + s_sum[3];
    host_word[3] = missed; host_word[4] = cycle;
    const unsigned state = dev_shards[2];
    if (state == 0u && (unsigned long long)missed > follow_from) dev_shards[2] = 1u;
    else if (state == 1u && (unsigned long long)missed > 4ull * follow_from) dev_shards[2] = 2u;
  }
}

__global__ __launch_bounds__(256) void fuse_check_kernel(const int *__restrict__ cursor, const int *__restrict__ starts, int n1, unsigned *__restrict__ bad) {
  const int k = blockIdx.x * 256 + threadIdx.x;
  const bool wrong = k + 1 < n1 && cursor[k] != starts[k + 1];
  const unsigned long long m = __ballot(wrong);
  if (m && (threadIdx.x & 63) == 0) atomicAdd(bad, (unsigned)__popcll(m));
}

__global__ void fuse_clear_kernel(unsigned *__restrict__ w) { *w = 0; }
__global__ void fuse_publish_kernel(unsigned *__restrict__ host_word, const unsigned *__restrict__ dev_word) { *host_word = *dev_word; }

int k_sort_check(Engine *e, Species &s, const int *starts, int n1) {
  unsigned *word = reinterpret_cast<unsigned *>(e->counters + 201);
  hipLaunchKernelGGL(fuse_clear_kernel, dim3(1), dim3(1), 0, e->stream, word);
  hipLaunchKernelGGL(fuse_check_kernel, dim3((n1 + 255) / 256), dim3(256), 0, e->stream, (const int *)e->sort_next, starts, n1, word);
  hipLaunchKernelGGL(fuse_publish_kernel, dim3(1), dim3(1), 0, e->stream, s.crossed_host_dev + PW_SORT_CHECK, (const unsigned *)word);
  VH_CHECK(hipGetLastError());
  return 0;
}

static int begin_profile(Engine *e, int64_t particles, int kind = 0, int species = -1) {
  if (!e->profile) return -1;
  if (e->ev_used == e->ev_pool.size()) {
    hipEvent_t a, b;
    if (hipEventCreate(&a) != hipSuccess || hipEventCreate(&b) != hipSuccess) return -1;
    e->ev_pool.push_back({a, b});
    e->ev_particles.push_back(0); e->ev_kind.push_back(0); e->ev_species.push_back(-1);
  }
  const int k = (int)e->ev_used++;
  e->ev_particles[k] = particles; e->ev_kind[k] = (char)kind; e->ev_species[k] = species;
  (void)hipEventRecord(e->ev_pool[k].first, e->stream);
  return k;
}

extern "C" int vpic_hip_push_plan(int64_t np, int iters, int64_t *start, int32_t *count, uint32_t *grid, int max_segments) {
  if (np < 0 || iters < 1 || iters > PUSH_ITERS || max_segments < 1) return -1;
  const int64_t per_chunk = (int64_t)PUSH_THREADS * iters;
  int64_t seg = push_segment_particles(per_chunk);
  if (np <= ((int64_t)1 << 30) && (np % 64 == 0 || np <= ((int64_t)1 << 30) - 64)) seg = (np + per_chunk - 1) / per_chunk * per_chunk;
  int n = 0;
  for (int64_t at = 0; at < np; at += seg, n++) {
    if (n >= max_segments) return -1;
    const int64_t c = np - at < seg ? np - at : seg;
    start[n] = at; count[n] = (int32_t)c;
    const uint32_t chunks = (uint32_t)((c + per_chunk - 1) / per_chunk);
    grid[n] = (chunks + 7u) & ~7u;
  }
  return n;
}

static int ensure_tile_lists(Engine *e) {
  if (e->tile_list[0] || e->tile_list_n[0] < 0) return 0;
  const TileK tk = make_tile_k(e->gk);
  bool shared[6]; bool any = false;
  for (int f = 0; f < 6; f++) { shared[f] = e->gk.pbc[f] >= 0 && e->gk.pbc[f] != e->gk.rank; any = any || shared[f]; }
  if (!any) { e->tile_list_n[0] = -1; return 0; }
  std::vector<int> list[2];
  for (int tz = 0; tz < tk.ntz; tz++) for (int ty = 0; ty < tk.nty; ty++) for (int tx = 0; tx < tk.ntx; tx++) {
    const bool edge = (shared[0] && tx == 0) || (shared[3] && tx == tk.ntx - 1) || (shared[1] && ty == 0) || (shared[4] && ty == tk.nty - 1) ||
                      (shared[2] && tz == 0) || (shared[5] && tz == tk.ntz - 1);
    list[edge ? 0 : 1].push_back((tz * tk.nty + ty) * tk.ntx + tx);
  }
  for (int k = 0; k < 2; k++) {
    VH_CHECK(hipMalloc(&e->tile_list[k], sizeof(int) * std::max<size_t>(list[k].size(), 1)));
    if (!list[k].empty()) VH_CHECK(hipMemcpy(e->tile_list[k], list[k].data(), sizeof(int) * list[k].size(), hipMemcpyHostToDevice));
    e->tile_list_n[k] = (int)list[k].size();
  }
  return 0;
}

template <bool CHARGELESS, int WIN = 0, bool HIST = false, bool SORT = false>
static void launch_push(bool fast, unsigned grid, hipStream_t stream, const ParticlesK &p, const float4 *fi, float *g_acc, DrainParams *d, const PushParams &P) {
  if (fast) hipLaunchKernelGGL((advance_p_kernel<CHARGELESS, true, WIN, HIST, SORT>), dim3(grid), dim3(PUSH_THREADS), 0, stream, p, fi, g_acc, d, P);
  else hipLaunchKernelGGL((advance_p_kernel<CHARGELESS, false, WIN, HIST, SORT>), dim3(grid), dim3(PUSH_THREADS), 0, stream, p, fi, g_acc, d, P);
}

int k_advance_p(Engine *e, Species &s, bool async, int phase) {
  const vpic_hip_grid_t &g = e->grid;
  PushParams P;
  P.qdt_2mc = (float)(0.5 * s.q_m * g.dt / g.cvac);
  P.cdt_dx = g.cvac * g.dt * g.rdx;
  P.cdt_dy = g.cvac * g.dt * g.rdy;
  P.cdt_dz = g.cvac * g.dt * g.rdz;
  P.np = (int)s.np;
  P.sy = e->gk.sy; P.sz = e->gk.sz;
#ifdef VPIC_HIP_ABLATION
  P.ablate = e->knobs.ablate;
#endif
  const unsigned *pinned = s.crossed_host;
  if (pinned[PW_SORT_CHECK]) VH_FAIL("advance_p: %u keys of the species' last sort did not receive the particles the push before it had counted for them", pinned[PW_SORT_CHECK]);
  if (phase == 2 && !s.phase_pending) return 0;
  if (phase != 2) {
    VH_CHECK(hipMemsetAsync(s.nm_dev, 0, sizeof(int), e->stream));
    s.nm = 0;
  }
  s.phase_pending = false;
  P.crossed = s.crossed_dev;
  if (s.np > 0) {
    PushInputs in;
    in.phase = phase; in.np = s.np; in.n_sorted = s.n_sorted; in.ppc = (double)s.np / ((double)e->gk.nx * e->gk.ny * e->gk.nz);
    in.crossers = pinned[PW_CROSSERS]; in.fullest_tile = pinned[PW_FULLEST_TILE];
    in.window = e->knobs.window; in.iters = e->knobs.iters; in.stage = e->knobs.stage;
    in.tail_sort_min = e->knobs.tail_sort_min; in.no_tail_sort = e->knobs.no_tail_sort;
    in.wx[0] = Window<false>::WX; in.wx[1] = Window<true>::WX; in.wmargin = WMARGIN; in.threads = PUSH_THREADS; in.max_iters = PUSH_ITERS;
    in.tile_valid = s.tile_valid; in.chargeless = s.chargeless; in.coarse_sorted = s.coarse_sorted; in.det_acc = e->det_acc; in.time_kernels = e->time_kernels;
    in.fuse_pending = s.fuse_pending; in.hist_request = s.hist_request; in.hist_valid = s.hist_valid; in.fuse_buffers = s.aux.r && s.tpart2;
    P.iters = push_passes(s.pol, in);
    int64_t seg_start[4]; int32_t seg_count[4]; uint32_t seg_grid[4];
    const int n_seg = vpic_hip_push_plan(s.np, P.iters, seg_start, seg_count, seg_grid, 4);
    if (n_seg < 1) VH_FAIL("advance_p: cannot plan %lld particles", (long long)s.np);
    if (e->time_kernels && phase != 2) { if (!s.ev[0]) for (int i = 0; i < 4; i++) VH_CHECK(hipEventCreate(&s.ev[i])); (void)hipEventRecord(s.ev[0], e->stream); }
    const PushPlan pl = plan_push(s.pol, in, n_seg);
    const bool tiled = pl.tiled, fuse = pl.fuse, hist = pl.hist, det = pl.det;
    P.tpart = s.tpart; P.ttail = nullptr; P.n_sorted = (int)s.n_sorted;
    P.tile_list = nullptr; P.n_launch = 0; P.tail_chunks = 0;
    P.nx = e->gk.nx; P.ny = e->gk.ny; P.nz = e->gk.nz;
    P.follow = e->knobs.follow;
    P.stage = pl.stage;
    s.fuse_pending = false;
    if (pl.sort_first) {
      if (k_sort_p(e, s, true, false)) return 1;
      return k_advance_p(e, s, async, phase);
    }
    if (phase && tiled && ensure_tile_lists(e)) return 1;
    const bool split = phase && tiled && e->tile_list_n[0] > 0 && e->tile_list_n[1] > 0;
    if (phase == 2 && !split) VH_FAIL("advance_p: phase 2 without phase 1");
    if (tiled) {
      const TileK tk = make_tile_k(e->gk);
      P.ntx = tk.ntx; P.nty = tk.nty; P.ntiles = tk.ntiles;
      P.mul_sy = tk.mul_sy; P.sh_sy = tk.sh_sy; P.mul_sz = tk.mul_sz; P.sh_sz = tk.sh_sz;
      const int64_t behind = s.np > s.n_sorted ? s.np - s.n_sorted : 0;
      if (!span_in_reach(0, behind)) VH_FAIL("advance_p: %lld particles appended since the last sort; sort the species first", (long long)behind);
      if (phase != 2 && pl.regroup_tail && k_tail_sort(e, s)) return 1;
      if (phase != 2) s.tail_regrouped = pl.regroup_tail && s.tail_sorted;
      P.ttail = s.tail_regrouped ? s.ttail : nullptr;
      P.n_launch = split ? e->tile_list_n[phase - 1] : tk.ntiles;
      P.tile_list = split ? e->tile_list[phase - 1] : nullptr;
      P.tail_chunks = (P.ttail || phase == 2) ? 0 : (int)((behind + TAIL_CHUNK - 1) / TAIL_CHUNK);
      seg_grid[0] = (uint32_t)(((int64_t)P.n_launch + P.tail_chunks + 7) / 8 * 8);
      s.phase_pending = split && phase == 1;
    }
    const int ev = begin_profile(e, phase == 2 ? -1 : s.np, fuse ? 1 : 0, (int)(&s - e->species.data()));
    if (fuse) {
      const TileK tk = make_tile_k(e->gk);
      if (k_sort_scan(e, s.hist, s.tpart2, tk.ntiles * TILE_CELLS + 1)) return 1;
      P.out = s.aux; P.next = e->sort_next;
    } else { P.out = ParticlesK{}; P.next = nullptr; }
    s.hist_request = false; s.hist_valid = false;
    if (hist) {
      const TileK tk = make_tile_k(e->gk);
      const int64_t n1 = (int64_t)tk.ntiles * TILE_CELLS + 1;
      if (s.hist_count < n1) { if (s.hist) VH_CHECK(hipFree(s.hist)); s.hist = nullptr; VH_CHECK(hipMalloc(&s.hist, sizeof(int) * n1)); s.hist_count = n1; }
      VH_CHECK(hipMemsetAsync(s.hist, 0, sizeof(int) * n1, e->stream));
      P.hist = s.hist; P.ntz = tk.ntz;
    } else { P.hist = nullptr; P.ntz = fuse ? make_tile_k(e->gk).ntz : 0; }
    if (det && acc_prepare_det(e)) return 1;
    P.acc_scale = e->acc_scale;
    float *const g_acc = det ? reinterpret_cast<float *>(e->acc64) : reinterpret_cast<float *>(e->acc);
#define PUSH_LAUNCH(...) launch_push<__VA_ARGS__>(e->push_fast, seg_grid[g], e->stream, ps, reinterpret_cast<const float4 *>(e->fi), g_acc, s.drain_k, P); break
    for (int g = 0; g < n_seg; g++) {
      const int64_t at = seg_start[g];
      const ParticlesK ps = offset_particles(s.p, at);
      P.np = seg_count[g]; P.idx_base = (int)at;
      switch (pl.instance) {
        case PushInstance::chargeless: PUSH_LAUNCH(true);
        case PushInstance::det_tile_only: PUSH_LAUNCH(false, 6);
        case PushInstance::det_tile: PUSH_LAUNCH(false, 4);
        case PushInstance::det_row: PUSH_LAUNCH(false, 5);
        case PushInstance::tile_only: PUSH_LAUNCH(false, 3);
        case PushInstance::tile_sort: PUSH_LAUNCH(false, 2, false, true);
        case PushInstance::tile_hist: PUSH_LAUNCH(false, 2, true);
        case PushInstance::tile: PUSH_LAUNCH(false, 2);
        case PushInstance::row_wide: PUSH_LAUNCH(false, 1);
        case PushInstance::row_narrow: PUSH_LAUNCH(false, 0);
      }
    }
#undef PUSH_LAUNCH
    if (ev >= 0) (void)hipEventRecord(e->ev_pool[ev].second, e->stream);
    if (hist) s.hist_valid = true;
    if (fuse) {
      const TileK tk = make_tile_k(e->gk);
      const int n1 = tk.ntiles * TILE_CELLS + 1;
      if (k_sort_check(e, s, s.tpart2, n1)) return 1;
      std::swap(s.tpart, s.tpart2); std::swap(s.tpart_count, s.tpart2_count);
      if (k_sort_finish(e, s, true, false)) return 1;
    }
    if (!s.phase_pending) {
      hipLaunchKernelGGL(publish_counter_kernel, dim3(1), dim3(256), 0, e->stream, s.crossed_host_dev, s.crossed_dev, (unsigned)(s.pol.n_cycle - (fuse ? 1 : 0)),
                         fuse ? ~0ull : (unsigned long long)e->knobs.follow_from * (unsigned long long)make_tile_k(e->gk).ntiles);
      if (e->time_kernels) { (void)hipEventRecord(s.ev[1], e->stream); s.push_timed = true; }
    }
    VH_CHECK(hipGetLastError());
  }
  if (!e->can_strand || async) { s.partition_valid = false; return 0; }
  VH_CHECK(hipMemcpyAsync(e->host_counters, s.nm_dev, sizeof(int), hipMemcpyDeviceToHost, e->stream));
  VH_CHECK(hipStreamSynchronize(e->stream));
  int64_t nm = e->host_counters[0];
  if (nm > s.max_nm) {
    fprintf(stderr, "vpic_hip: advance_p ran out of storage for %lld movers\n", (long long)(nm - s.max_nm));
    nm = s.max_nm;
  }
  s.nm = nm;
  s.partition_valid = false;
  return 0;
}

__global__ __launch_bounds__(256)
void energy_p_kernel(ParticlesK p, const float4 *__restrict__ fi, double *__restrict__ partial,
                     float qdt_2mc, int np) {
  __shared__ double s_sum[4];
  double en = 0;
  const float one = 1.f;
  for (long long idx = (long long)blockIdx.x * 256 + threadIdx.x; idx < np; idx += (long long)gridDim.x * 256) {
    const float4 rec = p.r[idx];
    if (record_cell(rec) < 0) continue;
    const float dx = rec.x, dy = rec.y, dz = rec.z;
    const float4 *f = fi + (size_t)record_cell(rec) * 5;
    const float4 fe_x = f[0], fe_y = f[1], fe_z = f[2];
    float v0 = p.ux[idx] + qdt_2mc * ((fe_x.x + dy * fe_x.y) + dz * (fe_x.z + dy * fe_x.w));
    float v1 = p.uy[idx] + qdt_2mc * ((fe_y.x + dz * fe_y.y) + dx * (fe_y.z + dz * fe_y.w));
    float v2 = p.uz[idx] + qdt_2mc * ((fe_z.x + dx * fe_z.y) + dy * (fe_z.z + dx * fe_z.w));
    v0 = v0 * v0 + v1 * v1 + v2 * v2;
    v0 /= sqrtf(one + v0) + one;
    en += (double)v0 * (double)p.q[idx];
  }
  for (int off = 32; off; off >>= 1) en += __shfl_down(en, off);
  if ((threadIdx.x & 63) == 0) s_sum[threadIdx.x >> 6] = en;
  __syncthreads();
  if (threadIdx.x == 0) partial[blockIdx.x] = (s_sum[0] + s_sum[1]) + (s_sum[2] + s_sum[3]);
}

int k_energy_p(Engine *e, Species &s, double *energy) {
  const vpic_hip_grid_t &g = e->grid;
  const float qdt_2mc = (float)(0.5 * s.q_m * g.dt / g.cvac);
  const int nb = (int)e->dsum_count;
  hipLaunchKernelGGL(energy_p_kernel, dim3(nb), dim3(256), 0, e->stream, s.p,
                     reinterpret_cast<const float4 *>(e->fi), e->dsum, qdt_2mc, (int)s.np);
  VH_CHECK(hipGetLastError());
  VH_CHECK(hipMemcpyAsync(e->host_dsum, e->dsum, sizeof(double) * nb, hipMemcpyDeviceToHost, e->stream));
  VH_CHECK(hipStreamSynchronize(e->stream));
  double sum = 0;
  for (int k = 0; k < nb; k++) sum += e->host_dsum[k];
  *energy = (double)g.cvac * (double)g.cvac * sum / (double)s.q_m;
  return 0;
}

}

namespace vpichip {
template <bool UNCENTER>
__global__ __launch_bounds__(256)
void center_p_kernel(ParticlesK p, const float4 *__restrict__ fi, float args_qdt_2mc, int np) {
  const int idx = blockIdx.x * 256 + threadIdx.x;
  if (idx >= np) return;
  const float4 rec = p.r[idx];
  if (record_cell(rec) < 0) return;
  const float qdt_2mc = UNCENTER ? -args_qdt_2mc : args_qdt_2mc;
  const float qdt_4mc = UNCENTER ? (float)(-0.5 * args_qdt_2mc) : (float)(0.5 * args_qdt_2mc);
  const float one = 1.f, one_third = 1. / 3., two_fifteenths = 2. / 15.;
  const float dx = rec.x, dy = rec.y, dz = rec.z;
  const float4 *f = fi + (size_t)record_cell(rec) * 5;
  const float4 fe_x = f[0], fe_y = f[1], fe_z = f[2], fb0 = f[3];
  const float2 fb1 = *reinterpret_cast<const float2 *>(f + 4);
// ... 118 lines not shown
```

### old-vpic_amd/engine.py

```python
import collections
import ctypes as C

import numpy as np

from . import layout as L
from ._lib import lib


class VpicHipError(RuntimeError):
    pass


class GridDesc(C.Structure):
    _fields_ = [("dt", C.c_float), ("cvac", C.c_float), ("eps0", C.c_float), ("damp", C.c_float),
                ("dx", C.c_float), ("dy", C.c_float), ("dz", C.c_float),
                ("rdx", C.c_float), ("rdy", C.c_float), ("rdz", C.c_float),
                ("nx", C.c_int32), ("ny", C.c_int32), ("nz", C.c_int32),
                ("fbc", C.c_int32 * 6), ("pbc", C.c_int32 * 6), ("rank", C.c_int32)]

    @property
    def nv(self):
        return L.nv(self.nx, self.ny, self.nz)


# ... 711 lines not shown
    def pack_jf(self, d, dev_ptr):
        self._ck(self._l.vpic_hip_pack_jf(self._h, d, C.c_void_p(dev_ptr)))

    def unpack_jf(self, d, dev_ptr):
        self._ck(self._l.vpic_hip_unpack_jf(self._h, d, C.c_void_p(dev_ptr)))

    def local_adjust_rho(self):
        self._ck(self._l.vpic_hip_local_adjust_rho(self._h))

    def synchronize_rho_self(self, axis):
        self._ck(self._l.vpic_hip_synchronize_rho_self(self._h, axis))

    def rho_count(self, d):
        return self._l.vpic_hip_rho_count(self._h, d)

    def pack_rho(self, d, dev_ptr):
        self._ck(self._l.vpic_hip_pack_rho(self._h, d, C.c_void_p(dev_ptr)))

    def unpack_rho(self, d, dev_ptr):
        self._ck(self._l.vpic_hip_unpack_rho(self._h, d, C.c_void_p(dev_ptr)))

    def local_adjust_hydro(self):
        self._ck(self._l.vpic_hip_local_adjust_hydro(self._h))

    def synchronize_hydro_self(self, axis):
        self._ck(self._l.vpic_hip_synchronize_hydro_self(self._h, axis))

    def hydro_count(self, d):
        return self._l.vpic_hip_hydro_count(self._h, d)

    def pack_hydro(self, d, dev_ptr):
        self._ck(self._l.vpic_hip_pack_hydro(self._h, d, C.c_void_p(dev_ptr)))

    def unpack_hydro(self, d, dev_ptr):
        self._ck(self._l.vpic_hip_unpack_hydro(self._h, d, C.c_void_p(dev_ptr)))

    def message_count(self, kind, d):
        return self._l.vpic_hip_face_message_count(self._h, kind, d)

    def pack_message(self, kind, d, dev_ptr):
        self._ck(self._l.vpic_hip_pack_face_message(self._h, kind, d, C.c_void_p(dev_ptr)))

    def unpack_message(self, kind, d, dev_ptr):
        err = C.c_double()
        self._ck(self._l.vpic_hip_unpack_face_message(self._h, kind, d, C.c_void_p(dev_ptr), C.byref(err)))
        return err.value

    def local_adjust_tang_e_norm_b(self):
        self._ck(self._l.vpic_hip_local_adjust_tang_e_norm_b(self._h))

    def synchronize_tang_e_norm_b_self(self, axis):
        err = C.c_double()
        self._ck(self._l.vpic_hip_synchronize_tang_e_norm_b_self(self._h, axis, C.byref(err)))
        return err.value

    def rms_div_e_err_local(self):
        l2 = (C.c_double * 2)()
        self._ck(self._l.vpic_hip_rms_div_e_err_local(self._h, l2))
        return l2[0], l2[1]

    def rms_div_b_err_local(self):
        l2 = (C.c_double * 2)()
        self._ck(self._l.vpic_hip_rms_div_b_err_local(self._h, l2))
        return l2[0], l2[1]

    def sort_due(self, sp, max_interval=0):
        d = C.c_int()
        self._ck(self._l.vpic_hip_sort_due(self._h, sp, int(max_interval), C.byref(d)))
        return bool(d.value)

    def set_sort_order(self, order):
        self._ck(self._l.vpic_hip_set_sort_order(self._h, {"reference": 0, "engine": 1}[order]))

    def species_order(self, sp):
        o = C.c_int(0)
        self._ck(self._l.vpic_hip_species_sort_order(self._h, sp, C.byref(o)))
        return ("none", "voxel", "tile")[o.value]

    def species_stats(self, sp):
        out = (C.c_int64 * 8)()
        self._ck(self._l.vpic_hip_species_stats(self._h, int(sp), out))
        return dict(zip(("crossed", "fullest_tile", "missed_runs", "sorts", "early_sorts", "too_clumped_for_tiles", "by_tile_only", "dead_slots"), [int(v) for v in out]))

    def measure_disorder(self, sp):
        f = C.c_double()
        self._ck(self._l.vpic_hip_measure_disorder(self._h, sp, C.byref(f)))
        return f.value

    def step(self, step, sort_interval=0):
        self._ck(self._l.vpic_hip_step(self._h, int(step), int(sort_interval)))

    def sync(self):
        self._ck(self._l.vpic_hip_sync(self._h))

    def stream(self):
        return self._l.vpic_hip_stream(self._h)

    def profile_enable(self, on=True):
        self._ck(self._l.vpic_hip_profile_enable(self._h, int(on)))

    def profile_read(self):
        ms, n, parts = C.c_double(), C.c_int64(), C.c_int64()
        self._ck(self._l.vpic_hip_profile_read(self._h, C.byref(ms), C.byref(n), C.byref(parts)))
        return ms.value, n.value, parts.value

    def profile_read_species(self, sp):
        ms, n, parts = C.c_double(), C.c_int64(), C.c_int64()
        self._ck(self._l.vpic_hip_profile_read_species(self._h, int(sp), C.byref(ms), C.byref(n), C.byref(parts)))
        return ms.value, n.value, parts.value

    def profile_read_sorting(self):
        ms, n, parts = C.c_double(), C.c_int64(), C.c_int64()
        self._ck(self._l.vpic_hip_profile_read_sorting(self._h, C.byref(ms), C.byref(n), C.byref(parts)))
        return ms.value, n.value, parts.value
```

Baseline: 60.80 billion.

## Reuse per-tile histogram counts from the hist pass to skip the sort-push counting pass

When the histogram pass runs, each tile's packed shared-memory cell counts and window base are written to a per-species table. The following fused sort-push reads that table instead of re-scanning its particles to count them, and it also skips the follow-window search. The tile decomposition parameters are now loaded from kernargs only when a lane actually falls outside the window, which lowers register pressure. Sort-push particle loads switch to absolute indexing, with an optional nontemporal variant that is off by default. The cost is an extra global table sized ntiles × packed counts, plus the risk of stale counts if particles change between the hist and fuse passes.

```diff
diff --git a/include/vpic_hip.h b/include/vpic_hip.h
--- a/include/vpic_hip.h
+++ b/include/vpic_hip.h
@@ -348,6 +348,7 @@
 int vpic_hip_measure_disorder(vpic_hip_engine_t *e, int sp, double *fraction);
 int vpic_hip_species_sort_order(vpic_hip_engine_t *e, int sp, int *order);
 int vpic_hip_species_stats(vpic_hip_engine_t *e, int sp, int64_t out[8]);
+int vpic_hip_species_sort_counts(vpic_hip_engine_t *e, int sp, int64_t out[2]);
 int vpic_hip_set_sort_order(vpic_hip_engine_t *e, int order);
 
 int vpic_hip_profile_enable(vpic_hip_engine_t *e, int on);
diff --git a/old-vpic_amd/_lib.py b/old-vpic_amd/_lib.py
--- a/old-vpic_amd/_lib.py
+++ b/old-vpic_amd/_lib.py
@@ -131,7 +131,7 @@
 vpic_hip_energy_f vpic_hip_boundary_p_pack vpic_hip_boundary_p_counts vpic_hip_boundary_p_send_buffer
 vpic_hip_boundary_p_inject vpic_hip_boundary_p_get_injectors vpic_hip_local_adjust_jf
 vpic_hip_synchronize_jf_self vpic_hip_face_count vpic_hip_pack_tang_b vpic_hip_unpack_tang_b
-vpic_hip_pack_jf vpic_hip_unpack_jf vpic_hip_step vpic_hip_profile_enable vpic_hip_profile_read vpic_hip_profile_read_sorting vpic_hip_sort_advance_p vpic_hip_species_get_tile_partition vpic_hip_profile_read_species vpic_hip_comm_unique_id vpic_hip_comm_create vpic_hip_comm_destroy vpic_hip_comm_start vpic_hip_comm_finish vpic_hip_comm_stats vpic_hip_comm_timing vpic_hip_species_stats
+vpic_hip_pack_jf vpic_hip_unpack_jf vpic_hip_step vpic_hip_profile_enable vpic_hip_profile_read vpic_hip_profile_read_sorting vpic_hip_sort_advance_p vpic_hip_species_get_tile_partition vpic_hip_profile_read_species vpic_hip_comm_unique_id vpic_hip_comm_create vpic_hip_comm_destroy vpic_hip_comm_start vpic_hip_comm_finish vpic_hip_comm_stats vpic_hip_comm_timing vpic_hip_species_stats vpic_hip_species_sort_counts
 vpic_hip_energy_spectrum vpic_hip_energy_bands vpic_hip_energy_spectrum_stats
 vpic_hip_species_distribution vpic_hip_species_distribution_stats vpic_hip_moments_stats
 vpic_hip_species_distribution_sums vpic_hip_species_distribution_sums_stats
diff --git a/old-vpic_amd/csrc/engine.h b/old-vpic_amd/csrc/engine.h
--- a/old-vpic_amd/csrc/engine.h
+++ b/old-vpic_amd/csrc/engine.h
@@ -98,6 +98,8 @@
   int *hist = nullptr; int64_t hist_count = 0; bool hist_request = false, hist_valid = false;
   bool tail_regrouped = false;
   int *tpart2 = nullptr; int64_t tpart2_count = 0; bool fuse_pending = false;
+  int *tile_counts = nullptr; int64_t tile_counts_tiles = 0; bool counts_in_table = false;
+  int64_t sorts_from_table = 0, sorts_precounted = 0;
   bool phase_pending = false;
   bool tile_valid = false, adaptive = false;
   int64_t n_sorted = 0;
@@ -107,6 +109,7 @@
 };
 
 constexpr int TILE_CELLS = TILE_EDGE * TILE_EDGE * TILE_EDGE;
+constexpr int TILE_COUNT_PACKED = (TILE_EDGE + 2) * (TILE_EDGE + 2) * (TILE_EDGE + 2) / 2, TILE_COUNT_WORDS = TILE_COUNT_PACKED + 1;
 struct TileK {
   int sy, sz, ntx, nty, ntz, ntiles;
   unsigned mul_sy, sh_sy, mul_sz, sh_sz;
@@ -194,6 +197,7 @@
   bool policy_debug = false;
   int follow = -1;
   int fuse_in_step = -1;
+  int sort_counts = -1;
   bool old_sort = false;
   int stage = -1;
   int follow_from = 16;
@@ -421,6 +425,7 @@
 int k_sort_p(Engine *e, Species &s, bool tile_order = false, bool may_fuse = false);
 int k_sort_scan(Engine *e, const int *counts, int *starts, int n1);
 int k_sort_check(Engine *e, Species &s, const int *starts, int n1);
+int k_tile_counts_reserve(Engine *e, Species &s);
 int k_sort_finish(Engine *e, Species &s, bool tile_order, bool coarse);
 int k_tail_sort(Engine *e, Species &s);
 int k_measure_disorder(Engine *e, Species &s, int slot);
diff --git a/old-vpic_amd/csrc/engine.hip b/old-vpic_amd/csrc/engine.hip
--- a/old-vpic_amd/csrc/engine.hip
+++ b/old-vpic_amd/csrc/engine.hip
@@ -35,6 +35,7 @@
   k.policy_debug = getenv("VPIC_HIP_POLICY_DEBUG") != nullptr;
   k.old_sort = getenv("VPIC_HIP_OLD_SORT") != nullptr;
   if (const char *v = getenv("VPIC_HIP_SORT_IN_PUSH")) k.fuse_in_step = atoi(v) != 0 ? 1 : 0;
+  if (const char *v = getenv("VPIC_HIP_SORT_COUNTS")) k.sort_counts = atoi(v) != 0 ? 1 : 0;
   if (const char *v = getenv("VPIC_HIP_FOLLOW")) k.follow = atoi(v) != 0;
   if (const char *v = getenv("VPIC_HIP_STAGE")) k.stage = atoi(v) != 0;
   if (const char *v = getenv("VPIC_HIP_FOLLOW_FROM")) k.follow_from = atoi(v) > 0 ? atoi(v) : 16;
@@ -168,7 +169,7 @@
   for (auto &s : e->species) {
     free_particles(s.p); free_particles(s.aux);
     (void)hipFree(s.tag); (void)hipFree(s.tag2); (void)hipFree(s.tag_aux); (void)hipFree(s.tag2_aux);
-    (void)hipFree(s.pm); (void)hipFree(s.partition); (void)hipFree(s.tpart); (void)hipFree(s.tpart2); (void)hipFree(s.ttail); (void)hipFree(s.hist); (void)hipFree(s.drain_k); (void)hipFree(s.crossed_dev); (void)hipHostFree(s.crossed_host);
+    (void)hipFree(s.pm); (void)hipFree(s.partition); (void)hipFree(s.tpart); (void)hipFree(s.tpart2); (void)hipFree(s.tile_counts); (void)hipFree(s.ttail); (void)hipFree(s.hist); (void)hipFree(s.drain_k); (void)hipFree(s.crossed_dev); (void)hipHostFree(s.crossed_host);
     for (int i = 0; i < 4; i++) if (s.ev[i]) (void)hipEventDestroy(s.ev[i]);
     for (auto ev : s.sp_ev) if (ev) (void)hipEventDestroy(ev);
     for (auto ev : s.hp_ev) if (ev) (void)hipEventDestroy(ev);
@@ -1087,6 +1088,11 @@
   e->species[sp].hist_request = true;
   return 0;
 }
+int vpic_hip_species_sort_counts(vpic_hip_engine_t *e, int sp, int64_t out[2]) {
+  ENGINE(e); SPECIES(e, sp); if (!out) VH_FAIL("Bad output");
+  out[0] = e->species[sp].sorts_from_table; out[1] = e->species[sp].sorts_precounted;
+  return 0;
+}
 int vpic_hip_species_stats(vpic_hip_engine_t *e, int sp, int64_t out[8]) {
   ENGINE(e); SPECIES(e, sp); if (!out) VH_FAIL("Bad output");
   const Species &s = e->species[sp];
diff --git a/old-vpic_amd/csrc/particles.hip b/old-vpic_amd/csrc/particles.hip
--- a/old-vpic_amd/csrc/particles.hip
+++ b/old-vpic_amd/csrc/particles.hip
@@ -508,6 +508,7 @@
   if (s.np == s.n_holes) { s.np = 0; s.n_holes = 0; }
   if (s.np == 0) return 0;
   if (!s.aux.r && alloc_particles(s.aux, s.max_np)) return 1;
+  if (tile_order && e->knobs.sort_counts != 0 && e->knobs.fuse_in_step != 0 && !s.has_tags && k_tile_counts_reserve(e, s)) return 1;
   if (s.has_tags && !s.tag_aux) {
     VH_CHECK(hipMalloc(&s.tag_aux, sizeof(int64_t) * s.max_np));
     VH_CHECK(hipMalloc(&s.tag2_aux, sizeof(int64_t) * s.max_np));
@@ -521,6 +522,7 @@
       VH_CHECK(hipMalloc(&s.tpart2, sizeof(int) * n1));
       s.tpart2_count = n1;
     }
+    if (e->knobs.sort_counts != 0 && k_tile_counts_reserve(e, s)) return 1;
     s.fuse_pending = true; s.tile_valid = true;
     return 0;
   }
diff --git a/old-vpic_amd/csrc/policy.h b/old-vpic_amd/csrc/policy.h
--- a/old-vpic_amd/csrc/policy.h
+++ b/old-vpic_amd/csrc/policy.h
@@ -139,10 +139,12 @@
   int wx[2] = {0, 0}, wmargin = 0, threads = 0, max_iters = 0;
   bool tile_valid = false, chargeless = false, coarse_sorted = false, det_acc = false, time_kernels = false;
   bool fuse_pending = false, hist_request = false, hist_valid = false, fuse_buffers = false;
+  bool counts_table = false, counts_in_table = false; int sort_counts = -1;
 };
 enum class PushInstance { chargeless, det_tile_only, det_tile, det_row, tile_only, tile_sort, tile_hist, tile, row_wide, row_narrow };
 struct PushPlan {
   bool tiled = false, fuse = false, sort_first = false, regroup_tail = false, hist = false, det = false; int stage = 0;
+  bool keep_counts = false, from_counts = false;
   PushInstance instance = PushInstance::row_narrow;
 };
 
@@ -172,6 +174,8 @@
   pl.regroup_tail = pl.tiled && behind >= in.tail_sort_min && behind > 0 && !in.no_tail_sort;
   pl.hist = !pl.fuse && in.hist_request && pl.tiled && !in.coarse_sorted && in.phase == 0 && !(in.det_acc && !in.chargeless) &&
             (uint64_t)in.fullest_tile + (uint64_t)behind < 30000u;
+  pl.keep_counts = pl.hist && in.counts_table && in.sort_counts != 0;
+  pl.from_counts = pl.fuse && in.counts_table && in.counts_in_table && in.hist_valid && in.sort_counts != 0;
   pl.det = in.det_acc && !in.chargeless;
   pl.instance = in.chargeless ? PushInstance::chargeless
               : pl.det ? (pl.tiled ? (in.coarse_sorted ? PushInstance::det_tile_only : PushInstance::det_tile) : PushInstance::det_row)
diff --git a/old-vpic_amd/csrc/push.hip b/old-vpic_amd/csrc/push.hip
--- a/old-vpic_amd/csrc/push.hip
+++ b/old-vpic_amd/csrc/push.hip
@@ -58,6 +58,18 @@
 __device__ __forceinline__ void stf_nt(float *base, unsigned off, float v) { __builtin_nontemporal_store(v, reinterpret_cast<float *>(reinterpret_cast<char *>(base) + off)); }
 
 
+#ifndef VPIC_HIP_SORT_NT_LOADS
+#define VPIC_HIP_SORT_NT_LOADS 0
+#endif
+__device__ __forceinline__ rec4 sort_ldr(float4 *base, unsigned at) {
+  if (VPIC_HIP_SORT_NT_LOADS) return __builtin_nontemporal_load(rec_at(base, at));
+  return *rec_at(base, at);
+}
+__device__ __forceinline__ float sort_ldf(const float *base, unsigned off) {
+  if (VPIC_HIP_SORT_NT_LOADS) return __builtin_nontemporal_load(reinterpret_cast<const float *>(reinterpret_cast<const char *>(base) + off));
+  return ldf(base, off);
+}
+
 __device__ __forceinline__ int in_vgpr(int s) { int v; asm volatile("v_mov_b32 %0, %1" : "=v"(v) : "s"(s)); return v; }
 
 __device__ __forceinline__ int mbcnt64(unsigned long long m) {
@@ -99,12 +111,29 @@
   }
 }
 
-struct HistK { int *hist; unsigned *s_cnt; TileK tk; };
+struct HistK { int *hist; unsigned *s_cnt; };
+constexpr int KERNARG_PUSH_PARAMS = 64;
+static_assert(sizeof(ParticlesK) == 40 && alignof(PushParams) == 8, "where PushParams lies in advance_p_kernel's argument");
+__device__ __forceinline__ TileK tile_k_outside(int sy, int sz, const TileDiv &td) {
+  int ntx, nty, nx, ny, nz;
+  asm volatile("s_load_dword %0, %5, %6\n\ts_load_dword %1, %5, %7\n\ts_load_dword %2, %5, %8\n\ts_load_dword %3, %5, %9\n\ts_load_dword %4, %5, %10\n\ts_waitcnt lgkmcnt(0)"
+               : "=&s"(ntx), "=&s"(nty), "=&s"(nx), "=&s"(ny), "=&s"(nz)
+               : "s"(__builtin_amdgcn_kernarg_segment_ptr()), "n"(KERNARG_PUSH_PARAMS + offsetof(PushParams, ntx)), "n"(KERNARG_PUSH_PARAMS + offsetof(PushParams, nty)),
+                 "n"(KERNARG_PUSH_PARAMS + offsetof(PushParams, nx)), "n"(KERNARG_PUSH_PARAMS + offsetof(PushParams, ny)), "n"(KERNARG_PUSH_PARAMS + offsetof(PushParams, nz)));
+  TileK tk;
+  tk.sy = sy; tk.sz = sz; tk.ntx = ntx; tk.nty = nty; tk.ntz = 0; tk.ntiles = 0;
+  tk.mul_sy = td.mul_sy; tk.sh_sy = td.sh_sy; tk.mul_sz = td.mul_sz; tk.sh_sz = td.sh_sz;
+  tk.mx = nx - 1; tk.my = ny - 1; tk.mz = nz - 1;
+  return tk;
+}
 template <class W>
 __device__ __forceinline__ void hist_count(const HistK &h, int key, int wbase, int sy, int sz, const TileDiv &td) {
   const int slot = slot_of<W>(key, wbase, sy, sz, td);
   if (slot >= 0) atomicAdd(&h.s_cnt[slot >> 1], 1u << ((slot & 1) << 4));
-  else atomicAdd(&h.hist[sort_key<true>(key, h.tk)], 1);
+  if (__ballot(slot < 0)) {
+    const TileK tk = tile_k_outside(sy, sz, td);
+    if (slot < 0) atomicAdd(&h.hist[sort_key<true>(key, tk)], 1);
+  }
 }
 
 template <class W>
@@ -180,9 +209,11 @@
     const unsigned long long inc = __ballot(counted);
     const unsigned long long run = ((2ull << lane) - 1ull) & ~((1ull << (lane - d)) - 1ull);
     const int n = __popcll(inc & run);
-    if (tail && key >= 0 && n) {
-      if (slot >= 0) atomicAdd(&hk->s_cnt[slot >> 1], (unsigned)n << ((slot & 1) << 4));
-      else atomicAdd(&hk->hist[sort_key<true>(key, hk->tk)], n);
+    const bool counts = tail && key >= 0 && n;
+    if (counts && slot >= 0) atomicAdd(&hk->s_cnt[slot >> 1], (unsigned)n << ((slot & 1) << 4));
+    if (__ballot(counts && slot < 0)) {
+      const TileK tk = tile_k_outside(sy, sz, td);
+      if (counts && slot < 0) atomicAdd(&hk->hist[sort_key<true>(key, tk)], n);
     }
     deposit_run<W>(tail && key >= 0, a, key, lane, s_acc, g_acc, wbase, sy, sz, td, ml, n_miss, slot);
     return;
@@ -417,6 +448,9 @@
   return n_again;
 }
 
+__host__ __device__ __forceinline__ int *counts_out(const PushParams &P) { return P.next; }
+__host__ __device__ __forceinline__ int *counts_in(const PushParams &P) { return P.hist; }
+__device__ __forceinline__ unsigned tile_row(const int *tile_list, unsigned chunk) { return tile_list ? (unsigned)tile_list[chunk] : chunk; }
 constexpr int TAIL_CHUNK = 1024;
 
 template <bool CHARGELESS = false, bool FAST = false, int WIN = 0, bool HIST = false, bool SORT = false>
@@ -454,6 +488,7 @@
   int first, last, wave_span = 0, tile_base = NO_WINDOW;
   int first2 = 0, last2 = 0;
   int bx0 = 0, by0 = 0, bz0 = 0;
+  const bool from_counts = SORT && counts_in(P) != nullptr;
   if (TILE) {
     if (chunk < (unsigned)P.n_launch) {
       const unsigned tile = P.tile_list ? (unsigned)P.tile_list[chunk] : chunk;
@@ -486,7 +521,7 @@
   constexpr int FOLLOW_REACH = 3;
   int sample = -1;
   bool follow = false;
-  if (TILE && VPIC_HIP_FOLLOW && tile_base != NO_WINDOW) {
+  if (TILE && VPIC_HIP_FOLLOW && tile_base != NO_WINDOW && !from_counts) {
     unsigned flag = 0;
     if (P.follow < 0) asm volatile("s_load_dword %0, %1, 0x8\n\ts_waitcnt lgkmcnt(0)" : "=s"(flag) : "s"(P.crossed));
     follow = P.follow > 0 || flag == 1u;
@@ -523,6 +558,8 @@
         }
         if (lane == 0) s_wbase = best[0] + P.sy * best[1] + P.sz * best[2];
       }
+    } else if (SORT && from_counts && tile_base != NO_WINDOW) {
+      if (tid == 0) s_wbase = counts_in(P)[(size_t)tile_row(P.tile_list, chunk) * TILE_COUNT_WORDS + TILE_COUNT_PACKED];
     } else if (tid == 0) s_wbase = tile_base;
   } else if (DET) {
     if (tid == 0) s_wbase = NO_WINDOW;
@@ -561,9 +598,6 @@
   HistK hk;
   if (HIST || SORT) {
     hk.hist = P.hist; hk.s_cnt = s_cnt;
-    hk.tk.sy = P.sy; hk.tk.sz = P.sz; hk.tk.ntx = P.ntx; hk.tk.nty = P.nty; hk.tk.ntz = P.ntz; hk.tk.ntiles = P.ntiles;
-    hk.tk.mul_sy = P.mul_sy; hk.tk.sh_sy = P.sh_sy; hk.tk.mul_sz = P.mul_sz; hk.tk.sh_sz = P.sh_sz;
-    hk.tk.mx = P.nx - 1; hk.tk.my = P.ny - 1; hk.tk.mz = P.nz - 1;
   }
 
   float st0x = 0.f, st0y = 0.f, st0z = 0.f, st1x = 0.f, st1y = 0.f, st1z = 0.f;
@@ -610,6 +644,7 @@
 
   if (SORT) {
     typedef __attribute__((address_space(1))) int *global_int_ptr;
+    if (!from_counts) {
 #pragma unroll 1
     for (int seg = 0; seg < 2; seg++) {
       const int sfirst = seg ? first2 : first, slast = seg ? last2 : last;
@@ -633,11 +668,14 @@
       }
     }
     __syncthreads();
+    }
+    const int *const counted = (from_counts && wbase != NO_WINDOW) ? counts_in(P) + (size_t)tile_row(P.tile_list, chunk) * TILE_COUNT_WORDS : nullptr;
+    const TileK tk_reserve = tile_k_outside(gsy, gsz, td);
     for (int t = tid; t < W::NSLOT; t += PUSH_THREADS) {
-      const unsigned c = s_cnt[t];
+      const unsigned c = counted ? ((unsigned)counted[t >> 1] >> ((t & 1) << 4)) & 0xffffu : s_cnt[t];
       if (c) {
         const int lx = t % WX, lyz = t / WX, ly = lyz % WX, lz = lyz / WX;
-        s_cnt[t] = (unsigned)__hip_atomic_fetch_add((global_int_ptr)P.next + sort_key<true>(wbase + lx + gsy * ly + gsz * lz, hk.tk), (int)c,
+        s_cnt[t] = (unsigned)__hip_atomic_fetch_add((global_int_ptr)P.next + sort_key<true>(wbase + lx + gsy * ly + gsz * lz, tk_reserve), (int)c,
                                                     __ATOMIC_RELAXED, __HIP_MEMORY_SCOPE_AGENT);
       }
     }
@@ -664,7 +702,12 @@
   const int vrel_max = TILE ? in_vgpr(P.np - 1 - sfirst) : P.np - 1 - sfirst;
   rec4 r_rec;
   float r_ux, r_uy, r_uz, r_q;
-  {
+  const int vabs_max = SORT ? in_vgpr(P.np - 1) : 0;
+  if (SORT) {
+    const unsigned ka = (unsigned)min(wave_first + lane, P.np - 1);
+    r_rec = sort_ldr(p.r, ka);
+    r_ux = sort_ldf(p.ux, ka << 2); r_uy = sort_ldf(p.uy, ka << 2); r_uz = sort_ldf(p.uz, ka << 2); r_q = sort_ldf(p.q, ka << 2);
+  } else {
     const unsigned k4 = (unsigned)min(wave_first - sfirst + lane, P.np - 1 - sfirst) << 2;
     r_rec = ldr(pw.r, k4 << 2);
     r_ux = ldf(pw.ux, k4); r_uy = ldf(pw.uy, k4); r_uz = ldf(pw.uz, k4); r_q = ldf(pw.q, k4);
@@ -708,8 +751,9 @@
       int b = 0;
       if (reserves && slot >= 0) b = (int)atomicAdd(&s_cnt[slot], (unsigned)(run_end - lane));
       if (__ballot(reserves && slot < 0)) {
+        const TileK tk = tile_k_outside(vsy, vsz, vtd);
         if (reserves && slot < 0)
-          b = __hip_atomic_fetch_add((global_int_ptr)P.next + sort_key<true>(key, hk.tk), run_end - lane, __ATOMIC_RELAXED, __HIP_MEMORY_SCOPE_AGENT);
+          b = __hip_atomic_fetch_add((global_int_ptr)P.next + sort_key<true>(key, tk), run_end - lane, __ATOMIC_RELAXED, __HIP_MEMORY_SCOPE_AGENT);
       }
       sort_b = b; sort_head = head;
     }
@@ -717,7 +761,11 @@
     const float4 fe_x = f[0], fe_y = f[1], fe_z = f[2], fb0 = f[3];
     const float2 fb1 = *reinterpret_cast<const float2 *>(f + 4);
     __builtin_amdgcn_sched_barrier(0);
-    {
+    if (SORT) {
+      const unsigned ka = (unsigned)min(base + ((it + 1 < wave_passes) ? PASS_STRIDE : 0) + lane, vabs_max);
+      r_rec = sort_ldr(p.r, ka);
+      r_ux = sort_ldf(p.ux, ka << 2); r_uy = sort_ldf(p.uy, ka << 2); r_uz = sort_ldf(p.uz, ka << 2); r_q = sort_ldf(p.q, ka << 2);
+    } else {
       const int k = base - sfirst + ((it + 1 < wave_passes) ? PASS_STRIDE : 0) + lane;
       const unsigned k4 = (unsigned)min(k, vrel_max) << 2;
       r_rec = ldr(pw.r, k4 << 2);
@@ -889,10 +937,15 @@
   __syncthreads();
   if (ablate & 8) return;
   if (HIST && wbase != NO_WINDOW) {
+    const TileK tk_flush = tile_k_outside(gsy, gsz, td);
     for (int slot = tid; slot < W::NSLOT; slot += PUSH_THREADS) {
       const unsigned n = (s_cnt[slot >> 1] >> ((slot & 1) << 4)) & 0xffffu;
       const int lx = slot % WX, lyz = slot / WX, ly = lyz % WX, lz = lyz / WX;
-      if (n) atomicAdd(&P.hist[sort_key<true>(wbase + lx + gsy * ly + gsz * lz, hk.tk)], (int)n);
+      if (n) atomicAdd(&P.hist[sort_key<true>(wbase + lx + gsy * ly + gsz * lz, tk_flush)], (int)n);
+    }
+    if (counts_out(P)) {
+      int *const row = counts_out(P) + (size_t)tile_row(P.tile_list, chunk) * TILE_COUNT_WORDS;
+      if (tid < TILE_COUNT_WORDS) row[tid] = tid < TILE_COUNT_PACKED ? (int)s_cnt[tid] : wbase;
     }
   }
   const int k = tid % 12, c0 = tid / 12;
@@ -972,6 +1025,16 @@
   return 0;
 }
 
+int k_tile_counts_reserve(Engine *e, Species &s) {
+  const int64_t ntiles = make_tile_k(e->gk).ntiles;
+  if (s.tile_counts && s.tile_counts_tiles >= ntiles) return 0;
+  if (s.tile_counts) VH_CHECK(hipFree(s.tile_counts));
+  s.tile_counts = nullptr; s.tile_counts_tiles = 0; s.counts_in_table = false;
+  VH_CHECK(hipMalloc(&s.tile_counts, sizeof(int) * (size_t)ntiles * TILE_COUNT_WORDS));
+  s.tile_counts_tiles = ntiles;
+  return 0;
+}
+
 static int begin_profile(Engine *e, int64_t particles, int kind = 0, int species = -1) {
   if (!e->profile) return -1;
   if (e->ev_used == e->ev_pool.size()) {
@@ -1058,6 +1121,8 @@
     in.wx[0] = Window<false>::WX; in.wx[1] = Window<true>::WX; in.wmargin = WMARGIN; in.threads = PUSH_THREADS; in.max_iters = PUSH_ITERS;
     in.tile_valid = s.tile_valid; in.chargeless = s.chargeless; in.coarse_sorted = s.coarse_sorted; in.det_acc = e->det_acc; in.time_kernels = e->time_kernels;
     in.fuse_pending = s.fuse_pending; in.hist_request = s.hist_request; in.hist_valid = s.hist_valid; in.fuse_buffers = s.aux.r && s.tpart2;
+    in.sort_counts = e->knobs.sort_counts; in.counts_in_table = s.counts_in_table;
+    in.counts_table = s.tile_counts && s.tile_counts_tiles >= make_tile_k(e->gk).ntiles;
     P.iters = push_passes(s.pol, in);
     int64_t seg_start[4]; int32_t seg_count[4]; uint32_t seg_grid[4];
     const int n_seg = vpic_hip_push_plan(s.np, P.iters, seg_start, seg_count, seg_grid, 4);
@@ -1107,6 +1172,8 @@
       VH_CHECK(hipMemsetAsync(s.hist, 0, sizeof(int) * n1, e->stream));
       P.hist = s.hist; P.ntz = tk.ntz;
     } else { P.hist = nullptr; P.ntz = fuse ? make_tile_k(e->gk).ntz : 0; }
+    if (pl.keep_counts) P.next = s.tile_counts;
+    if (pl.from_counts) P.hist = s.tile_counts;
     if (det && acc_prepare_det(e)) return 1;
     P.acc_scale = e->acc_scale;
     float *const g_acc = det ? reinterpret_cast<float *>(e->acc64) : reinterpret_cast<float *>(e->acc);
@@ -1130,8 +1197,9 @@
     }
 #undef PUSH_LAUNCH
     if (ev >= 0) (void)hipEventRecord(e->ev_pool[ev].second, e->stream);
-    if (hist) s.hist_valid = true;
+    if (hist) { s.hist_valid = true; s.counts_in_table = pl.keep_counts; }
     if (fuse) {
+      if (pl.from_counts) s.sorts_from_table++; else s.sorts_precounted++;
       const TileK tk = make_tile_k(e->gk);
       const int n1 = tk.ntiles * TILE_CELLS + 1;
       if (k_sort_check(e, s, s.tpart2, n1)) return 1;
diff --git a/old-vpic_amd/engine.py b/old-vpic_amd/engine.py
--- a/old-vpic_amd/engine.py
+++ b/old-vpic_amd/engine.py
@@ -817,6 +817,11 @@
         self._ck(self._l.vpic_hip_species_stats(self._h, int(sp), out))
         return dict(zip(("crossed", "fullest_tile", "missed_runs", "sorts", "early_sorts", "too_clumped_for_tiles", "by_tile_only", "dead_slots"), [int(v) for v in out]))
 
+    def species_sort_counts(self, sp):
+        out = (C.c_int64 * 2)()
+        self._ck(self._l.vpic_hip_species_sort_counts(self._h, int(sp), out))
+        return int(out[0]), int(out[1])
+
     def measure_disorder(self, sp):
         f = C.c_double()
         self._ck(self._l.vpic_hip_measure_disorder(self._h, sp, C.byref(f)))
```

After: 60.81 billion (median of 2 runs). No clear change (+0.0%).
